# quanpn90/avsr

Hardware: AMD Instinct MI355X
Metric: AV-frames/sec/GPU (fwd+bwd) on 15s clips; WER parity on LRS2 test (higher is better)
Workload: dtype bf16

## Files before the change

### avsr_amd/_lib.py

```python
import ctypes
import os

import torch

_HERE = os.path.dirname(os.path.abspath(__file__))
LIB_PATH = os.environ.get("AVSR_LIB_PATH_AB") or os.path.join(_HERE, "libavsr_hip.so")

AVSR_F32, AVSR_BF16 = 0, 1
ACT_NONE, ACT_GELU, ACT_RELU = 0, 1, 2

_c_p = ctypes.c_void_p
_i64 = ctypes.c_int64
_f = ctypes.c_float
_i = ctypes.c_int


class GemmParams(ctypes.Structure):
    _fields_ = [
        ("M", _i), ("N", _i), ("K", _i), ("batch", _i),
        ("dtype", _i), ("a_kmajor", _i), ("b_kmajor", _i), ("c_f32", _i),
        ("A", _c_p), ("lda", _i64), ("strideA", _i64),
        ("B", _c_p), ("ldb", _i64), ("strideB", _i64),
        ("C", _c_p), ("ldc", _i64), ("strideC", _i64),
        ("alpha", _f), ("beta", _f),
        ("bias", _c_p),
        ("act", _i), ("epi_bwd", _i),
        ("preact", _c_p),
        ("res", _c_p), ("ldr", _i64), ("strideR", _i64),
        ("gate", _c_p),
        ("drop_p", _f),
        ("seed", ctypes.c_uint64),
        ("splitk", _i),
        ("ws", _c_p),
        ("db", _c_p),
        ("db_ws", _c_p),
        ("stamp", _c_p),
        ("skinny_ws", _c_p), ("ln_c1", _c_p), ("ln_eps", ctypes.c_float),
        ("kv_k", _c_p), ("kv_v", _c_p), ("kv_pos", _c_p), ("kv_rows", _i),
        ("slab_cnt", _c_p), ("kv_pos_stride", _i),
    ]


class ConvParams(ctypes.Structure):
    _fields_ = [
        ("dtype", _i),
        ("nimg", _i), ("hin", _i), ("win", _i), ("cin", _i),
        ("hout", _i), ("wout", _i), ("cout", _i),
        ("kh", _i), ("kw", _i), ("sh", _i), ("sw", _i), ("ph", _i), ("pw", _i),
        ("groups", _i),
        ("ldx", _i64), ("ldy", _i64),
        ("x", _c_p), ("w", _c_p), ("y", _c_p),
        ("dx", _c_p), ("dy", _c_p), ("dw", _c_p),
        ("stats", _c_p),
        ("alpha", _f), ("beta", _f),
        ("splitk", _i),
        ("bias", _c_p), ("act", _i), ("preact", _c_p), ("res", _c_p),
        ("ws", _c_p),
        ("bnr_h", _c_p), ("bnr_res", _c_p), ("bnr_scale", _c_p), ("bnr_shift", _c_p), ("bnr_prelu", _c_p),
        ("bnr_mean", _c_p), ("bnr_invstd", _c_p), ("bnr_scale2", _c_p), ("bnr_shift2", _c_p),
        ("bnr_mean2", _c_p), ("bnr_invstd2", _c_p), ("bnr_ws", _c_p),
    ]


class LayerNormParams(ctypes.Structure):
    _fields_ = [
        ("dtype", _i), ("rows", _i), ("N", _i), ("eps", _f),
        ("x", _c_p), ("ldx", _i64), ("y", _c_p), ("ldy", _i64),
        ("gamma", _c_p), ("beta", _c_p), ("mean", _c_p), ("rstd", _c_p),
        ("dy", _c_p), ("lddy", _i64), ("dx", _c_p), ("lddx", _i64),
        ("dres", _c_p), ("lddres", _i64), ("dgamma", _c_p), ("dbeta", _c_p), ("ws", _c_p),
        ("g", _c_p), ("ldg", _i64), ("drop_p", _f), ("seed", ctypes.c_uint64), ("db", _c_p),
    ]


class BnFinalizeParams(ctypes.Structure):
    _fields_ = [
        ("tiles", _i), ("C", _i), ("partials", _c_p), ("gamma", _c_p), ("beta", _c_p),
        ("running_mean", _c_p), ("running_var", _c_p), ("momentum", _f), ("eps", _f),
        ("training", _i), ("mean", _c_p), ("invstd", _c_p), ("scale", _c_p), ("shift", _c_p),
    ]


class BnActParams(ctypes.Structure):
    _fields_ = [
        ("dtype", _i), ("M", _i), ("C", _i),
        ("h", _c_p), ("scale", _c_p), ("shift", _c_p), ("res", _c_p), ("scale2", _c_p), ("shift2", _c_p),
        ("prelu", _c_p), ("y", _c_p), ("dy", _c_p), ("dz", _c_p),
        ("mean", _c_p), ("invstd", _c_p), ("mean2", _c_p), ("invstd2", _c_p),
        ("sums", _c_p), ("dprelu", _c_p), ("dgamma", _c_p), ("dbeta", _c_p), ("dgamma2", _c_p), ("dbeta2", _c_p),
        ("dh", _c_p), ("dh2", _c_p), ("beta_acc", _f), ("ws", _c_p),
    ]


class StemPoolParams(ctypes.Structure):
    _fields_ = [
        ("dtype", _i), ("nimg", _i), ("H", _i), ("W", _i), ("C", _i), ("Ho", _i), ("Wo", _i),
        ("h", _c_p), ("scale", _c_p), ("shift", _c_p), ("prelu", _c_p), ("y", _c_p), ("argmax", _c_p),
        ("dy", _c_p), ("dz", _c_p), ("mean", _c_p), ("invstd", _c_p),
        ("sums", _c_p), ("dprelu", _c_p), ("dgamma", _c_p), ("dbeta", _c_p), ("ws", _c_p),
        ("hmax", _c_p), ("dh", _c_p), ("m_total", _i64),
    ]


class AttnParams(ctypes.Structure):
    _fields_ = [
        ("dtype", _i), ("B", _i), ("H", _i), ("Lq", _i), ("Lk", _i), ("scale", _f),
        ("q", _c_p), ("ldq", _i64), ("k", _c_p), ("ldk", _i64), ("v", _c_p), ("ldv", _i64),
        ("o", _c_p), ("ldo", _i64), ("lse", _c_p), ("klen", _c_p), ("causal", _i),
        ("drop_p", _f), ("seed", ctypes.c_uint64),
        ("dout", _c_p), ("lddo", _i64), ("delta", _c_p), ("dq", _c_p), ("lddq", _i64),
        ("dk", _c_p), ("lddk", _i64), ("dv", _c_p), ("lddv", _i64), ("dq_out", _c_p), ("lddq_out", _i64),
        ("db", _c_p), ("db_ws", _c_p), ("drop_mask", _c_p),
    ]


class XentParams(ctypes.Structure):
    _fields_ = [
        ("dtype", _i), ("rows", _i), ("V", _i), ("x", _c_p), ("ldx", _i64), ("target", _c_p),
        ("smoothing", _f), ("lse", _c_p), ("row_loss", _c_p), ("row_correct", _c_p),
        ("dloss", _c_p), ("coef", _f), ("dx", _c_p), ("lddx", _i64),
    ]


class CtcParams(ctypes.Structure):
    _fields_ = [
        ("dtype", _i), ("B", _i), ("T", _i), ("V", _i), ("Lmax", _i), ("x", _c_p), ("ldx", _i64),
        ("lse", _c_p), ("labels", _c_p), ("label_len", _c_p), ("in_len", _c_p),
        ("alpha", _c_p), ("gamma", _c_p), ("nll", _c_p), ("dloss", _c_p), ("coef", _f),
        ("dx", _c_p), ("lddx", _i64),
    ]


class CtcAlignParams(ctypes.Structure):
    _fields_ = [
        ("dtype", _i), ("B", _i), ("T", _i), ("V", _i), ("Lmax", _i), ("blank", _i), ("x", _c_p), ("ldx", _i64),
        ("lse", _c_p), ("labels", _c_p), ("label_len", _c_p), ("in_len", _c_p),
        ("ws", _c_p), ("ali", _c_p), ("score", _c_p), ("feasible", _c_p),
    ]


class CtcBeamParams(ctypes.Structure):
    _fields_ = [
        ("U", _i), ("Tm", _i), ("V", _i), ("N", _i), ("C", _i), ("blank", _i), ("eos", _i), ("Lcap", _i),
        ("logp", _c_p), ("ldp", _i64), ("tlen", _c_p), ("cand", _c_p), ("ws", _c_p),
        ("n_out", _c_p), ("tokens", _c_p), ("len", _c_p), ("score", _c_p),
    ]


class EwParams(ctypes.Structure):
    _fields_ = [
        ("dtype", _i), ("rows", _i), ("N", _i), ("dy", _c_p), ("lddy", _i64), ("out", _c_p), ("ldout", _i64),
        ("gate", _c_p), ("ldgate", _i64), ("act", _i), ("drop_p", _f), ("seed", ctypes.c_uint64),
        ("alpha", _f), ("db", _c_p), ("ws", _c_p),
    ]


class EmbedParams(ctypes.Structure):
    _fields_ = [
        ("dtype", _i), ("rows", _i), ("L", _i), ("D", _i), ("tok", _c_p), ("table", _c_p), ("pe", _c_p),
        ("scale", _f), ("y", _c_p), ("drop_p", _f), ("seed", ctypes.c_uint64), ("dy", _c_p), ("dtable", _c_p),
        ("pe_row", _c_p), ("pe_row_stride", _i),
    ]


class AdamWParams(ctypes.Structure):
    _fields_ = [
        ("n", _i64), ("param", _c_p), ("grad", _c_p), ("exp_avg", _c_p), ("exp_avg_sq", _c_p),
        ("shadow", _c_p), ("shadow_dtype", _i), ("lr", _f), ("beta1", _f), ("beta2", _f), ("eps", _f),
        ("weight_decay", _f), ("bias_corr1", _f), ("bias_corr2", _f), ("sumsq", _c_p), ("max_norm", _f),
        ("grad_scale", _f), ("max_blocks", _i), ("grad_clear", _c_p),
    ]


def fill(struct_cls, **kw):
    p = struct_cls()
    keep = []
    for k, v in kw.items():
        if v is None:
            continue
        if isinstance(v, torch.Tensor):
            keep.append(v)
            v = v.data_ptr()
        setattr(p, k, v)
    p._keep = keep
    return p


class DecAttnParams(ctypes.Structure):
    _fields_ = [
        ("dtype", _i), ("n", _i), ("H", _i), ("klen_max", _i), ("scale", _f),
        ("q", _c_p), ("ldq", _i64), ("k", _c_p), ("ldk", _i64), ("k_bstride", _i64),
        ("v", _c_p), ("ldv", _i64), ("v_bstride", _i64), ("klen", _c_p), ("o", _c_p), ("ldo", _i64),
        ("kidx", _c_p), ("kmap", _c_p), ("ldmap", _i64), ("group", _i), ("ksplit", _i), ("ws", _c_p),
        ("cnt", _c_p),
    ]


class TopkParams(ctypes.Structure):
    _fields_ = [("rows", _i), ("V", _i), ("K", _i), ("x", _c_p), ("ldx", _i64), ("ids", _c_p)]


class CtcPrefixParams(ctypes.Structure):
    _fields_ = [
        ("n", _i), ("T", _i), ("V", _i), ("P", _i), ("blank", _i), ("eos", _i), ("out_len", _i),
        ("logp", _c_p), ("r_prev", _c_p), ("last", _c_p), ("ids", _c_p), ("r_new", _c_p), ("psi", _c_p),
        ("uidx", _c_p), ("logp_ustride", _i64), ("tlen", _c_p), ("out_len_dev", _c_p),
        ("out_len_stride", _i),
    ]


class BeamSelectParams(ctypes.Structure):
    _fields_ = [
        ("n", _i), ("V", _i), ("P", _i), ("beam", _i), ("blank", _i), ("eos", _i), ("w_dec", _f), ("w_ctc", _f),
        ("dec", _c_p), ("ld", _i64), ("ids", _c_p), ("psi", _c_p), ("s_prev", _c_p), ("score", _c_p),
        ("out_prev", _c_p), ("out_tok", _c_p), ("out_col", _c_p), ("out_score", _c_p), ("out_dec", _c_p),
        ("out_ctc", _c_p), ("out_s", _c_p), ("nseg", _i), ("seg", _c_p),
        ("bonus", _c_p), ("next", _c_p), ("out_bonus", _c_p), ("out_next", _c_p),
        ("lm", _c_p), ("lm_next", _c_p), ("w_lm", _f), ("w_len", _f), ("lm_hi", _f), ("out_lm", _c_p),
        ("out_lm_next", _c_p),
    ]


class NgramLMStruct(ctypes.Structure):
    _fields_ = [
        ("order", _i), ("nodes", _i), ("V", _i), ("start", _i),
        ("child_off", _c_p), ("backoff", _c_p), ("fail", _c_p), ("tok", _c_p), ("logp", _c_p), ("next", _c_p),
        ("uni_logp", _c_p), ("uni_next", _c_p),
    ]


class NgramParams(ctypes.Structure):
    _fields_ = [
        ("lm", NgramLMStruct), ("R", _i), ("P", _i), ("blank", _i), ("eos", _i),
        ("state", _c_p), ("ids", _c_p), ("out", _c_p), ("out_next", _c_p),
    ]

# ... 25 lines not shown
        ("sel_bonus", _c_p), ("sel_next", _c_p), ("shw", _c_p), ("end_hw", _c_p), ("node_out", _c_p),
        ("sel_lm", _c_p), ("sel_lm_next", _c_p), ("slm", _c_p), ("end_lm", _c_p), ("lm_state_out", _c_p),
        ("slen", _c_p), ("end_len", _c_p), ("lm_start", _i),
    ]


class BeamSlotResetParams(ctypes.Structure):
    _fields_ = [
        ("U", _i), ("beam", _i), ("R", _i), ("Lmax", _i), ("slot", _i), ("sos", _i), ("maxlen", _i), ("tlen", _i),
        ("upos", _c_p), ("rowpos", _c_p), ("done", _c_p),
        ("tok", _c_p), ("score", _c_p), ("sdec", _c_p), ("sctc", _c_p), ("s_prev", _c_p),
        ("best_len", _c_p), ("best_end", _c_p), ("maxlen_arr", _c_p), ("tlen_arr", _c_p), ("klen_mem", _c_p),
    ]


class FbankParams(ctypes.Structure):
    _fields_ = [
        ("B", _i), ("T", _i), ("wav", _c_p), ("ldw", _i64), ("n_samples", _c_p),
        ("bins", _i * 28), ("preemph", _f), ("ln_eps", _f), ("out", _c_p),
    ]


class TimeMaskParams(ctypes.Structure):
    _fields_ = [("B", _i), ("L", _i), ("nspan", _i), ("row_bytes", _i64), ("clip_stride_bytes", _i64),
                ("x", _c_p), ("spans", _c_p)]


class AddNoiseParams(ctypes.Structure):
    _fields_ = [("B", _i), ("L", _i), ("x", _c_p), ("ldx", _i64), ("noise", _c_p), ("ldn", _i64),
                ("lengths", _c_p), ("snr_db", _c_p), ("y", _c_p), ("ldy", _i64), ("ws", _c_p)]


class VideoNormParams(ctypes.Structure):
    _fields_ = [
        ("B", _i), ("T", _i), ("H", _i), ("W", _i), ("crop", _i), ("oy", _i), ("ox", _i),
        ("frames", _c_p), ("mean", _f), ("std", _f), ("out", _c_p),
    ]


SYMBOLS = {
    "avsr_version": ([], ctypes.c_char_p),
    "avsr_set_option": ([_i, _i64], _i),
    "avsr_get_option": ([_i], _i64),
    "avsr_gemm": ([ctypes.POINTER(GemmParams), _c_p], _i),
    "avsr_gemm_wgrad_group": ([ctypes.POINTER(GemmParams), _i, _c_p], _i),
    "avsr_gemm_skinny_splits": ([_i, _i, _i], _i),
    "avsr_conv_fwd": ([ctypes.POINTER(ConvParams), _c_p], _i),
    "avsr_conv_bwd_data": ([ctypes.POINTER(ConvParams), _c_p], _i),
    "avsr_conv_bwd_weight": ([ctypes.POINTER(ConvParams), _c_p], _i),
    "avsr_conv_stat_tiles": ([ctypes.POINTER(ConvParams)], _i),
    "avsr_conv_bnr_tiles": ([ctypes.POINTER(ConvParams)], _i),
    "avsr_conv_wgrad_ws": ([ctypes.POINTER(ConvParams)], _i64),
    "avsr_conv_path": ([ctypes.POINTER(ConvParams), _i], _i),
    "avsr_layernorm_fwd": ([ctypes.POINTER(LayerNormParams), _c_p], _i),
    "avsr_layernorm_bwd": ([ctypes.POINTER(LayerNormParams), _c_p], _i),
    "avsr_bn_finalize": ([ctypes.POINTER(BnFinalizeParams), _c_p], _i),
    "avsr_bn_act_fwd": ([ctypes.POINTER(BnActParams), _c_p], _i),
    "avsr_bn_act_bwd_reduce": ([ctypes.POINTER(BnActParams), _c_p], _i),
    "avsr_bn_bwd_apply": ([ctypes.POINTER(BnActParams), _c_p], _i),
    "avsr_stem_pool_fwd": ([ctypes.POINTER(StemPoolParams), _c_p], _i),
    "avsr_stem_pool_bwd_apply": ([ctypes.POINTER(StemPoolParams), _c_p], _i),
    "avsr_bn_bwd_finalize": ([ctypes.POINTER(BnActParams), _i, _c_p], _i),
    "avsr_avgpool_fwd": ([_i, _i, _i, _i, _c_p, _c_p, _c_p], _i),
    "avsr_avgpool_bwd": ([_i, _i, _i, _i, _c_p, _c_p, _c_p], _i),
    "avsr_attn_fwd": ([ctypes.POINTER(AttnParams), _c_p], _i),
    "avsr_debug_attn_stamps": ([_c_p], _i),
    "avsr_attn_bwd_prep": ([ctypes.POINTER(AttnParams), _c_p], _i),
    "avsr_attn_bwd": ([ctypes.POINTER(AttnParams), _c_p], _i),
    "avsr_attn_dropmask": ([ctypes.POINTER(AttnParams), _c_p], _i),
    "avsr_attn_path": ([ctypes.POINTER(AttnParams), _i], _i),
    "avsr_row_lse": ([ctypes.POINTER(XentParams), _c_p], _i),
    "avsr_lsm_fwd": ([ctypes.POINTER(XentParams), _c_p], _i),
    "avsr_lsm_bwd": ([ctypes.POINTER(XentParams), _c_p], _i),
    "avsr_ctc_fwd": ([ctypes.POINTER(CtcParams), _c_p], _i),
    "avsr_ctc_bwd": ([ctypes.POINTER(CtcParams), _c_p], _i),
    "avsr_ctc_align": ([ctypes.POINTER(CtcAlignParams), _c_p], _i),
    "avsr_ctc_beam": ([ctypes.POINTER(CtcBeamParams), _c_p], _i),
    "avsr_loss_finalize": ([_i, _c_p, _i, _c_p, _c_p, _f, _i, _c_p, _c_p], _i),
    "avsr_ew_bwd": ([ctypes.POINTER(EwParams), _c_p], _i),
    "avsr_colsum_defer": ([_i], _i),
    "avsr_colsum_flush": ([_c_p], _i),
    "avsr_colsum_inline": ([_i], _i),
    "avsr_dropout_fwd": ([ctypes.POINTER(EwParams), _c_p], _i),
    "avsr_mask_rows": ([_i, _i, _i, _i, _c_p, _i64, _c_p, _c_p], _i),
    "avsr_embed_fwd": ([ctypes.POINTER(EmbedParams), _c_p], _i),
    "avsr_embed_bwd": ([ctypes.POINTER(EmbedParams), _c_p], _i),
    "avsr_cast": ([_i, _i, _i, _i, _c_p, _i64, _c_p, _i64, _f, _f, _c_p], _i),
    "avsr_cast_flat": ([_i, _i, _i64, _c_p, _c_p, _c_p], _i),
    "avsr_stem_pack": ([_i, _i, _i, _c_p, _c_p, _c_p], _i),
    "avsr_stem_wpack": ([_i, _c_p, _c_p, _c_p], _i),
    "avsr_stem_conv_tiles": ([_i, _i], _i),
    "avsr_stem_wpack2": ([_c_p, _c_p, _c_p], _i),
    "avsr_stem_conv_fwd": ([_i, _i, _c_p, _c_p, _c_p, _c_p, _c_p], _i),
    "avsr_stem_wgrad_unpack": ([_c_p, _c_p, _c_p], _i),
    "avsr_audio_pack": ([_i, _i, _i, _i, _c_p, _c_p, _c_p], _i),
    "avsr_weightnorm_fwd": ([_i, _i, _i, _i, _c_p, _c_p, _c_p, _c_p, _c_p], _i),
    "avsr_weightnorm_bwd": ([_i, _i, _i, _c_p, _c_p, _c_p, _c_p, _c_p, _c_p, _c_p, _c_p], _i),
    "avsr_sumsq": ([_c_p, _i64, _c_p, _c_p, _c_p], _i),
    "avsr_adamw": ([ctypes.POINTER(AdamWParams), _c_p], _i),
    "avsr_log_softmax_rows": ([_i, _i, _i, _c_p, _i64, _c_p, _i64, _c_p], _i),
    "avsr_dec_attn": ([ctypes.POINTER(DecAttnParams), _c_p], _i),
    "avsr_row_topk": ([ctypes.POINTER(TopkParams), _c_p], _i),
    "avsr_log_softmax_topk": ([_i, _i, _i, _c_p, _i64, _c_p, _i64, _i, _c_p, _c_p], _i),
    "avsr_ctc_prefix": ([ctypes.POINTER(CtcPrefixParams), _c_p], _i),
    "avsr_beam_select": ([ctypes.POINTER(BeamSelectParams), _c_p], _i),
    "avsr_hotword_step": ([ctypes.POINTER(HotwordParams), _c_p], _i),
    "avsr_ngram_step": ([ctypes.POINTER(NgramParams), _c_p], _i),
    "avsr_ngram_score_seqs": ([ctypes.POINTER(NgramSeqParams), _c_p], _i),
    "avsr_beam_step_prep": ([_i, _i, _c_p, _c_p, _c_p, _c_p], _i),
    "avsr_beam_kv_put": ([_i, _i, _i, _c_p, _i64, _c_p, _c_p, _c_p, _c_p], _i),
    "avsr_beam_post": ([ctypes.POINTER(BeamPostParams), _c_p], _i),
    "avsr_beam_step_prep_rows": ([_i, _i, _c_p, _c_p, _c_p, _c_p], _i),
    "avsr_beam_kv_put_rows": ([_i, _i, _i, _c_p, _i64, _c_p, _c_p, _c_p, _c_p], _i),
    "avsr_beam_slot_reset": ([ctypes.POINTER(BeamSlotResetParams), _c_p], _i),
    "avsr_gather_rows": ([_i, _i, _i64, _c_p, _i64, _i64, _c_p, _i64, _i64, _c_p, _c_p], _i),
    "avsr_fbank_stack": ([ctypes.POINTER(FbankParams), _c_p], _i),
    "avsr_video_normalize": ([ctypes.POINTER(VideoNormParams), _c_p], _i),
    "avsr_time_mask": ([ctypes.POINTER(TimeMaskParams), _c_p], _i),
    "avsr_add_noise": ([ctypes.POINTER(AddNoiseParams), _c_p], _i),
    "avsr_rgb_to_gray": ([_c_p, _c_p, _i64, _c_p], _i),
}

_lib = None


class AvsrLibError(RuntimeError):
    pass


def load():
    global _lib
    if _lib is not None:
        return _lib
    if not os.path.exists(LIB_PATH):
        raise AvsrLibError(f"{LIB_PATH} not built: run `python -c 'import __graft_entry__ as g; g.build()'`")
    lib = ctypes.CDLL(LIB_PATH, mode=ctypes.RTLD_GLOBAL)
    for name, (argtypes, restype) in SYMBOLS.items():
        if os.environ.get("AVSR_LIB_PATH_AB") and not hasattr(lib, name):
            continue
        fn = getattr(lib, name)
        fn.argtypes = argtypes
        fn.restype = restype
    _lib = lib
    return lib


def check(rc, op):
    if rc != 0:
        raise AvsrLibError(f"{op} failed with code {rc}")


OPTIONS = {"gemm_tile": 0, "attn_sq_fwd": 1, "attn_sq_bwd": 2, "wgrad_dual": 3, "conv_192": 4, "conv_s2phase": 5,
           "conv_patch": 6, "conv_wpatch": 7, "stem_pool_2x2": 8,
           "stem_wpatch": 9, "attn_enc_fused": 10}
TILES = ["128", "256", "256x128", "128x256", "128s3", "128w8s3", "pp", "192", "192x256", "192w8s3", "64", "64s4"]
ATTN_PATHS = ["f32", "tiled", "resident", "sq", "enc"]
CONV_PATHS = ["reg", "glds", "patch", "s2", "wpatch", "stem_wpatch"]
CONV_PASSES = ["fwd", "dgrad", "wgrad"]


def set_option(name, value):
    if name == "gemm_tile" and not isinstance(value, int):
        value = 0 if value in (None, "auto") else TILES.index(value) + 1
    lib = load()
    prev = get_option(name)
    check(lib.avsr_set_option(OPTIONS[name], int(value)), f"avsr_set_option({name}, {value})")
# ... 19 lines not shown
```

### avsr_amd/csrc/common.h

```cpp
#pragma once
#include <hip/hip_runtime.h>
#include <stdint.h>
#include "avsr_hip.h"

typedef __bf16 bf16;
typedef __bf16 bf16x8 __attribute__((ext_vector_type(8)));
typedef __bf16 bf16x4 __attribute__((ext_vector_type(4)));
typedef float f32x16 __attribute__((ext_vector_type(16)));
typedef float f32x4 __attribute__((ext_vector_type(4)));
typedef int v4i32 __attribute__((ext_vector_type(4)));
typedef float f32x2 __attribute__((ext_vector_type(2)));

#define AVSR_DEV __device__ __forceinline__

AVSR_DEV float to_f(float x) { return x; }
AVSR_DEV float to_f(bf16 x) { return (float)x; }
template <typename T> AVSR_DEV T from_f(float x);
template <> AVSR_DEV float from_f<float>(float x) { return x; }
template <> AVSR_DEV bf16 from_f<bf16>(float x) { return (bf16)x; }

struct alignas(16) v16 { uint32_t w[4]; };

AVSR_DEV float fexp2(float x) { return __builtin_amdgcn_exp2f(x); }

template <int R> AVSR_DEV float rorf(float x) {
  return __int_as_float(__builtin_amdgcn_update_dpp(0, __float_as_int(x), 0x120 + R, 0xf, 0xf, false));
}
template <int R> AVSR_DEV int rori(int x) { return __builtin_amdgcn_update_dpp(0, x, 0x120 + R, 0xf, 0xf, false); }
AVSR_DEV float lanef(float x, int l) { return __int_as_float(__builtin_amdgcn_readlane(__float_as_int(x), l)); }
AVSR_DEV float row_sum16(float x) {
  x += rorf<8>(x); x += rorf<4>(x); x += rorf<2>(x); x += rorf<1>(x);
  return x;
}
AVSR_DEV float wave_sum(float x) {
  x = row_sum16(x);
  return (lanef(x, 0) + lanef(x, 16)) + (lanef(x, 32) + lanef(x, 48));
}
AVSR_DEV float xor32_max(float x) {
  const auto r = __builtin_amdgcn_permlane32_swap(__float_as_uint(x), __float_as_uint(x), false, false);
  return fmaxf(__uint_as_float(r[0]), __uint_as_float(r[1]));
}
AVSR_DEV float xor32_sum(float x) {
  const auto r = __builtin_amdgcn_permlane32_swap(__float_as_uint(x), __float_as_uint(x), false, false);
  return __uint_as_float(r[0]) + __uint_as_float(r[1]);
}
AVSR_DEV float wave_max(float x) {
  x = fmaxf(x, rorf<8>(x)); x = fmaxf(x, rorf<4>(x)); x = fmaxf(x, rorf<2>(x)); x = fmaxf(x, rorf<1>(x));
  return fmaxf(fmaxf(lanef(x, 0), lanef(x, 16)), fmaxf(lanef(x, 32), lanef(x, 48)));
}

AVSR_DEV uint32_t fmix32(uint32_t h) {
  h ^= h >> 16; h *= 0x85EBCA6Bu;
  h ^= h >> 13; h *= 0xC2B2AE35u;
  return h ^ (h >> 16);
}
AVSR_DEV uint32_t mix32_hi(uint64_t seed, uint32_t hi) {
  return (uint32_t)seed ^ fmix32(hi ^ (uint32_t)(seed >> 32) ^ 0x68E31DA4u);
}
AVSR_DEV uint32_t mix32_lo(uint32_t pre, uint32_t lo) { return fmix32((lo * 0x9E3779B1u) ^ pre); }
AVSR_DEV uint32_t mix32(uint64_t seed, uint64_t idx) {
  return mix32_lo(mix32_hi(seed, (uint32_t)(idx >> 32)), (uint32_t)idx);
}
AVSR_DEV uint32_t drop_thr16(float p) { return (uint32_t)(p * 65536.f + 0.5f); }
AVSR_DEV float drop_keep_scale(uint32_t thr) { return thr < 65536u ? 65536.f / (float)(65536u - thr) : 0.f; }
AVSR_DEV uint32_t drop_half(uint32_t h, bool odd) { return odd ? (h >> 16) : (h & 0xFFFFu); }

AVSR_DEV float drop_scale(float p, uint64_t seed, uint64_t idx) {
  const uint32_t thr = drop_thr16(p);
  return drop_half(mix32(seed, idx >> 1), idx & 1) >= thr ? drop_keep_scale(thr) : 0.0f;
}

AVSR_DEV void drop8(float p, uint64_t seed, uint64_t d0, float* v) {
  const uint32_t thr = drop_thr16(p);
  const float ks = drop_keep_scale(thr);
  const uint64_t p0 = d0 >> 1;
  const uint32_t lo = (uint32_t)p0;
  if (!(d0 & 1) && lo <= 0xFFFFFFFCu) {
    const uint32_t pre = mix32_hi(seed, (uint32_t)(p0 >> 32));
    const uint32_t g0 = lo * 0x9E3779B1u;
#pragma unroll
    for (int q = 0; q < 4; ++q) {
      const uint32_t h = fmix32((g0 + (uint32_t)q * 0x9E3779B1u) ^ pre);
      v[2 * q] *= (h & 0xFFFFu) >= thr ? ks : 0.0f;
      v[2 * q + 1] *= (h >> 16) >= thr ? ks : 0.0f;
    }
  } else {
#pragma unroll
    for (int q = 0; q < 8; ++q) v[q] *= drop_scale(p, seed, d0 + q);
  }
}

AVSR_DEV float gelu_erf(float x) { return 0.5f * x * (1.0f + erff(x * 0.70710678118654752f)); }
AVSR_DEV float gelu_erf_grad(float x) {
  float cdf = 0.5f * (1.0f + erff(x * 0.70710678118654752f));
  float pdf = 0.39894228040143268f * __expf(-0.5f * x * x);
  return cdf + x * pdf;
}
AVSR_DEV float erf_as(float z, float ez2) {
  const float t = __builtin_amdgcn_rcpf(fmaf(0.3275911f, fabsf(z), 1.0f));
  const float p = t * fmaf(t, fmaf(t, fmaf(t, fmaf(t, 1.061405429f, -1.453152027f), 1.421413741f), -0.284496736f), 0.254829592f);
  return copysignf(fmaf(-p, ez2, 1.0f), z);
}
AVSR_DEV float gelu_fast(float x) {
  const float z = x * 0.70710678118654752f;
  return 0.5f * x * (1.0f + erf_as(z, __expf(-z * z)));
}
AVSR_DEV float gelu_fast_grad(float x) {
  const float z = x * 0.70710678118654752f, e = __expf(-z * z);
  return 0.5f * (1.0f + erf_as(z, e)) + x * 0.39894228040143268f * e;
}
typedef float f32x2 __attribute__((ext_vector_type(2)));
AVSR_DEV f32x2 erf_as2(f32x2 z, f32x2 ez2) {
  const f32x2 az = {fabsf(z.x), fabsf(z.y)};
  const f32x2 d = az * 0.3275911f + 1.0f;
  const f32x2 t = {__builtin_amdgcn_rcpf(d.x), __builtin_amdgcn_rcpf(d.y)};
  f32x2 p = t * 1.061405429f + -1.453152027f;
  p = p * t + 1.421413741f;
  p = p * t + -0.284496736f;
  p = p * t + 0.254829592f;
  const f32x2 r = 1.0f - (p * t) * ez2;
  return f32x2{copysignf(r.x, z.x), copysignf(r.y, z.y)};
}
AVSR_DEV f32x2 exp_negsq2(f32x2 z) {
  const f32x2 q = z * z;
  return f32x2{__expf(-q.x), __expf(-q.y)};
}
AVSR_DEV f32x2 gelu_fast2(f32x2 x) {
  const f32x2 z = x * 0.70710678118654752f;
  const f32x2 hx = x * 0.5f;
  return hx + hx * erf_as2(z, exp_negsq2(z));
}
AVSR_DEV f32x2 gelu_fast_grad2(f32x2 x) {
  const f32x2 z = x * 0.70710678118654752f, e = exp_negsq2(z);
  return 0.5f + 0.5f * erf_as2(z, e) + (x * 0.39894228040143268f) * e;
}
template <typename T> AVSR_DEV float act_fwd_t(int act, float h) {
  if constexpr (sizeof(T) == 2) return act == AVSR_ACT_GELU ? gelu_fast(h) : (act == AVSR_ACT_RELU ? fmaxf(h, 0.f) : h);
  else return act == AVSR_ACT_GELU ? gelu_erf(h) : (act == AVSR_ACT_RELU ? fmaxf(h, 0.f) : h);
}
template <typename T> AVSR_DEV float act_bwd_t(int act, float h) {
  if constexpr (sizeof(T) == 2) return act == AVSR_ACT_GELU ? gelu_fast_grad(h) : (act == AVSR_ACT_RELU ? (h > 0.f ? 1.f : 0.f) : 1.f);
  else return act == AVSR_ACT_GELU ? gelu_erf_grad(h) : (act == AVSR_ACT_RELU ? (h > 0.f ? 1.f : 0.f) : 1.f);
}
AVSR_DEV float act_fwd(int act, float h) {
  return act == AVSR_ACT_GELU ? gelu_erf(h) : (act == AVSR_ACT_RELU ? fmaxf(h, 0.f) : h);
}
AVSR_DEV float act_bwd(int act, float h) {
  return act == AVSR_ACT_GELU ? gelu_erf_grad(h) : (act == AVSR_ACT_RELU ? (h > 0.f ? 1.f : 0.f) : 1.f);
}

AVSR_DEV void split8(const float* x, bf16x8& hi, bf16x8& lo) {
#pragma unroll
  for (int j = 0; j < 8; ++j) {
    bf16 h = (bf16)x[j];
    hi[j] = h;
    lo[j] = (bf16)(x[j] - (float)h);
  }
}

AVSR_DEV f32x4 mfma16(const bf16x8& a, const bf16x8& b, const f32x4& c) {
  return __builtin_amdgcn_mfma_f32_16x16x32_bf16(a, b, c, 0, 0, 0);
}
AVSR_DEV f32x16 mfma32(const bf16x8& a, const bf16x8& b, const f32x16& c) {
  return __builtin_amdgcn_mfma_f32_32x32x16_bf16(a, b, c, 0, 0, 0);
}

int64_t avsr_opt(int option);

#define AVSR_CHECK_LAUNCH() do { hipError_t e_ = hipGetLastError(); if (e_ != hipSuccess) return (int)e_; } while (0)

static inline int avsr_aligned16(const void* p) { return ((uintptr_t)p & 15u) == 0; }

// ... 52 lines not shown
```

### avsr_amd/csrc/elementwise.hip

```cpp
#include "common.h"

namespace {

struct EwArgs {
  int rows, N;
  const void* dy; int64_t lddy; void* out; int64_t ldout;
  const void* gate; int64_t ldgate; int act;
  float drop_p; uint64_t seed; float alpha; float* db; float* ws;
};

template <typename T>
__global__ __launch_bounds__(256) void ew_bwd_kernel(EwArgs a) {
  constexpr int VE = VecW<T>::VE;
  __shared__ float red[4 * 64 * 8];
  const int nv = a.N / VE;
  const int cvl = threadIdx.x & 63, rl = threadIdx.x >> 6;
  const int cv = blockIdx.x * 64 + cvl;
  const int chunk = (a.rows + gridDim.y - 1) / gridDim.y;
  const int r0 = blockIdx.y * chunk, r1 = min(a.rows, r0 + chunk);
  float acc[VE];
#pragma unroll
  for (int j = 0; j < VE; ++j) acc[j] = 0.f;
  if (cv < nv) {
    for (int r = r0 + rl; r < r1; r += 4) {
      float d[VE], g[VE];
      ldv((const T*)a.dy + (int64_t)r * a.lddy + cv * VE, d);
      if (a.gate) ldv((const T*)a.gate + (int64_t)r * a.ldgate + cv * VE, g);
#pragma unroll
      for (int j = 0; j < VE; ++j) d[j] *= a.alpha;
      if (a.drop_p > 0.f) {
        const uint64_t i0 = (uint64_t)r * a.N + cv * VE;
        if constexpr (VE == 8) drop8(a.drop_p, a.seed, i0, d);
        else {
#pragma unroll
          for (int j = 0; j < VE; ++j) d[j] *= drop_scale(a.drop_p, a.seed, i0 + j);
        }
      }
#pragma unroll
      for (int j = 0; j < VE; ++j) {
        float v = d[j];
        if (a.gate) v *= act_bwd_t<T>(a.act, g[j]);
        acc[j] += v;
        d[j] = v;
      }
      if (a.out) stv((T*)a.out + (int64_t)r * a.ldout + cv * VE, d);
    }
  }
  if (!a.db) return;
#pragma unroll
  for (int j = 0; j < VE; ++j) red[(rl * 64 + cvl) * VE + j] = acc[j];
  __syncthreads();
  if (rl == 0 && cv < nv) {
#pragma unroll
    for (int j = 0; j < VE; ++j) {
      const float t = red[(0 * 64 + cvl) * VE + j] + red[(1 * 64 + cvl) * VE + j] + red[(2 * 64 + cvl) * VE + j] +
                      red[(3 * 64 + cvl) * VE + j];
      a.ws[(int64_t)blockIdx.y * a.N + cv * VE + j] = t;
    }
  }
}

template <typename T>
__global__ __launch_bounds__(256) void mask_rows_kernel(int B, int T_, int N, T* x, int64_t ldx, const int* len) {
  constexpr int VE = VecW<T>::VE;
  const int nv = N / VE;
  const int64_t total = (int64_t)B * T_ * nv;
  for (int64_t i = blockIdx.x * 256 + threadIdx.x; i < total; i += (int64_t)gridDim.x * 256) {
    const int64_t row = i / nv;
    const int b = (int)(row / T_), t = (int)(row % T_);
    if (t >= len[b]) {
      float z[VE];
#pragma unroll
      for (int j = 0; j < VE; ++j) z[j] = 0.f;
      stv(x + row * ldx + (i % nv) * VE, z);
    }
  }
}

template <typename T>
__global__ __launch_bounds__(256) void embed_kernel(avsr_embed_params p, int bwd) {
  constexpr int VE = VecW<T>::VE;
  const int nv = p.D / VE;
  const int64_t total = (int64_t)p.rows * nv;
  for (int64_t i = blockIdx.x * 256 + threadIdx.x; i < total; i += (int64_t)gridDim.x * 256) {
    const int r = (int)(i / nv), d0 = (int)(i % nv) * VE;
    const int tok = p.tok[r];
    const int pos = p.pe_row ? p.pe_row[(int64_t)r * p.pe_row_stride] : r % p.L;
    if (!bwd) {
      float e[VE], o[VE];
      ldv((const T*)p.table + (int64_t)tok * p.D + d0, e);
#pragma unroll
      for (int j = 0; j < VE; ++j) {
        float v = e[j] * p.scale + p.pe[(int64_t)pos * p.D + d0 + j];
        if (p.drop_p > 0.f) v *= drop_scale(p.drop_p, p.seed, (uint64_t)r * p.D + d0 + j);
        o[j] = v;
      }
      stv((T*)p.y + (int64_t)r * p.D + d0, o);
    }
  }
}

template <typename T>
__global__ __launch_bounds__(256) void embed_bwd_kernel(avsr_embed_params p) {
  constexpr int VE = VecW<T>::VE;
  const int r = blockIdx.x;
  const int tok = p.tok[r];
  __shared__ int seen;
  if (threadIdx.x == 0) seen = 0;
  __syncthreads();
  for (int q = threadIdx.x; q < r; q += 256)
    if (p.tok[q] == tok) seen = 1;
  __syncthreads();
  if (seen) return;
  const int nv = p.D / VE;
  for (int c = threadIdx.x; c < nv; c += 256) {
    const int d0 = c * VE;
    float acc[VE];
#pragma unroll
    for (int j = 0; j < VE; ++j) acc[j] = 0.f;
    for (int q = r; q < p.rows; ++q) {
      if (p.tok[q] != tok) continue;
      float g[VE];
      ldv((const T*)p.dy + (int64_t)q * p.D + d0, g);
#pragma unroll
      for (int j = 0; j < VE; ++j) {
        float v = g[j] * p.scale;
        if (p.drop_p > 0.f) v *= drop_scale(p.drop_p, p.seed, (uint64_t)q * p.D + d0 + j);
        acc[j] += v;
      }
    }
    float* dt = p.dtable + (int64_t)tok * p.D + d0;
#pragma unroll
    for (int j = 0; j < VE; ++j) dt[j] += acc[j];
  }
}

template <typename S, typename D>
__global__ __launch_bounds__(256) void cast_kernel(int rows, int cols, const S* src, int64_t lds, D* dst,
                                                   int64_t ldd, float alpha, float beta) {
  const int64_t c0 = ((int64_t)blockIdx.x * 256 + threadIdx.x) * 4;
  if (c0 >= cols) return;
  for (int r = blockIdx.y; r < rows; r += gridDim.y) {
    const S* s = src + (int64_t)r * lds + c0;
    D* d = dst + (int64_t)r * ldd + c0;
#pragma unroll
    for (int q = 0; q < 4; ++q) {
      if (c0 + q < cols) {
        float v = alpha * to_f(s[q]);
        if (beta != 0.f) v += beta * to_f(d[q]);
        d[q] = from_f<D>(v);
      }
    }
  }
}

__global__ __launch_bounds__(256) void cast_flat_f32_bf16_kernel(int64_t n8, const float4* __restrict__ src,
                                                                 bf16x8* __restrict__ dst) {
  for (int64_t i = (int64_t)blockIdx.x * 256 + threadIdx.x; i < n8; i += (int64_t)gridDim.x * 256) {
    const float4 a = src[2 * i], b = src[2 * i + 1];
    bf16x8 o;
    o[0] = (bf16)a.x; o[1] = (bf16)a.y; o[2] = (bf16)a.z; o[3] = (bf16)a.w;
    o[4] = (bf16)b.x; o[5] = (bf16)b.y; o[6] = (bf16)b.z; o[7] = (bf16)b.w;
    dst[i] = o;
  }
}

__global__ __launch_bounds__(256) void cast_flat_bf16_f32_kernel(int64_t n8, const bf16x8* __restrict__ src,
                                                                 float4* __restrict__ dst) {
  for (int64_t i = (int64_t)blockIdx.x * 256 + threadIdx.x; i < n8; i += (int64_t)gridDim.x * 256) {
    const bf16x8 v = src[i];
    dst[2 * i] = float4{(float)v[0], (float)v[1], (float)v[2], (float)v[3]};
    dst[2 * i + 1] = float4{(float)v[4], (float)v[5], (float)v[6], (float)v[7]};
  }
}

template <typename T>
__global__ __launch_bounds__(256) void audio_pack_kernel(int B, int F, int T_, const float* a, T* out) {
  const int64_t total = (int64_t)B * T_ * F;
  for (int64_t i = blockIdx.x * 256 + threadIdx.x; i < total; i += (int64_t)gridDim.x * 256) {
    const int f = (int)(i % F);
    const int64_t bt = i / F;
    const int b = (int)(bt / T_), t = (int)(bt % T_);
    out[i] = from_f<T>(a[((int64_t)b * F + f) * T_ + t]);
  }
}

template <typename T>
int ew_launch(const avsr_ew_params* p, hipStream_t st) {
  constexpr int VE = VecW<T>::VE;
  if (p->N % VE) return AVSR_E_SHAPE;
  if (p->rows == 0) return 0;
  if (p->db && !p->ws) return AVSR_E_ARG;
  const int nv = p->N / VE;
  dim3 grid((nv + 63) / 64, 1);
  int gy = 4096 / (int)grid.x;
  gy = gy < 16 ? 16 : (gy > AVSR_EW_ROWBLOCKS ? AVSR_EW_ROWBLOCKS : gy);
  gy = gy > p->rows ? p->rows : gy;
  grid.y = gy;
  EwArgs a;
  a.rows = p->rows; a.N = p->N; a.dy = p->dy; a.lddy = p->lddy; a.out = p->out; a.ldout = p->ldout;
  a.gate = p->gate; a.ldgate = p->ldgate; a.act = p->act; a.drop_p = p->drop_p; a.seed = p->seed;
  a.alpha = p->alpha; a.db = p->db; a.ws = p->ws;
  hipLaunchKernelGGL(ew_bwd_kernel<T>, grid, dim3(256), 0, st, a);
  AVSR_CHECK_LAUNCH();
  if (p->db) return colsum_launch((const float*)p->ws, (int)grid.y, (int64_t)p->N, p->N, p->db, 0, nullptr, st);
  return 0;
}

int embed_launch(const avsr_embed_params* p, int bwd, hipStream_t st) {
  if (!p) return AVSR_E_ARG;
  return avsr_by_dtype(p->dtype, [&](auto t) -> int {
    using T = decltype(t);
    constexpr int VE = VecW<T>::VE;
    if (p->D % VE) return AVSR_E_SHAPE;
    if (p->rows <= 0) return 0;
    if (bwd) hipLaunchKernelGGL(embed_bwd_kernel<T>, dim3(p->rows), dim3(256), 0, st, *p);
    else hipLaunchKernelGGL(embed_kernel<T>, dim3(avsr_grid((int64_t)p->rows * p->D / VE)), dim3(256), 0, st, *p, bwd);
    AVSR_CHECK_LAUNCH();
    return 0;
  });
}

}

extern "C" int avsr_ew_bwd(const avsr_ew_params* p, void* stream) {
  if (!p) return AVSR_E_ARG;
  return avsr_by_dtype(p->dtype, [&](auto t) -> int { return ew_launch<decltype(t)>(p, (hipStream_t)stream); });
}

extern "C" int avsr_dropout_fwd(const avsr_ew_params* p, void* stream) {
  if (!p) return AVSR_E_ARG;
  return avsr_by_dtype(p->dtype, [&](auto t) -> int {
    if (!p->out) return AVSR_E_ARG;
    avsr_ew_params q = *p;
    q.gate = nullptr; q.db = nullptr;
    return ew_launch<decltype(t)>(&q, (hipStream_t)stream);
  });
}

extern "C" int avsr_mask_rows(int dtype, int B, int T, int N, void* x, int64_t ldx, const int* len, void* stream) {
  return avsr_by_dtype(dtype, [&](auto t) -> int {
    using E = decltype(t);
    constexpr int VE = VecW<E>::VE;
    if (N % VE || ldx % VE) return AVSR_E_ALIGN;
    const int g = avsr_grid((int64_t)B * T * N / VE);
    hipLaunchKernelGGL(mask_rows_kernel<E>, dim3(g), dim3(256), 0, (hipStream_t)stream, B, T, N, (E*)x, ldx, len);
    AVSR_CHECK_LAUNCH();
    return 0;
  });
}

extern "C" int avsr_embed_fwd(const avsr_embed_params* p, void* stream) { return embed_launch(p, 0, (hipStream_t)stream); }
extern "C" int avsr_embed_bwd(const avsr_embed_params* p, void* stream) { return embed_launch(p, 1, (hipStream_t)stream); }

extern "C" int avsr_cast(int sd, int dd, int rows, int cols, const void* src, int64_t lds, void* dst, int64_t ldd,
                         float alpha, float beta, void* stream) {
  if (rows <= 0 || cols <= 0) return 0;
  const int64_t gx = ((int64_t)cols + 1023) / 1024;
  int64_t gy = 4096 / gx;
  gy = gy < 1 ? 1 : (gy > rows ? rows : gy);
  gy = gy > 65535 ? 65535 : gy;
  const dim3 g((unsigned)gx, (unsigned)gy);
  hipStream_t st = (hipStream_t)stream;
  if (sd == AVSR_F32 && dd == AVSR_BF16) hipLaunchKernelGGL((cast_kernel<float, bf16>), dim3(g), dim3(256), 0, st, rows, cols, (const float*)src, lds, (bf16*)dst, ldd, alpha, beta);
  else if (sd == AVSR_F32 && dd == AVSR_F32) hipLaunchKernelGGL((cast_kernel<float, float>), dim3(g), dim3(256), 0, st, rows, cols, (const float*)src, lds, (float*)dst, ldd, alpha, beta);
  else if (sd == AVSR_BF16 && dd == AVSR_F32) hipLaunchKernelGGL((cast_kernel<bf16, float>), dim3(g), dim3(256), 0, st, rows, cols, (const bf16*)src, lds, (float*)dst, ldd, alpha, beta);
  else if (sd == AVSR_BF16 && dd == AVSR_BF16) hipLaunchKernelGGL((cast_kernel<bf16, bf16>), dim3(g), dim3(256), 0, st, rows, cols, (const bf16*)src, lds, (bf16*)dst, ldd, alpha, beta);
  else return AVSR_E_DTYPE;
  AVSR_CHECK_LAUNCH();
  return 0;
}

extern "C" int avsr_cast_flat(int sd, int dd, int64_t n, const void* src, void* dst, void* stream) {
  if (n <= 0) return 0;
  hipStream_t st = (hipStream_t)stream;
  if (sd == AVSR_F32 && dd == AVSR_BF16 && n % 8 == 0 && ((uintptr_t)src & 15) == 0 && ((uintptr_t)dst & 15) == 0) {
    const int64_t n8 = n / 8;
    int64_t g = (n8 + 255) / 256;
    g = g > 256 * 32 ? 256 * 32 : g;
    hipLaunchKernelGGL(cast_flat_f32_bf16_kernel, dim3((unsigned)g), dim3(256), 0, st, n8, (const float4*)src, (bf16x8*)dst);
    AVSR_CHECK_LAUNCH();
    return 0;
  }
  if (sd == AVSR_BF16 && dd == AVSR_F32 && n % 8 == 0 && ((uintptr_t)src & 15) == 0 && ((uintptr_t)dst & 15) == 0) {
    const int64_t n8 = n / 8;
    int64_t g = (n8 + 255) / 256;
    g = g > 256 * 32 ? 256 * 32 : g;
    hipLaunchKernelGGL(cast_flat_bf16_f32_kernel, dim3((unsigned)g), dim3(256), 0, st, n8, (const bf16x8*)src, (float4*)dst);
    AVSR_CHECK_LAUNCH();
    return 0;
  }
  const int64_t cols = 4096, rows = n / cols, tail = n - rows * cols;
  const size_t es = sd == AVSR_F32 ? 4 : 2, ed = dd == AVSR_F32 ? 4 : 2;
  if (rows > 0) {
    const int rc = avsr_cast(sd, dd, (int)rows, (int)cols, src, cols, dst, cols, 1.f, 0.f, stream);
    if (rc) return rc;
  }
  if (tail > 0) return avsr_cast(sd, dd, 1, (int)tail, (const char*)src + rows * cols * es, tail,
                                 (char*)dst + rows * cols * ed, tail, 1.f, 0.f, stream);
  return 0;
}

extern "C" int avsr_audio_pack(int dtype, int B, int F, int T, const float* audio, void* out, void* stream) {
  return avsr_by_dtype(dtype, [&](auto t) -> int {
    using E = decltype(t);
    const int g = avsr_grid((int64_t)B * T * F);
    hipLaunchKernelGGL(audio_pack_kernel<E>, dim3(g), dim3(256), 0, (hipStream_t)stream, B, F, T, audio, (E*)out);
    AVSR_CHECK_LAUNCH();
    return 0;
  });
}
```

### avsr_amd/csrc/gemm.hip

```cpp
#include "gemm_dense.h"
#include "gemm_pp.h"
#include <type_traits>
#include <utility>

using namespace gemmd;

namespace {

template <typename T, typename OutT, int WM, int WN, bool AK, bool BK>
__global__ __launch_bounds__(NT) void dense_kernel(DenseArgs a) {
  extern __shared__ __attribute__((aligned(16))) char smem[];
  using TL = Tile<T, WM, WN, AK, BK>;
  const int z = blockIdx.z, bz = z / a.splits, sp = z % a.splits;
  const int m0 = blockIdx.y * TL::BM, n0 = blockIdx.x * TL::BN;
  using LA = typename std::conditional<AK, LdDenseK<T, TL::BM>, LdDenseR<T, TL::BM>>::type;
  using LB = typename std::conditional<BK, LdDenseK<T, TL::BN>, LdDenseR<T, TL::BN>>::type;
  LA la; la.p = (const T*)a.A + (int64_t)bz * a.sA; la.ld = a.lda; la.rext = a.M; la.K = a.K;
  LB lb; lb.p = (const T*)a.B + (int64_t)bz * a.sB; lb.ld = a.ldb; lb.rext = a.N; lb.K = a.K;
  const int kbeg = sp * a.kchunk, kend = min(a.K, kbeg + a.kchunk);
  f32x16 acc[2][2];
  mainloop<T, WM, WN>(la, lb, m0, n0, kbeg, kend, acc, smem);
  const Epi e = tile_epi<T, OutT, EV_GENERIC>(a, bz, sp);
  epilogue<T, OutT, WM, WN>(e, m0, n0, acc, smem);
}

template <typename OutT, bool AK, bool BK, class CF, int EV = EV_GENERIC>
__global__ __launch_bounds__(CF::NTH, CF::MINB) void dense_glds_kernel(DenseArgs a, int tiles_m, int tiles_n) {
  extern __shared__ __attribute__((aligned(16))) char smem[];
  if (a.stamp != nullptr && threadIdx.x == 0) atomicMin(a.stamp, (unsigned long long)__builtin_amdgcn_s_memrealtime());
  const int id = gemmg::xcd_remap(blockIdx.x, gridDim.x);
  int tm, tn, z;
  gemmg::tile_of(id, tiles_m, tiles_n, tm, tn, z);
  const int bz = z / a.splits, sp = z % a.splits;
  const int m0 = tm * CF::BM, n0 = tn * CF::BN;
  const int kbeg = sp * a.kchunk, kend = min(a.K, kbeg + a.kchunk);
  const int lane = threadIdx.x & 63, wave = __builtin_amdgcn_readfirstlane(threadIdx.x >> 6);
  f32x4 acc[CF::TM][CF::TN];
  const int nk = (kend - kbeg + gemmg::GBK - 1) / gemmg::GBK;
  if (a.a_bytes) {
    using LA = typename std::conditional<AK, gemmg::BDenseK<CF::BM, CF::NW>, gemmg::BDenseR<CF::BM, CF::NW>>::type;
    using LB = typename std::conditional<BK, gemmg::BDenseK<CF::BN, CF::NW>, gemmg::BDenseR<CF::BN, CF::NW>>::type;
    LA la; la.init((const bf16*)a.A + (int64_t)bz * a.sA, a.a_bytes, a.lda, m0, a.M, kend, wave, lane);
    LB lb; lb.init((const bf16*)a.B + (int64_t)bz * a.sB, a.b_bytes, a.ldb, n0, a.N, kend, wave, lane);
    gemmg::mainloop_glds<CF>(la, lb, kbeg, nk, acc, smem);
  } else {
    using LA = typename std::conditional<AK, gemmg::GDenseK<CF::BM, CF::NW>, gemmg::GDenseR<CF::BM, CF::NW>>::type;
    using LB = typename std::conditional<BK, gemmg::GDenseK<CF::BN, CF::NW>, gemmg::GDenseR<CF::BN, CF::NW>>::type;
    LA la; la.init((const bf16*)a.A + (int64_t)bz * a.sA, a.lda, m0, a.M, kend, wave, lane);
    LB lb; lb.init((const bf16*)a.B + (int64_t)bz * a.sB, a.ldb, n0, a.N, kend, wave, lane);
    gemmg::mainloop_glds<CF>(la, lb, kbeg, nk, acc, smem);
  }
  const Epi e = tile_epi<bf16, OutT, EV>(a, bz, sp);
  gemmg::epilogue_g<bf16, OutT, CF, EV>(e, m0, n0, acc, smem);
  if (a.stamp != nullptr) {
    __syncthreads();
    if (threadIdx.x == 0) atomicMax(a.stamp + 1, (unsigned long long)__builtin_amdgcn_s_memrealtime());
  }
}

template <typename OutT, bool AK, bool BK>
__global__ __launch_bounds__(gemmpp::NTH, 1) void dense_pp_kernel(DenseArgs a, int tiles_m, int tiles_n) {
  extern __shared__ __attribute__((aligned(16))) char smem[];
  const int id = gemmg::xcd_remap(blockIdx.x, gridDim.x);
  int tm, tn, z;
  gemmg::tile_of(id, tiles_m, tiles_n, tm, tn, z);
  const int bz = z / a.splits, sp = z % a.splits;
  const int m0 = tm * gemmpp::BM, n0 = tn * gemmpp::BN;
  const int kbeg = sp * a.kchunk, kend = min(a.K, kbeg + a.kchunk);
  const int lane = threadIdx.x & 63, wave = __builtin_amdgcn_readfirstlane(threadIdx.x >> 6);
  using LA = typename std::conditional<AK, gemmpp::HalfK<64>, gemmpp::HalfR<64>>::type;
  using LB = typename std::conditional<BK, gemmpp::HalfK<32>, gemmpp::HalfR<32>>::type;
  LA la; la.init((const bf16*)a.A + (int64_t)bz * a.sA, a.lda, m0, a.M, kend, wave, lane);
  LB lb; lb.init((const bf16*)a.B + (int64_t)bz * a.sB, a.ldb, n0, a.N, kend, wave, lane);
  f32x4 acc[8][4];
  gemmpp::mainloop_pp(la, lb, kbeg, (kend - kbeg + gemmg::GBK - 1) / gemmg::GBK, acc, smem);
  const Epi e = tile_epi<bf16, OutT, EV_GENERIC>(a, bz, sp);
  gemmg::epilogue_g<bf16, OutT, gemmpp::CF>(e, m0, n0, acc, smem);
}

template <typename OutT, bool AK, bool BK>
int launch_pp(const DenseArgs& a, int batch, hipStream_t st) {
  const int tm = (a.M + 255) / 256, tn = (a.N + 255) / 256;
  const long nwg = (long)tm * tn * batch * a.splits;
  if (nwg > 0x7fffffffL) return AVSR_E_SHAPE;
  hipLaunchKernelGGL((dense_pp_kernel<OutT, AK, BK>), dim3((unsigned)nwg), dim3(gemmpp::NTH), gemmpp::LDS_BYTES, st, a,
                     tm, tn);
  AVSR_CHECK_LAUNCH();
  return 0;
}

template <typename OutT>
int epi_variant(const DenseArgs& a, int batch) {
  const Epi& e = a.e;
  if (e.atomic || e.stats || e.rm_wc || e.alpha != 1.f || e.beta != 0.f || (e.N % 8)) return EV_GENERIC;
  const uintptr_t ptrs = (uintptr_t)e.C | (uintptr_t)e.preact | (uintptr_t)e.res | (uintptr_t)e.gate | (uintptr_t)e.bias;
  if (ptrs & 15u) return EV_GENERIC;
  const int64_t so = (int64_t)sizeof(OutT);
  if (((e.ldc * so) | (e.ldc * 2) | (e.ldr * 2)) & 15) return EV_GENERIC;
  if (batch > 1 && (((a.sC * so) | (a.sC * 2) | (a.sR * 2)) & 15)) return EV_GENERIC;
  if (a.splits > 1 && ((a.sSplit * so) & 15)) return EV_GENERIC;
  const bool drop = e.drop_p > 0.f;
  if (!e.bwd) {
    if (e.gate || e.colsum) return EV_GENERIC;
    if (!e.bias) return (!e.preact && !e.act && !e.res && !drop) ? EV_PLAIN : EV_GENERIC;
    if (!e.preact && !e.act && !e.res && !drop) return EV_BIAS;
    if (!e.preact && !e.act && e.res) return EV_BIAS_RES;
    if (e.preact && e.act == AVSR_ACT_GELU && !e.res) return EV_BIAS_ACT_PRE;
    return EV_GENERIC;
  }
  if (e.bias || e.preact || e.res) return EV_GENERIC;
  if (e.gate && e.act == AVSR_ACT_GELU) return EV_GATE;
  if (!e.gate && !e.act && !drop && !e.colsum) return EV_PLAIN;
  return EV_GENERIC;
}

template <typename OutT, bool BK, int EV>
constexpr bool ev_built() {
  if (EV == EV_GENERIC) return true;
  if (sizeof(OutT) != 2) return false;
  return BK ? (EV == EV_BIAS || EV == EV_BIAS_RES || EV == EV_BIAS_ACT_PRE) : (EV == EV_PLAIN || EV == EV_GATE);
}

template <typename OutT, bool AK, bool BK, class CF, int EV>
int launch_glds_ev(const DenseArgs& a, int tm, int tn, long nwg, hipStream_t st) {
  if constexpr (!ev_built<OutT, BK, EV>()) {
    return launch_glds_ev<OutT, AK, BK, CF, EV_GENERIC>(a, tm, tn, nwg, st);
  } else {
    hipLaunchKernelGGL((dense_glds_kernel<OutT, AK, BK, CF, EV>), dim3((unsigned)nwg), dim3(CF::NTH), CF::LDS_BYTES,
                       st, a, tm, tn);
    AVSR_CHECK_LAUNCH();
    return 0;
  }
}

template <typename OutT, bool AK, bool BK, class CF, bool VARIANTS = false>
int launch_glds(const DenseArgs& a, int batch, hipStream_t st) {
  const int tm = (a.M + CF::BM - 1) / CF::BM, tn = (a.N + CF::BN - 1) / CF::BN;
  const long nwg = (long)tm * tn * batch * a.splits;
  if (nwg > 0x7fffffffL) return AVSR_E_SHAPE;
  if constexpr (VARIANTS) {
    switch (epi_variant<OutT>(a, batch)) {
      case EV_PLAIN: return launch_glds_ev<OutT, AK, BK, CF, EV_PLAIN>(a, tm, tn, nwg, st);
      case EV_BIAS: return launch_glds_ev<OutT, AK, BK, CF, EV_BIAS>(a, tm, tn, nwg, st);
      case EV_BIAS_RES: return launch_glds_ev<OutT, AK, BK, CF, EV_BIAS_RES>(a, tm, tn, nwg, st);
      case EV_BIAS_ACT_PRE: return launch_glds_ev<OutT, AK, BK, CF, EV_BIAS_ACT_PRE>(a, tm, tn, nwg, st);
      case EV_GATE: return launch_glds_ev<OutT, AK, BK, CF, EV_GATE>(a, tm, tn, nwg, st);
      default: break;
    }
  }
  return launch_glds_ev<OutT, AK, BK, CF, EV_GENERIC>(a, tm, tn, nwg, st);
}

using Cfg128 = gemmg::GCfg<2, 2, 2, 2, 2>;
using Cfg256 = gemmg::GCfg<2, 4, 4, 2, 2>;
using Cfg256x128 = gemmg::GCfg<4, 2, 2, 2, 3>;
using Cfg128x256 = gemmg::GCfg<2, 4, 2, 2, 3>;
using Cfg128s3 = gemmg::GCfg<2, 2, 2, 2, 3>;
using Cfg128w8s3 = gemmg::GCfg<2, 4, 2, 1, 3>;
using Cfg192 = gemmg::GCfg<2, 2, 3, 2, 2>;
using Cfg192x256 = gemmg::GCfg<2, 4, 3, 2, 2>;
using Cfg192w8s3 = gemmg::GCfg<2, 4, 3, 1, 3>;
using Cfg64 = gemmg::GCfg<2, 2, 1, 1, 2>;
using Cfg64s4 = gemmg::GCfg<2, 2, 1, 1, 4>;
struct CorePP { static constexpr int BM = gemmpp::BM; };

template <int ID_, class CF_, bool VARIANTS_ = false>
struct TileRow {
  static constexpr int ID = ID_;
  static constexpr bool R_OK = 512 % CF_::BM == 0;
  template <bool AK> using CF = std::conditional_t<AK || R_OK, CF_, Cfg128>;
  static constexpr int bm(bool ak) { return ak ? CF<true>::BM : CF<false>::BM; }
  template <typename OutT, bool AK, bool BK>
  static int launch(const DenseArgs& a, int batch, hipStream_t st) {
    if constexpr (std::is_same_v<CF<AK>, CorePP>) return launch_pp<OutT, AK, BK>(a, batch, st);
    else return launch_glds<OutT, AK, BK, CF<AK>, VARIANTS_ && (AK || R_OK)>(a, batch, st);
  }
};
template <class... R> struct TileTable { static constexpr int COUNT = sizeof...(R); };

using Tiles = TileTable<
    TileRow<AVSR_TILE_128, Cfg128>,
    TileRow<AVSR_TILE_256, Cfg256>,
    TileRow<AVSR_TILE_256x128, Cfg256x128>,
    TileRow<AVSR_TILE_128x256, Cfg128x256>,
// ... 23 lines not shown
template <typename OutT, bool AK, bool BK, class... R>
int launch_cfg(TileTable<R...>, int cfg, const DenseArgs& a, int batch, hipStream_t st) {
  int rc = AVSR_E_ARG;
  (void)((cfg == R::ID && ((rc = R::template launch<OutT, AK, BK>(a, batch, st)), true)) || ...);
  return rc;
}

#ifndef AVSR_AB_FWD2
#define AVSR_AB_FWD2 AVSR_TILE_192
#endif
#ifndef AVSR_AB_ROUND1
#define AVSR_AB_ROUND1 AVSR_TILE_192w8s3
#endif
int tile_cfg(const avsr_gemm_params* p, int splits) {
  const int forced = (int)avsr_opt(AVSR_OPT_GEMM_TILE) - 1;
  if (forced >= 0) return forced;
  const long tiles_z = (long)p->batch * splits;
  const long t128 = (long)((p->M + 127) / 128) * ((p->N + 127) / 128) * tiles_z;
  if (p->a_kmajor) {
    const long t192 = (long)((p->M + 191) / 192) * ((p->N + 127) / 128) * tiles_z;
    const long n128 = (t128 + 255) / 256, n192 = (t192 + 255) / 256;
    if (n192 >= 2 && 3 * n192 * 50 <= 2 * n128 * 51) return AVSR_AB_FWD2;
    if (t192 > 128 && t192 <= 256) return AVSR_AB_ROUND1;
  }
  const long t64 = (long)((p->M + 63) / 64) * ((p->N + 63) / 64) * tiles_z;
  if (t128 < 256 && t64 >= 2 * t128) return (t64 <= 256 && p->K >= 2048) ? AVSR_TILE_64s4 : AVSR_TILE_64;
  return AVSR_TILE_128;
}

template <typename OutT>
int glds_by_layout(const avsr_gemm_params* p, int cfg, const DenseArgs& a, hipStream_t st) {
  if (p->a_kmajor && p->b_kmajor) return launch_cfg<OutT, true, true>(Tiles{}, cfg, a, p->batch, st);
  if (p->a_kmajor) return launch_cfg<OutT, true, false>(Tiles{}, cfg, a, p->batch, st);
  if (p->b_kmajor) return launch_cfg<OutT, false, true>(Tiles{}, cfg, a, p->batch, st);
  return launch_cfg<OutT, false, false>(Tiles{}, cfg, a, p->batch, st);
}

template <typename T, typename OutT, int WM, int WN, bool AK, bool BK>
int launch(const DenseArgs& a, int batch, hipStream_t st) {
  using TL = Tile<T, WM, WN, AK, BK>;
  dim3 grid((a.N + TL::BN - 1) / TL::BN, (a.M + TL::BM - 1) / TL::BM, batch * a.splits);
  hipLaunchKernelGGL((dense_kernel<T, OutT, WM, WN, AK, BK>), grid, dim3(NT), TL::LDS_BYTES, st, a);
  AVSR_CHECK_LAUNCH();
  return 0;
}

template <typename T, typename OutT, int WM, int WN>
int by_layout(const avsr_gemm_params* p, const DenseArgs& a, hipStream_t st) {
  if (p->a_kmajor && p->b_kmajor) return launch<T, OutT, WM, WN, true, true>(a, p->batch, st);
  if (p->a_kmajor) return launch<T, OutT, WM, WN, true, false>(a, p->batch, st);
  if (p->b_kmajor) return launch<T, OutT, WM, WN, false, true>(a, p->batch, st);
  return launch<T, OutT, WM, WN, false, false>(a, p->batch, st);
}

template <typename T, typename OutT>
int by_tile(const avsr_gemm_params* p, const DenseArgs& a, hipStream_t st) {
  if (p->N <= 64) return by_layout<T, OutT, 4, 1>(p, a, st);
  if (p->M <= 64) return by_layout<T, OutT, 1, 4>(p, a, st);
  return by_layout<T, OutT, 2, 2>(p, a, st);
}

int check_params(const avsr_gemm_params* p, int splits, bool slab, bool glds) {
  if (p->M < 0 || p->N < 0 || p->K < 0 || p->batch <= 0) return AVSR_E_SHAPE;
  if (p->dtype != AVSR_F32 && p->dtype != AVSR_BF16) return AVSR_E_DTYPE;
  const int ve = p->dtype == AVSR_BF16 ? 8 : 4;
  if (!avsr_aligned16(p->A) || !avsr_aligned16(p->B)) return AVSR_E_ALIGN;
  if (p->lda % ve || p->ldb % ve || p->strideA % ve || p->strideB % ve) return AVSR_E_ALIGN;
  if ((p->a_kmajor || p->b_kmajor) && (p->K % ve)) return AVSR_E_ALIGN;
  if (splits > 1 && !(p->c_f32 || p->dtype == AVSR_F32)) return AVSR_E_ARG;
  if (slab && (p->bias || p->act || p->preact || p->res || p->gate || p->drop_p > 0.f || p->epi_bwd || (p->N % 4) ||
               (p->ldc % 4) || (p->strideC % 4) || !avsr_aligned16(p->C)))
    return AVSR_E_ARG;
  const bool skinny = !glds && !slab && skinny_ok(p, splits);
  if (p->kv_k && (p->dtype != AVSR_F32 || p->M > 64 || splits > 1 || (p->N % 3) || !p->kv_v || !p->kv_pos ||
                  p->kv_rows < p->M || p->kv_pos_stride < 0))
    return AVSR_E_ARG;
  if (p->kv_k && !skinny) return AVSR_E_ARG;
  if (p->ln_c1 && (p->dtype != AVSR_F32 || p->M > 64 || splits > 1)) return AVSR_E_ARG;
  if (p->db && (!glds || p->dtype != AVSR_BF16 || p->c_f32 || splits > 1 || p->batch != 1 || !p->db_ws || (p->N % 8) ||
                (p->ldc % 8) || (p->ldr % 8) || !avsr_aligned16(p->C) || (p->gate && !avsr_aligned16(p->gate)) ||
                (p->preact && !avsr_aligned16(p->preact)) || (p->res && (!avsr_aligned16(p->res) || (p->ldr % 8))) ||
                (p->bias && !avsr_aligned16(p->bias))))
    return AVSR_E_ARG;
  if (p->K == 0) return AVSR_E_SHAPE;
  if (p->ln_c1 && !skinny) return AVSR_E_ARG;
  return 0;
}

}

bool gemmd::glds_ok(const avsr_gemm_params* p) {
  return p->dtype == AVSR_BF16 && p->M >= 128 && p->N >= 128 && (p->a_kmajor || p->M % 8 == 0) &&
         (p->b_kmajor || p->N % 8 == 0);
}

DenseArgs gemmd::dense_args(const avsr_gemm_params* p, int splits, bool slab) {
  DenseArgs a{};
  a.M = p->M; a.N = p->N; a.K = p->K;
  a.splits = splits;
  const int kq = glds_ok(p) ? gemmg::GBK : BKE;
  a.kchunk = ((p->K + splits - 1) / splits + kq - 1) / kq * kq;
  a.A = p->A; a.lda = p->lda; a.sA = p->strideA;
  a.B = p->B; a.ldb = p->ldb; a.sB = p->strideB;
  {
    const int esz = p->dtype == AVSR_BF16 ? 2 : 4;
    const int64_t ea = (p->a_kmajor ? ((int64_t)(p->M - 1) * p->lda + p->K) : ((int64_t)(p->K - 1) * p->lda + p->M)) * esz;
    const int64_t eb = (p->b_kmajor ? ((int64_t)(p->N - 1) * p->ldb + p->K) : ((int64_t)(p->K - 1) * p->ldb + p->N)) * esz;
    const int64_t lim = (int64_t)gemmg::OOB - (1 << 20);
    const bool ok = ea > 0 && eb > 0 && ea < lim && eb < lim;
    a.a_bytes = ok ? (uint32_t)ea : 0u;
    a.b_bytes = ok ? (uint32_t)eb : 0u;
  }
  a.sC = p->strideC; a.sR = p->strideR;
  a.stamp = p->stamp;
  a.falpha = 1.f;
  a.ln_c1 = p->ln_c1; a.ln_eps = p->ln_eps;
  a.kvk = (float*)p->kv_k; a.kvv = (float*)p->kv_v; a.kvpos = p->kv_pos; a.kvrows = p->kv_rows; a.kvposs = p->kv_pos_stride;
  Epi& e = a.e;
  e.M = p->M; e.N = p->N; e.C = p->C; e.ldc = p->ldc;
  e.alpha = p->alpha; e.beta = p->beta; e.bias = p->bias;
  e.act = p->act; e.bwd = p->epi_bwd; e.atomic = splits > 1 && !slab;
  if (slab) {
    e.C = p->ws; e.ldc = p->N; e.alpha = 1.f; e.beta = 0.f;
    a.sSplit = (int64_t)p->M * p->N + AVSR_GEMM_SLAB_PAD; a.sC = (int64_t)splits * a.sSplit;
  }
  e.preact = p->preact; e.res = p->res; e.ldr = p->ldr; e.gate = p->gate;
  e.drop_p = p->drop_p; e.seed = p->seed;
  e.colsum = p->db ? p->db_ws : nullptr;
  return a;
}

extern "C" int avsr_gemm(const avsr_gemm_params* p, void* stream) {
  if (!p) return AVSR_E_ARG;
  if (p->M == 0 || p->N == 0) return 0;
  const int splits = p->splitk > 1 ? p->splitk : 1;
  const bool slab = splits > 1 && p->ws != nullptr;
  const bool glds = glds_ok(p);
  int rc = check_params(p, splits, slab, glds);
  if (rc) return rc;
  const DenseArgs a = dense_args(p, splits, slab);
  hipStream_t st = (hipStream_t)stream;
  int colsum_bm = 0;
  if (!glds && !slab && skinny_ok(p, splits)) return skinny_launch(p, a, st);
  if (glds && wgrad_dual_ok(p, splits, slab)) {
    bool reduced;
    rc = wgrad_dual_launch(p, a, st, &reduced);
    if (reduced) return rc;
  } else if (glds) {
    const int cfg = tile_cfg(p, splits);
    rc = p->c_f32 ? glds_by_layout<float>(p, cfg, a, st) : glds_by_layout<bf16>(p, cfg, a, st);
    if (p->db) colsum_bm = cfg_bm(Tiles{}, cfg, p->a_kmajor != 0);
  } else if (p->dtype == AVSR_F32) rc = by_tile<float, float>(p, a, st);
  else if (p->c_f32) rc = by_tile<bf16, float>(p, a, st);
  else rc = by_tile<bf16, bf16>(p, a, st);
  if (rc) return rc;
  if (colsum_bm) {
    const int tiles = (p->M + colsum_bm - 1) / colsum_bm;
    rc = colsum_launch((const float*)p->db_ws, tiles, (int64_t)p->N, p->N, p->db, 0, nullptr, st);
    if (rc) return rc;
  }
  if (!slab) return 0;
  const int64_t per = (int64_t)p->M * (p->N / 4);
  if (per >= (1ll << 31)) return AVSR_E_SHAPE;
  const dim3 g((unsigned)avsr_grid(per, 256, 4096), p->batch);
  hipLaunchKernelGGL(slab_reduce_kernel, g, dim3(256), 0, st, (const float*)p->ws, splits, p->M, p->N,
                     (int64_t)p->M * p->N + AVSR_GEMM_SLAB_PAD, (float*)p->C, p->ldc, p->strideC, p->alpha, p->beta);
  AVSR_CHECK_LAUNCH();
  return 0;
}
```

### avsr_amd/csrc/gemm_core.h

```cpp
#pragma once
#include "common.h"

namespace gemmcore {

constexpr int BKE = 32, NT = 256;

template <typename T> struct V { static constexpr int VE = 16 / (int)sizeof(T); static constexpr int ROW = BKE + VE; };

AVSR_DEV void zero(v16& v) { v.w[0] = v.w[1] = v.w[2] = v.w[3] = 0u; }

struct ConvGeom {
  int nimg, hin, win, hout, wout;
  int kh, kw, sh, sw, ph, pw;
  int cin, cout;
  int64_t ldx, ldy;
  FastDiv f_hw_out, f_w_out;
  FastDiv f_hw_in, f_w_in;
  FastDiv f_kw;
  int cin_shift, cout_shift;
  int ktot_w, tap_kfw, tap_kh0, tap_kw0, tap_step;
};

template <typename T, int R> struct LdDenseK {
  static constexpr bool KMAJ = true;
// ... 176 lines not shown
  }
}

template <typename T, int WM, int WN, bool AK = true, bool BK = true> struct Tile {
  static constexpr int BM = 64 * WM, BN = 64 * WN;
  static constexpr int SA = Img<T, BM, AK>::ELEMS, SB = Img<T, BN, BK>::ELEMS;
  static constexpr int ML_BYTES = 2 * (SA + SB) * (int)sizeof(T);
  static constexpr int EP_BYTES = (BM / 2) * (BN + 4) * 4;
  static constexpr int LDS_BYTES = ML_BYTES > EP_BYTES ? ML_BYTES : EP_BYTES;
};

template <typename T, int WM, int WN, class LA, class LB>
AVSR_DEV void mainloop(LA& la, LB& lb, int m0, int n0, int kbeg, int kend, f32x16 (&acc)[2][2], char* smem) {
  using TL = Tile<T, WM, WN, LA::KMAJ, LB::KMAJ>;
  T* lA = (T*)smem;
  T* lB = lA + 2 * TL::SA;
  const int tid = threadIdx.x, lane = tid & 63, wid = tid >> 6;
  const int wm = wid / WN, wn = wid % WN;
#pragma unroll
  for (int i = 0; i < 2; ++i)
#pragma unroll
    for (int j = 0; j < 2; ++j)
#pragma unroll
      for (int r = 0; r < 16; ++r) acc[i][j][r] = 0.f;
  if (kbeg >= kend) return;
  la.init(m0, tid);
  lb.init(n0, tid);
  v16 ra[LA::VPT], rb[LB::VPT];
  const int nk = (kend - kbeg + BKE - 1) / BKE;
  la.load(m0, kbeg, ra, tid);
  lb.load(n0, kbeg, rb, tid);
  lstore<T, TL::BM, LA::KMAJ>(lA, ra, tid);
  lstore<T, TL::BN, LB::KMAJ>(lB, rb, tid);
  __syncthreads();
  for (int kt = 0; kt < nk; ++kt) {
    const int cur = kt & 1;
    const bool more = kt + 1 < nk;
    if (more) {
      la.load(m0, kbeg + (kt + 1) * BKE, ra, tid);
      lb.load(n0, kbeg + (kt + 1) * BKE, rb, tid);
    }
    const T* cA = lA + cur * TL::SA;
    const T* cB = lB + cur * TL::SB;
#pragma unroll
    for (int s = 0; s < BKE / 16; ++s) {
      bf16x8 ah[2], al[2], bh[2], bl[2];
#pragma unroll
      for (int i = 0; i < 2; ++i) frag<T, TL::BM, LA::KMAJ>(cA, wm * 64 + i * 32, s, lane, ah[i], al[i]);
#pragma unroll
      for (int j = 0; j < 2; ++j) frag<T, TL::BN, LB::KMAJ>(cB, wn * 64 + j * 32, s, lane, bh[j], bl[j]);
#pragma unroll
      for (int i = 0; i < 2; ++i)
#pragma unroll
        for (int j = 0; j < 2; ++j) {
          acc[i][j] = mfma32(ah[i], bh[j], acc[i][j]);
          if constexpr (sizeof(T) == 4) {
            acc[i][j] = mfma32(ah[i], bl[j], acc[i][j]);
            acc[i][j] = mfma32(al[i], bh[j], acc[i][j]);
          }
        }
    }
    if (more) {
      lstore<T, TL::BM, LA::KMAJ>(lA + (cur ^ 1) * TL::SA, ra, tid);
      lstore<T, TL::BN, LB::KMAJ>(lB + (cur ^ 1) * TL::SB, rb, tid);
    }
    __syncthreads();
  }
}

struct Epi {
  int M, N;
  void* C; int64_t ldc;
  float alpha, beta;
  const float* bias;
  int act, bwd, atomic;
  void* preact;
  const void* res; int64_t ldr;
  const void* gate;
  float drop_p; uint64_t seed; uint64_t drop_base;
  float* stats;
  int stats_tiles;
  int rm_wc, rm_hc, rm_hin, rm_win, rm_a, rm_b;
  float* colsum;
};

AVSR_DEV int epi_row(const Epi& e, int r) {
  if (e.rm_wc == 0) return r;
  const int q = r / e.rm_wc, j = r - q * e.rm_wc;
  const int n = q / e.rm_hc, i = q - n * e.rm_hc;
  return (n * e.rm_hin + 2 * i + e.rm_a) * e.rm_win + 2 * j + e.rm_b;
}

AVSR_DEV int acc_row(int wm, int i, int r, int lane) { return wm * 64 + i * 32 + (r & 3) + 8 * (r >> 2) + 4 * (lane >> 5); }
AVSR_DEV int acc_col(int wn, int j, int lane) { return wn * 64 + j * 32 + (lane & 31); }

template <typename T, typename OutT, int NE>
AVSR_DEV void epi_elems(const Epi& e, int row, int col, const float* v_in) {
  OutT* C = (OutT*)e.C;
  const T* R = (const T*)e.res;
  T* P = (T*)e.preact;
  const T* G = (const T*)e.gate;
  const int64_t off = (int64_t)row * e.ldc + col;
  if (e.atomic) {
#pragma unroll
    for (int q = 0; q < NE; ++q)
      if (col + q < e.N) atomicAdd((float*)C + off + q, e.alpha * v_in[q]);
    return;
  }
#pragma unroll
  for (int q = 0; q < NE; ++q) {
    if (col + q >= e.N) break;
    float v = e.alpha * v_in[q];
    const uint64_t didx = e.drop_base + (uint64_t)row * (uint64_t)e.N + col + q;
    if (!e.bwd) {
      if (e.bias) v += e.bias[col + q];
      if (P) P[off + q] = from_f<T>(v);
      v = act_fwd_t<T>(e.act, v);
      if (e.drop_p > 0.f) v *= drop_scale(e.drop_p, e.seed, didx);
      if (R) v += to_f(R[(int64_t)row * e.ldr + col + q]);
    } else {
      if (e.drop_p > 0.f) v *= drop_scale(e.drop_p, e.seed, didx);
      if (G) v *= act_bwd_t<T>(e.act, to_f(G[off + q]));
    }
    if (e.beta != 0.f) v += e.beta * to_f(C[off + q]);
    C[off + q] = from_f<OutT>(v);
  }
}

template <typename T, typename OutT>
AVSR_DEV bool epi_vec_ok(const Epi& e) {
  const uintptr_t a = (uintptr_t)e.C | (uintptr_t)e.preact | (uintptr_t)e.res | (uintptr_t)e.gate | (uintptr_t)e.bias;
  return !e.atomic && (a & 15u) == 0 && ((e.ldc * (int64_t)sizeof(OutT)) & 15) == 0 &&
         ((e.ldc * (int64_t)sizeof(T)) & 15) == 0 && ((e.ldr * (int64_t)sizeof(T)) & 15) == 0;
}

template <typename T> AVSR_DEV void ld8(const T* p, float (&o)[8]) {
  if constexpr (sizeof(T) == 2) {
    const bf16x8 x = *(const bf16x8*)p;
#pragma unroll
    for (int j = 0; j < 8; ++j) o[j] = (float)x[j];
  } else {
    const f32x4 x0 = *(const f32x4*)p, x1 = *(const f32x4*)(p + 4);
#pragma unroll
    for (int j = 0; j < 4; ++j) { o[j] = x0[j]; o[j + 4] = x1[j]; }
  }
}
template <typename T> AVSR_DEV void st8(T* p, const float (&o)[8]) {
  if constexpr (sizeof(T) == 2) {
    bf16x8 x;
#pragma unroll
    for (int j = 0; j < 8; ++j) x[j] = (bf16)o[j];
    *(bf16x8*)p = x;
  } else {
    *(f32x4*)p = f32x4{o[0], o[1], o[2], o[3]};
    *(f32x4*)(p + 4) = f32x4{o[4], o[5], o[6], o[7]};
  }
}

enum { EV_GENERIC = 0, EV_PLAIN = 1, EV_BIAS = 2, EV_BIAS_RES = 3, EV_BIAS_ACT_PRE = 4, EV_GATE = 5 };

template <int EV> AVSR_DEV void epi_fold(Epi& e) {
  if constexpr (EV != EV_GENERIC) {
    e.alpha = 1.f; e.beta = 0.f; e.atomic = 0; e.stats = nullptr; e.rm_wc = 0;
    e.bwd = EV == EV_GATE;
    if constexpr (EV == EV_PLAIN || EV == EV_GATE) e.bias = nullptr;
    else __builtin_assume(e.bias != nullptr);
    if constexpr (EV == EV_BIAS_ACT_PRE) __builtin_assume(e.preact != nullptr);
    else e.preact = nullptr;
    if constexpr (EV == EV_BIAS_RES) __builtin_assume(e.res != nullptr);
    else e.res = nullptr;
    if constexpr (EV == EV_GATE) __builtin_assume(e.gate != nullptr);
    else e.gate = nullptr;
    e.act = (EV == EV_BIAS_ACT_PRE || EV == EV_GATE) ? AVSR_ACT_GELU : AVSR_ACT_NONE;
    if constexpr (EV == EV_PLAIN || EV == EV_BIAS) e.drop_p = 0.f;
    if constexpr (EV != EV_GATE) e.colsum = nullptr;
  }
}

template <typename T, typename OutT>
AVSR_DEV void epi_vec8(const Epi& e, int row, int col, float (&v)[8], const float* bv = nullptr,
                       const bf16x8* op = nullptr) {
  const int64_t off = (int64_t)row * e.ldc + col;
#pragma unroll
  for (int q = 0; q < 8; ++q) v[q] *= e.alpha;
  float t[8];
  const uint64_t d0 = e.drop_base + (uint64_t)row * (uint64_t)e.N + col;
  if (!e.bwd) {
    if (e.bias) {
      if (bv) {
#pragma unroll
        for (int q = 0; q < 8; ++q) t[q] = bv[q];
      } else {
        ld8(e.bias + col, t);
      }
#pragma unroll
      for (int q = 0; q < 8; ++q) v[q] += t[q];
    }
    if (e.preact) st8((T*)e.preact + off, v);
    if (e.act) {
      if (sizeof(T) == 2 && e.act == AVSR_ACT_GELU) {
#pragma unroll
        for (int q = 0; q < 8; q += 2) {
          const f32x2 r = gelu_fast2(f32x2{v[q], v[q + 1]});
          v[q] = r.x; v[q + 1] = r.y;
        }
      } else {
#pragma unroll
        for (int q = 0; q < 8; ++q) v[q] = act_fwd_t<T>(e.act, v[q]);
      }
    }
    if (e.drop_p > 0.f) drop8(e.drop_p, e.seed, d0, v);
    if (e.res) {
      if (op) {
#pragma unroll
        for (int q = 0; q < 8; ++q) t[q] = (float)(*op)[q];
      } else {
        ld8((const T*)e.res + (int64_t)row * e.ldr + col, t);
      }
#pragma unroll
      for (int q = 0; q < 8; ++q) v[q] += t[q];
    }
  } else {
    if (e.drop_p > 0.f) drop8(e.drop_p, e.seed, d0, v);
    if (e.gate) {
      if (op) {
#pragma unroll
        for (int q = 0; q < 8; ++q) t[q] = (float)(*op)[q];
      } else {
        ld8((const T*)e.gate + off, t);
      }
      if (sizeof(T) == 2 && e.act == AVSR_ACT_GELU) {
#pragma unroll
        for (int q = 0; q < 8; q += 2) {
          const f32x2 r = gelu_fast_grad2(f32x2{t[q], t[q + 1]});
          v[q] *= r.x; v[q + 1] *= r.y;
        }
      } else {
#pragma unroll
        for (int q = 0; q < 8; ++q) v[q] *= act_bwd_t<T>(e.act, t[q]);
      }
    }
  }
  if (e.beta != 0.f) {
    ld8((const OutT*)e.C + off, t);
#pragma unroll
    for (int q = 0; q < 8; ++q) v[q] += e.beta * t[q];
  }
  st8((OutT*)e.C + off, v);
}

template <typename T, typename OutT, int WM, int WN>
AVSR_DEV void epilogue(const Epi& e, int m0, int n0, f32x16 (&acc)[2][2], char* smem) {
  constexpr int BM = 64 * WM, BN = 64 * WN, HR = BM / 2, LDR = BN + 4;
  const int tid = threadIdx.x, lane = tid & 63, wid = tid >> 6;
  const int wm = wid / WN, wn = wid % WN;
  float* st = (float*)smem;
  if (e.stats) {
    __syncthreads();
    float* red = st;
#pragma unroll
    for (int j = 0; j < 2; ++j) {
      float s = 0.f, c = 0.f;
#pragma unroll
      for (int i = 0; i < 2; ++i)
#pragma unroll
        for (int r = 0; r < 16; ++r) {
          const bool ok = m0 + acc_row(wm, i, r, lane) < e.M;
          s += ok ? e.alpha * acc[i][j][r] : 0.f;
          c += ok ? 1.f : 0.f;
        }
      s += __shfl_xor(s, 32, 64);
      c += __shfl_xor(c, 32, 64);
      const float mean = c > 0.f ? s / c : 0.f;
      float m2 = 0.f;
#pragma unroll
      for (int i = 0; i < 2; ++i)
#pragma unroll
        for (int r = 0; r < 16; ++r) {
          const bool ok = m0 + acc_row(wm, i, r, lane) < e.M;
          const float d = e.alpha * acc[i][j][r] - mean;
          m2 += ok ? d * d : 0.f;
        }
      m2 += __shfl_xor(m2, 32, 64);
      if (lane < 32) {
        const int lc = acc_col(wn, j, lane);
        red[(wm * BN + lc) * 3 + 0] = c;
        red[(wm * BN + lc) * 3 + 1] = mean;
        red[(wm * BN + lc) * 3 + 2] = m2;
      }
    }
    __syncthreads();
    for (int lc = tid; lc < BN; lc += NT) {
      const int col = n0 + lc;
      if (col < e.N) {
        float n = 0.f, mean = 0.f, m2 = 0.f;
        for (int w = 0; w < WM; ++w) {
          const float nb = red[(w * BN + lc) * 3 + 0], mb = red[(w * BN + lc) * 3 + 1], qb = red[(w * BN + lc) * 3 + 2];
          if (nb > 0.f) {
            const float nn = n + nb, d = mb - mean;
            mean += d * nb / nn;
            m2 += qb + d * d * n * nb / nn;
            n = nn;
          }
        }
        float* o = e.stats + ((int64_t)col * e.stats_tiles + m0 / BM) * 3;
        o[0] = n; o[1] = mean; o[2] = m2;
// ... 47 lines not shown
```

### avsr_amd/csrc/gemm_glds.h

```cpp
#pragma once
#include "gemm_core.h"

namespace gemmg {
using namespace gemmcore;

constexpr int GBK = 64;

static __device__ __attribute__((aligned(16))) uint4 g_zero_line[64];

typedef __attribute__((address_space(3))) void lds_void_t;
typedef const __attribute__((address_space(1))) void gbl_void_t;

AVSR_DEV void glds16(const void* src, char* lds_wave_base) {
  __builtin_amdgcn_global_load_lds((gbl_void_t*)src, (lds_void_t*)lds_wave_base, 16, 0, 0);
}

template <int CPR> AVSR_DEV int rswz(int k) {
  return CPR >= 16 ? ((k & 3) | (((k >> 3) & 1) << 2)) << 1 : (((k >> 1) & 1) | (((k >> 3) & 1) << 1)) << 1;
}

template <int R, int NW> struct GDenseK {
  static constexpr bool KMAJ = true;
  static constexpr int SLOTS = R / 8 / NW;
  const bf16* p[SLOTS];
// ... 219 lines not shown

template <class CF, class LA, class LB>
AVSR_DEV void mainloop_glds(const LA& la, const LB& lb, int kbeg, int nk, f32x4 (&acc)[CF::TM][CF::TN], char* smem) {
  mainloop_glds<CF>(la, lb, kbeg, nk, acc, smem, __builtin_amdgcn_readfirstlane(threadIdx.x >> 6));
}

template <typename T, typename OutT, class CF, int EV = EV_GENERIC>
AVSR_DEV void epilogue_g(const Epi& e, int m0, int n0, f32x4 (&acc)[CF::TM][CF::TN], char* smem) {
  constexpr int BN = CF::BN, LDR = BN + 4, SR = CF::WM * 32;
  const int tid = threadIdx.x, lane = tid & 63, wave = tid >> 6;
  const int wm = wave / CF::WN, wn = wave % CF::WN;
  float* st = (float*)smem;
  const bool vec = EV != EV_GENERIC || epi_vec_ok<T, OutT>(e);
  if (e.stats) {
    __syncthreads();
    float* red = st;
#pragma unroll
    for (int j = 0; j < CF::TN; ++j) {
      float s = 0.f, c = 0.f;
#pragma unroll
      for (int i = 0; i < CF::TM; ++i)
#pragma unroll
        for (int r = 0; r < 4; ++r) {
          const int row = wm * 32 * CF::FM + i * 16 + 4 * (lane >> 4) + r;
          const bool ok = m0 + row < e.M;
          s += ok ? e.alpha * acc[i][j][r] : 0.f;
          c += ok ? 1.f : 0.f;
        }
      s += __shfl_xor(s, 16, 64); s += __shfl_xor(s, 32, 64);
      c += __shfl_xor(c, 16, 64); c += __shfl_xor(c, 32, 64);
      const float mean = c > 0.f ? s / c : 0.f;
      float m2 = 0.f;
#pragma unroll
      for (int i = 0; i < CF::TM; ++i)
#pragma unroll
        for (int r = 0; r < 4; ++r) {
          const int row = wm * 32 * CF::FM + i * 16 + 4 * (lane >> 4) + r;
          const float d = e.alpha * acc[i][j][r] - mean;
          m2 += m0 + row < e.M ? d * d : 0.f;
        }
      m2 += __shfl_xor(m2, 16, 64); m2 += __shfl_xor(m2, 32, 64);
      if (lane < 16) {
        const int lc = (wn * CF::TN + j) * 16 + lane;
        red[(wm * BN + lc) * 3 + 0] = c;
        red[(wm * BN + lc) * 3 + 1] = mean;
        red[(wm * BN + lc) * 3 + 2] = m2;
      }
    }
    __syncthreads();
    for (int lc = tid; lc < BN; lc += CF::NTH) {
      const int col = n0 + lc;
      if (col < e.N) {
        float n = 0.f, mean = 0.f, m2 = 0.f;
        for (int w = 0; w < CF::WM; ++w) {
          const float nb = red[(w * BN + lc) * 3 + 0], mb = red[(w * BN + lc) * 3 + 1], qb = red[(w * BN + lc) * 3 + 2];
          if (nb > 0.f) {
            const float nn = n + nb, d = mb - mean;
            mean += d * nb / nn;
            m2 += qb + d * d * n * nb / nn;
            n = nn;
          }
        }
        float* o = e.stats + ((int64_t)col * e.stats_tiles + m0 / CF::BM) * 3;
        o[0] = n; o[1] = mean; o[2] = m2;
      }
    }
  }
  static_assert(CF::NTH % (BN / 8) == 0, "a thread's column group must be fixed");
  float cs[8];
#pragma unroll
  for (int j = 0; j < 8; ++j) cs[j] = 0.f;
  constexpr int CGV = BN / 8, IT = SR * CGV / CF::NTH;
  constexpr bool PREB = EV == EV_BIAS || EV == EV_BIAS_RES || EV == EV_BIAS_ACT_PRE;
  constexpr bool PREOP = (EV == EV_BIAS_RES || EV == EV_GATE) && sizeof(T) == 2;
  static_assert(EV == EV_GENERIC || IT * CF::NTH == SR * CGV, "whole vectors per thread per strip");
  const int lc0 = (tid % CGV) * 8;
  float bv[8];
  if constexpr (PREB) {
    if (n0 + lc0 < e.N) ld8(e.bias + n0 + lc0, bv);
  }
#pragma unroll
  for (int i = 0; i < CF::FM; ++i) {
    bf16x8 pre[PREOP ? IT : 1];
    if constexpr (PREOP) {
#pragma unroll
      for (int it = 0; it < IT; ++it) {
        const int lr = (tid + it * CF::NTH) / CGV;
        const int row = m0 + ((lr >> 5) * CF::FM + i) * 32 + (lr & 31);
        if (row < e.M && n0 + lc0 < e.N) {
          const int orow = epi_row(e, row);
          pre[it] = EV == EV_GATE ? *(const bf16x8*)((const bf16*)e.gate + (int64_t)orow * e.ldc + n0 + lc0)
                                  : *(const bf16x8*)((const bf16*)e.res + (int64_t)orow * e.ldr + n0 + lc0);
        }
      }
    }
    __syncthreads();
#pragma unroll
    for (int h = 0; h < 2; ++h)
#pragma unroll
      for (int j = 0; j < CF::TN; ++j)
#pragma unroll
        for (int r = 0; r < 4; ++r) {
          const int lr = wm * 32 + h * 16 + 4 * (lane >> 4) + r;
          st[lr * LDR + (wn * CF::TN + j) * 16 + (lane & 15)] = acc[2 * i + h][j][r];
        }
    __syncthreads();
    if constexpr (EV != EV_GENERIC) {
#pragma unroll
      for (int it = 0; it < IT; ++it) {
        const int lr = (tid + it * CF::NTH) / CGV;
        const int row = m0 + ((lr >> 5) * CF::FM + i) * 32 + (lr & 31);
        const int col = n0 + lc0;
        if (row < e.M && col < e.N) {
          const f32x4 v0 = *(const f32x4*)(st + lr * LDR + lc0), v1 = *(const f32x4*)(st + lr * LDR + lc0 + 4);
          float v[8] = {v0[0], v0[1], v0[2], v0[3], v1[0], v1[1], v1[2], v1[3]};
          epi_vec8<T, OutT>(e, epi_row(e, row), col, v, PREB ? bv : nullptr, PREOP ? &pre[it] : nullptr);
          if (e.colsum) {
#pragma unroll
            for (int j = 0; j < 8; ++j) cs[j] += v[j];
          }
        }
      }
    } else
    for (int c = tid; c < SR * BN / 8; c += CF::NTH) {
      const int lr = c / (BN / 8), lc = (c % (BN / 8)) * 8;
      const int row = m0 + ((lr >> 5) * CF::FM + i) * 32 + (lr & 31);
      const int col = n0 + lc;
      if (row < e.M && col < e.N) {
        const f32x4 v0 = *(const f32x4*)(st + lr * LDR + lc), v1 = *(const f32x4*)(st + lr * LDR + lc + 4);
        float v[8] = {v0[0], v0[1], v0[2], v0[3], v1[0], v1[1], v1[2], v1[3]};
        const int orow = epi_row(e, row);
        if (vec && col + 8 <= e.N) {
          epi_vec8<T, OutT>(e, orow, col, v);
          if (e.colsum) {
#pragma unroll
            for (int j = 0; j < 8; ++j) cs[j] += v[j];
          }
        } else {
          epi_elems<T, OutT, 4>(e, orow, col, v);
          if (col + 4 < e.N) epi_elems<T, OutT, 4>(e, orow, col + 4, v + 4);
        }
      }
    }
  }
  if (e.colsum) {
    constexpr int CG = BN / 8, RP = 9;
    __syncthreads();
#pragma unroll
    for (int j = 0; j < 8; ++j) st[tid * RP + j] = cs[j];
    __syncthreads();
    for (int t = tid; t < BN; t += CF::NTH) {
      const int g = t >> 3, j = t & 7;
      float s = 0.f;
      for (int k = g; k < CF::NTH; k += CG) s += st[k * RP + j];
      if (n0 + t < e.N) e.colsum[(int64_t)(m0 / CF::BM) * e.N + n0 + t] = s;
    }
  }
}

struct BnrArgs {
  const bf16* h; const bf16* res;
  const float *scale, *shift, *prelu, *mean, *invstd, *scale2, *shift2, *mean2, *invstd2;
  float* ws;
};

template <class CF, int RES>
AVSR_DEV void epilogue_bnr(const Epi& e, const BnrArgs& b, int m0, int n0, f32x4 (&acc)[CF::TM][CF::TN], char* smem) {
  constexpr int BN = CF::BN, LDR = BN + 4, SR = CF::WM * 32, CG = BN / 8, RP = 33, IT = SR * CG / CF::NTH;
  static_assert(CF::NTH % CG == 0 && (SR * CG) % CF::NTH == 0, "a thread's column group must be fixed");
  static_assert(CF::NTH * RP * 4 <= CF::LDS_BYTES, "partials staging exceeds LDS");
  const int tid = threadIdx.x, lane = tid & 63, wave = tid >> 6;
  const int wm = wave / CF::WN, wn = wave % CF::WN;
  float* st = (float*)smem;
  const int lc = (tid % CG) * 8, col = n0 + lc;
  const bool colok = col < e.N;
  const bool beta = e.beta != 0.f, alpha1 = e.alpha == 1.f;
  float sc[8], sh[8], pw[8], mu[8], is[8], sc2[8], sh2[8], mu2[8], is2[8];
#pragma unroll
  for (int j = 0; j < 8; ++j) {
    const int c = colok ? col + j : 0;
    sc[j] = b.scale[c]; sh[j] = b.shift[c]; pw[j] = b.prelu[c]; mu[j] = b.mean[c]; is[j] = b.invstd[c];
    if constexpr (RES == 2) { sc2[j] = b.scale2[c]; sh2[j] = b.shift2[c]; mu2[j] = b.mean2[c]; is2[j] = b.invstd2[c]; }
  }
  float s0[8], s1[8], s2[8], s3[8];
#pragma unroll
  for (int j = 0; j < 8; ++j) s0[j] = s1[j] = s2[j] = s3[j] = 0.f;
  bf16* C = (bf16*)e.C;
#pragma unroll
  for (int i = 0; i < CF::FM; ++i) {
    bf16x8 ph[IT], pr[IT], pc[IT];
    int64_t off[IT];
    bool ok[IT];
#pragma unroll
    for (int it = 0; it < IT; ++it) {
      const int lr = (tid + it * CF::NTH) / CG;
      const int row = m0 + ((lr >> 5) * CF::FM + i) * 32 + (lr & 31);
      ok[it] = row < e.M && colok;
      off[it] = ok[it] ? (int64_t)epi_row(e, row) * e.ldc + col : 0;
      ph[it] = *(const bf16x8*)(b.h + off[it]);
// ... 88 lines not shown
```

### avsr_amd/csrc/layernorm.hip

```cpp
#include <algorithm>

#include "common.h"

namespace {

struct LnArgs {
  int rows, N; float eps;
  const void* x; int64_t ldx; void* y; int64_t ldy;
  const float* gamma; const float* beta; float* mean; float* rstd;
  const void* dy; int64_t lddy; void* dx; int64_t lddx; const void* dres; int64_t lddres;
  float* dgamma; float* dbeta; float* ws;
  void* g; int64_t ldg; float drop_p; uint64_t seed; bool db;
};

template <typename T, int VPL>
__global__ __launch_bounds__(256) void ln_fwd_kernel(LnArgs a) {
  constexpr int VE = VecW<T>::VE;
  const int row = blockIdx.x * 4 + (threadIdx.x >> 6), lane = threadIdx.x & 63;
  if (row >= a.rows) return;
  const T* x = (const T*)a.x + (int64_t)row * a.ldx;
  float v[VPL][VE];
  float s = 0.f;
#pragma unroll
  for (int i = 0; i < VPL; ++i) {
    const int c = (lane + i * 64) * VE;
    if (c < a.N) ldv(x + c, v[i]);
    else
#pragma unroll
      for (int j = 0; j < VE; ++j) v[i][j] = 0.f;
#pragma unroll
    for (int j = 0; j < VE; ++j) s += v[i][j];
  }
  const float mean = wave_sum(s) / a.N;
  float q = 0.f;
#pragma unroll
  for (int i = 0; i < VPL; ++i) {
    const int c = (lane + i * 64) * VE;
    if (c < a.N)
#pragma unroll
      for (int j = 0; j < VE; ++j) { const float d = v[i][j] - mean; q += d * d; }
  }
  const float rstd = rsqrtf(wave_sum(q) / a.N + a.eps);
  T* y = (T*)a.y + (int64_t)row * a.ldy;
#pragma unroll
  for (int i = 0; i < VPL; ++i) {
    const int c = (lane + i * 64) * VE;
    if (c < a.N) {
      float o[VE];
#pragma unroll
      for (int j = 0; j < VE; ++j) o[j] = (v[i][j] - mean) * rstd * a.gamma[c + j] + a.beta[c + j];
      stv(y + c, o);
    }
  }
  if (lane == 0) { a.mean[row] = mean; a.rstd[row] = rstd; }
}

template <typename T, int VPL, int W, int R>
__global__ __launch_bounds__(64 * W) void ln_bwd_kernel(LnArgs a) {
  constexpr int VE = VecW<T>::VE;
  const int lane = threadIdx.x & 63;
  const int nw = gridDim.x * W;
  float dg[VPL][VE], db[VPL][VE], gm[VPL][VE], gb[VPL][VE];
#pragma unroll
  for (int i = 0; i < VPL; ++i) {
    const int c = (lane + i * 64) * VE;
#pragma unroll
    for (int j = 0; j < VE; ++j) {
      dg[i][j] = 0.f; db[i][j] = 0.f; gb[i][j] = 0.f; gm[i][j] = c < a.N ? a.gamma[c + j] : 0.f;
    }
  }
  for (int row0 = blockIdx.x * W + (threadIdx.x >> 6); row0 < a.rows; row0 += R * nw) {
    float xv[R][VPL][VE], dv[R][VPL][VE], rv[R][VPL][VE];
    float mean[R], rstd[R];
    bool live[R];
#pragma unroll
    for (int u = 0; u < R; ++u) {
      const int row = min(row0 + u * nw, a.rows - 1);
      live[u] = row0 + u * nw < a.rows;
      const T* x = (const T*)a.x + (int64_t)row * a.ldx;
      const T* dy = (const T*)a.dy + (int64_t)row * a.lddy;
      const T* dr = a.dres ? (const T*)a.dres + (int64_t)row * a.lddres : nullptr;
      mean[u] = a.mean[row]; rstd[u] = a.rstd[row];
#pragma unroll
      for (int i = 0; i < VPL; ++i) {
        const int c = min((lane + i * 64) * VE, a.N - VE);
        ldv(x + c, xv[u][i]);
        ldv(dy + c, dv[u][i]);
        if (dr) ldv(dr + c, rv[u][i]);
        else
#pragma unroll
          for (int j = 0; j < VE; ++j) rv[u][i][j] = 0.f;
      }
    }
#pragma unroll
    for (int u = 0; u < R; ++u) {
      float s1 = 0.f, s2 = 0.f;
#pragma unroll
      for (int i = 0; i < VPL; ++i) {
        const bool cok = (lane + i * 64) * VE < a.N && live[u];
#pragma unroll
        for (int j = 0; j < VE; ++j) {
          const float xh = (xv[u][i][j] - mean[u]) * rstd[u];
          const float g = cok ? dv[u][i][j] * gm[i][j] : 0.f;
          s1 += g;
          s2 += g * xh;
          dg[i][j] += cok ? dv[u][i][j] * xh : 0.f;
          db[i][j] += cok ? dv[u][i][j] : 0.f;
          xv[u][i][j] = xh;
          dv[u][i][j] = g;
        }
      }
      s1 = wave_sum(s1) / a.N;
      s2 = wave_sum(s2) / a.N;
      if (live[u]) {
        T* dx = (T*)a.dx + (int64_t)(row0 + u * nw) * a.lddx;
#pragma unroll
        for (int i = 0; i < VPL; ++i) {
          const int c = (lane + i * 64) * VE;
          if (c < a.N) {
            float o[VE];
#pragma unroll
            for (int j = 0; j < VE; ++j) o[j] = rv[u][i][j] + rstd[u] * (dv[u][i][j] - s1 - xv[u][i][j] * s2);
            stv(dx + c, o);
            if (a.g) {
              float d[VE];
#pragma unroll
              for (int j = 0; j < VE; ++j) d[j] = to_f(from_f<T>(o[j]));
              if (a.drop_p > 0.f) {
                const uint64_t i0 = (uint64_t)(row0 + u * nw) * a.N + c;
                if constexpr (VE == 8) drop8(a.drop_p, a.seed, i0, d);
                else {
#pragma unroll
                  for (int j = 0; j < VE; ++j) d[j] *= drop_scale(a.drop_p, a.seed, i0 + j);
                }
              }
#pragma unroll
              for (int j = 0; j < VE; ++j) gb[i][j] += d[j];
              stv((T*)a.g + (int64_t)(row0 + u * nw) * a.ldg + c, d);
            }
          }
        }
      }
    }
  }
  if (!a.dgamma) return;
  extern __shared__ __attribute__((aligned(16))) float red[];
  const int w = threadIdx.x >> 6;
  const int nq = a.db ? 3 : 2;
  for (int q = 0; q < nq; ++q) {
    __syncthreads();
#pragma unroll
    for (int i = 0; i < VPL; ++i) {
      const int c = (lane + i * 64) * VE;
      if (c < a.N) {
        float* dst = red + w * a.N + c;
#pragma unroll
        for (int j = 0; j < VE; j += 4)
          *(f32x4*)(dst + j) = q == 0 ? f32x4{dg[i][j], dg[i][j + 1], dg[i][j + 2], dg[i][j + 3]}
                             : q == 1 ? f32x4{db[i][j], db[i][j + 1], db[i][j + 2], db[i][j + 3]}
                                      : f32x4{gb[i][j], gb[i][j + 1], gb[i][j + 2], gb[i][j + 3]};
      }
    }
    __syncthreads();
    for (int c = threadIdx.x; c < a.N; c += 64 * W) {
      float t = 0.f;
#pragma unroll
      for (int v = 0; v < W; ++v) t += red[v * a.N + c];
      a.ws[((int64_t)blockIdx.x * nq + q) * a.N + c] = t;
    }
  }
}

constexpr int LN_BWD_WAVES = 4, LN_BWD_ROWS = 1;

template <typename T, int VPL>
void ln_launch_vpl(bool bwd, int blocks, hipStream_t st, const LnArgs& a) {
  if (bwd)
    hipLaunchKernelGGL((ln_bwd_kernel<T, VPL, LN_BWD_WAVES, LN_BWD_ROWS>), dim3(blocks), dim3(64 * LN_BWD_WAVES),
                       (size_t)LN_BWD_WAVES * a.N * sizeof(float), st, a);
  else
    hipLaunchKernelGGL((ln_fwd_kernel<T, VPL>), dim3(blocks), dim3(256), 0, st, a);
}

template <typename T>
int ln_launch(const avsr_layernorm_params* p, bool bwd, hipStream_t st) {
  constexpr int VE = VecW<T>::VE;
  LnArgs a;
  a.rows = p->rows; a.N = p->N; a.eps = p->eps;
  a.x = p->x; a.ldx = p->ldx; a.y = p->y; a.ldy = p->ldy; a.gamma = p->gamma; a.beta = p->beta;
  a.mean = p->mean; a.rstd = p->rstd; a.dy = p->dy; a.lddy = p->lddy; a.dx = p->dx; a.lddx = p->lddx;
  a.dres = p->dres; a.lddres = p->lddres; a.dgamma = p->dgamma; a.dbeta = p->dbeta; a.ws = p->ws;
  a.g = bwd ? p->g : nullptr; a.ldg = p->ldg; a.drop_p = p->drop_p; a.seed = p->seed; a.db = bwd && p->db != nullptr;
  if (a.db && (!a.g || !p->dgamma)) return AVSR_E_ARG;
  if (bwd && p->dgamma && (!p->ws || p->N > 2048)) return AVSR_E_ARG;
  const int vpl = (p->N / VE + 63) / 64;
  const int blocks = bwd ? std::min((p->rows + LN_BWD_WAVES - 1) / LN_BWD_WAVES, AVSR_LN_BLOCKS) : (p->rows + 3) / 4;
  if (vpl <= 1) ln_launch_vpl<T, 1>(bwd, blocks, st, a);
  else if (vpl <= 2) ln_launch_vpl<T, 2>(bwd, blocks, st, a);
  else if (vpl <= 4) ln_launch_vpl<T, 4>(bwd, blocks, st, a);
  else if (vpl <= 8) ln_launch_vpl<T, 8>(bwd, blocks, st, a);
  else return AVSR_E_SHAPE;
  AVSR_CHECK_LAUNCH();
  if (!bwd || !p->dgamma) return 0;
  const int nq = a.db ? 3 : 2;
  const int rc = colsum_launch((const float*)p->ws, blocks, (int64_t)nq * p->N, 2 * p->N, p->dgamma, p->N, p->dbeta, st);
  if (rc || !a.db) return rc;
  return colsum_launch((const float*)p->ws + 2 * p->N, blocks, (int64_t)3 * p->N, p->N, p->db, 0, nullptr, st);
}

template <typename T>
int ln_check(const avsr_layernorm_params* p) {
  constexpr int VE = VecW<T>::VE;
  if (p->N % VE || p->ldx % VE || p->ldy % VE) return AVSR_E_ALIGN;
  return 0;
}

int ln_entry(const avsr_layernorm_params* p, bool bwd, void* stream) {
  if (!p) return AVSR_E_ARG;
  return avsr_by_dtype(p->dtype, [&](auto t) -> int {
    using T = decltype(t);
    const int rc = ln_check<T>(p);
    if (rc) return rc;
    if (p->rows == 0) return 0;
    return ln_launch<T>(p, bwd, (hipStream_t)stream);
  });
}

}

extern "C" int avsr_layernorm_fwd(const avsr_layernorm_params* p, void* stream) { return ln_entry(p, false, stream); }
extern "C" int avsr_layernorm_bwd(const avsr_layernorm_params* p, void* stream) { return ln_entry(p, true, stream); }
```

### avsr_amd/engine.py

```python
import math
import os
import random

import numpy as np
import torch

from . import ops
from . import _lib as L
from .arena import Arena

GELU, RELU, NONE = L.ACT_GELU, L.ACT_RELU, L.ACT_NONE
_BN_FUSE = True
_DB_FUSE = True
_COLSUM_DEFER = True
_SIDE_BIAS = True
WGRAD_GROUP = False
SIDE_ORDER = "o,f2,f1,c,q"
ATTN_MASK = True
_CTC_SIDE = True
_STEM_DIRECT = True
_LN_EW_FUSE = True
SIDE_STREAM = True
EARLY_NORM = True
OPT_OVERLAP = True
OPT_OVERLAP_BLOCKS = 128
OPT_CLEAR_IN_UPDATE = True


_STEP_STREAMS = {}


def prioritize_step_stream(device):
    if device.type != "cuda":
        return None
    idx = device.index if device.index is not None else torch.cuda.current_device()
    s = _STEP_STREAMS.get(idx)
    if s is None:
        s = _STEP_STREAMS[idx] = torch.cuda.Stream(device=idx, priority=-1)
    prev = torch.cuda.current_stream(idx)
    if prev != s:
        s.wait_stream(prev)
    torch.cuda.set_stream(s)
    return s


def wgrad_splitk(M, N, K):
    tiles = ((N + 127) // 128) * ((K + 127) // 128)
    if ops.L.get_option("wgrad_dual") == 0:
        return 1 if tiles > 256 else max(1, min(16, 512 // max(tiles, 1), M // 512))
    return 1 if tiles >= 128 else max(1, min(16, 256 // max(tiles, 1), M // 1024))


def _pad8(n):
    return (n + 7) // 8 * 8


class _Plan:
    __slots__ = ("fz", "cut", "enc", "resnet", "dec", "ctc", "dirty")


class _Seeds:

    def __init__(self, base):
        self.base = base & 0xFFFFFFFFFFFF
        self.i = 0

    def next(self):
        self.i += 1
        return self.peek(0)

    def peek(self, k):
        return (self.base * 0x9E3779B97F4A7C15 + (self.i + k) * 0xBF58476D1CE4E5B9) & 0xFFFFFFFFFFFFFFFF


def positional_encoding(L_, d, device):
    pe = torch.zeros(L_, d)
    pos = torch.arange(0, L_, dtype=torch.float32).unsqueeze(1)
    div = torch.exp(torch.arange(0, d, 2, dtype=torch.float32) * -(math.log(10000.0) / d))
    pe[:, 0::2] = torch.sin(pos * div)
    pe[:, 1::2] = torch.cos(pos * div)
    return pe.to(device)


class Engine:
    RES_BLOCKS = [(1, 0, 64, 64, 1), (1, 1, 64, 64, 1), (2, 0, 64, 128, 2), (2, 1, 128, 128, 1),
                  (3, 0, 128, 256, 2), (3, 1, 256, 256, 1), (4, 0, 256, 512, 2), (4, 1, 512, 512, 1)]

    def __init__(self, shell, cfg, device, dtype=torch.bfloat16):
        self.cfg = cfg
        self.device = torch.device(device)
        self.dtype = dtype
        self.D = cfg.hidden_size
        self.H = cfg.num_attention_heads
        self.F = cfg.intermediate_size
        self.nl = cfg.num_hidden_layers
        self.dD = cfg.ddim
        self.dH = cfg.dheads
        self.dF = cfg.dunits
        self.dl = cfg.dlayers
        self.V = cfg.odim
        self.Vp = _pad8(cfg.odim)
        self.G = cfg.num_conv_pos_embedding_groups
        self.PK = cfg.num_conv_pos_embeddings
        assert self.D // self.H == 64 and self.dD // self.dH == 64, "kernels use head dim 64"
        assert cfg.adim == self.D == self.dD, "proj_decoder (adim != ddim) not on the hot path"
        self.layerdrop = float(getattr(cfg, "layerdrop", 0.0) or 0.0)
        self.len_norm = bool(getattr(cfg, "transformer_length_normalized_loss", False))
        if getattr(cfg, "modality_fuse", "concat") not in ("concat", "add"):
            raise ValueError(f"unknown modality_fuse {cfg.modality_fuse!r}")
        self.fuse_add = getattr(cfg, "modality_fuse", "concat") == "add"
        if getattr(cfg, "modality", "av") not in ("av", "audio", "video"):
            raise ValueError(f"unknown modality {cfg.modality!r}")
        self.last_modality = None
        self.force_modality = None
        self.capture = None
        self._pinned = [(None, None)] * 4
        self._pin_next = 0
        self._nbt = None
        self.side = (torch.cuda.Stream(device=self.device)
                     if self.device.type == "cuda" and SIDE_STREAM else None)
        self._side_ev = [torch.cuda.Event() for _ in range(8)] if self.side is not None else []
        self._amask, self._amask_wait = None, False
        self._amask_ev = torch.cuda.Event() if self.side is not None else None
        self._side_i = 0
        self._side_keep = []
        self._side_defer = None
        E = "encoder.encoder.layers"
        groups = []
        for i in range(self.nl):
            a = f"{E}.{i}.attention."
            groups.append([a + "q_proj.weight", a + "k_proj.weight", a + "v_proj.weight"])
            groups.append([a + "q_proj.bias", a + "k_proj.bias", a + "v_proj.bias"])
        for i in range(self.dl):
            s = f"decoder.decoders.{i}.self_attn."
            groups.append([s + "linear_q.weight", s + "linear_k.weight", s + "linear_v.weight"])
            groups.append([s + "linear_q.bias", s + "linear_k.bias", s + "linear_v.bias"])
            c = f"decoder.decoders.{i}.src_attn."
            groups.append([c + "linear_k.weight", c + "linear_v.weight"])
            groups.append([c + "linear_k.bias", c + "linear_v.bias"])
        perms = {}
        for n, p in shell.named_parameters():
            if p.dim() == 4:
                perms[n] = (0, 2, 3, 1)
        self.pc = "encoder.encoder.pos_conv_embed.conv."
        perms[self.pc + "parametrizations.weight.original1"] = (0, 2, 1)
        pad_rows = {"decoder.output_layer.weight": self.Vp, "ctc.ctc_lo.weight": self.Vp,
                    "decoder.output_layer.bias": self.Vp, "ctc.ctc_lo.bias": self.Vp}
        frozen = ["encoder.mask_emb", "encoder.label_embs_concat"]
        stats = []
        for m in shell.modules():
            for k, b in list(m._buffers.items()):
                if b is not None:
                    m._buffers[k] = b.to(self.device)
                    if k in ("running_mean", "running_var") and b.dtype == torch.float32:
                        stats.append((m, k))
        self.bn_flat = torch.empty(sum(m._buffers[k].numel() for m, k in stats), device=self.device)
        o = 0
        for m, k in stats:
            b = m._buffers[k]
            view = self.bn_flat[o:o + b.numel()].view(b.shape)
            view.copy_(b)
            m._buffers[k] = view
            o += b.numel()
        self.arena = Arena(shell, self.device, dtype, fuse_groups=groups, pad_rows=pad_rows, perms=perms, frozen=frozen)
        self.on_grad_ready = None
        self.pre_video_grads = None
        self.before_forward = None
        self.before_backward = None
        self.after_backward = None
        d0, d1 = self.arena.segments["decay"]
        self._layer_decay_off = []
        for i in range(self.nl):
            pre = f"encoder.encoder.layers.{i}."
            offs = [m["off"] for n, m in self.arena.meta.items() if n.startswith(pre) and d0 <= m["off"] < d1]
            self._layer_decay_off.append(min(offs) if offs else d1)
        if self.layerdrop > 0:
            self.arena.ld_ranges = [self.arena.ranges_of(f"encoder.encoder.layers.{i}.") for i in range(self.nl)]
        self._fz = None
        EN = "encoder."
        self._units = ([(EN + "feature_extractor_audio.", EN + "feature_extractor_video."),
                        (EN + "layer_norm.", EN + "post_extract_proj."), (self.pc,)]
                       + [(f"{E}.{i}.",) for i in range(self.nl)] + [(EN + "encoder.layer_norm.",)])
        self.shell = shell
        self.step_count = 0
        self._pe = positional_encoding(max(512, 64), self.dD, self.device)
        self._stem_wp = None

    @staticmethod
    def new_seeds(seed=None):
        return _Seeds(random.getrandbits(48) if seed is None else seed)

    def draw_modality(self, train):
        cfg = self.cfg
        mod = getattr(cfg, "modality", "av")
        if mod == "audio":
            return "video_off"
        if mod == "video":
            return "audio_off"
        if not train:
            return None
        p_modality, p_audio = np.random.random(), np.random.random()
        if p_modality < cfg.modality_dropout:
            return "audio_off" if p_audio < cfg.audio_dropout else "video_off"
        return None

    def ensure_pe(self, L_):
# ... 330 lines not shown
        R = "encoder.feature_extractor_video.resnet."
        hw = ctx["hw_last"]
        fuse = self.dtype == torch.bfloat16 and _BN_FUSE
        blocks = ctx["blocks"]
        dout = self._e(N * hw * hw, 512)
        ops.avgpool_bwd(dfeat, N, hw * hw, 512, dout)
        red = None
        for j in range(len(blocks) - 1, -1, -1):
            blk = blocks[j]
            p, cout, cin = blk["p"], blk["cout"], blk["cin"]
            M2 = blk["h2"].shape[0]
            down = blk["gd"] is not None
            res, rst = (blk["hd"], blk["std"]) if down else (blk["x"], None)
            g2 = dict(dprelu=self.g(p + "relu2.weight"), dgamma=self.g(p + "bn2.weight"), dbeta=self.g(p + "bn2.bias"))
            if down:
                g2.update(dgamma2=self.g(p + "downsample.1.weight"), dbeta2=self.g(p + "downsample.1.bias"))
            if red is None:
                dz2, sums2 = ops.bn_act_bwd_reduce(dout, blk["h2"], blk["st2"], self.arena.master(p + "relu2.weight"),
                                                   res=res, st2=rst, **g2)
            else:
                dz2, sums2 = dout, ops.bn_bwd_finalize(red[0], red[1], cout, **g2)
            dh2 = self._e(M2, cout)
            dhd = self._e(M2, cout) if down else None
            ops.bn_bwd_apply(dz2, blk["h2"], blk["st2"], sums2, dh2, res=res, st2=rst, dh2=dhd)
            if self._live(p + "conv2.weight"):
                self._conv_wgrad(blk["g2"], blk["a1"], dh2, self.g(p + "conv2.weight"))
            da1 = self._e(M2, cout)
            g1 = dict(dprelu=self.g(p + "relu1.weight"), dgamma=self.g(p + "bn1.weight"), dbeta=self.g(p + "bn1.bias"))
            prelu1 = self.arena.master(p + "relu1.weight")
            if fuse:
                ws, tiles = ops.conv_bwd_data_bnr(blk["g2"], dh2, self.w(p + "conv2.weight"), da1, blk["h1"],
                                                  blk["st1"], prelu1)
                dz1, sums1 = da1, ops.bn_bwd_finalize(ws, tiles, cout, **g1)
            else:
                ops.conv_bwd_data(blk["g2"], dh2, self.w(p + "conv2.weight"), da1)
                dz1, sums1 = ops.bn_act_bwd_reduce(da1, blk["h1"], blk["st1"], prelu1, **g1)
            dh1 = self._e(M2, cout)
            ops.bn_bwd_apply(dz1, blk["h1"], blk["st1"], sums1, dh1)
            if self._live(p + "conv1.weight"):
                self._conv_wgrad(blk["g1"], blk["x"], dh1, self.g(p + "conv1.weight"))
            if fuse:
                if j > 0:
                    pb = blocks[j - 1]
                    pdown = pb["gd"] is not None
                    tgt = dict(h=pb["h2"], st=pb["st2"], prelu=self.arena.master(pb["p"] + "relu2.weight"),
                               res=pb["hd"] if pdown else pb["x"], st2=pb["std"] if pdown else None)
                else:
                    tgt = dict(h=ctx["hmax"], st=ctx["st0"], prelu=self.arena.master(R + "frontend3D.2.weight"))
            red = None
            if not down:
                dx = dz2
                if fuse:
                    red = ops.conv_bwd_data_bnr(blk["g1"], dh1, self.w(p + "conv1.weight"), dx, beta=1.0, **tgt)
                else:
                    ops.conv_bwd_data(blk["g1"], dh1, self.w(p + "conv1.weight"), dx, beta=1.0)
            else:
                dx = self._e(blk["x"].shape[0], cin)
                ops.conv_bwd_data(blk["g1"], dh1, self.w(p + "conv1.weight"), dx)
                if self._live(p + "downsample.0.weight"):
                    self._conv_wgrad(blk["gd"], blk["x"], dhd, self.g(p + "downsample.0.weight"))
                if fuse:
                    red = ops.conv_bwd_data_bnr(blk["gd"], dhd, self.w(p + "downsample.0.weight"), dx, beta=1.0, **tgt)
                else:
                    ops.conv_bwd_data(blk["gd"], dhd, self.w(p + "downsample.0.weight"), dx, beta=1.0)
            dout = dx
        dh0 = self._e(N * 44 * 44, 64)
        dzp, sums = ops.stem_pool_bwd_reduce(dout, ctx["hmax"], N, 44, 44, ctx["st0"],
                                             self.arena.master(R + "frontend3D.2.weight"),
                                             dprelu=self.g(R + "frontend3D.2.weight"),
                                             dgamma=self.g(R + "frontend3D.1.weight"),
                                             dbeta=self.g(R + "frontend3D.1.bias"), reduced=red)
        ops.stem_pool_bwd_apply(dzp, ctx["am"], ctx["h0"], N, 44, 44, ctx["st0"], sums, dh0)
        if self._live(R + "frontend3D.0.weight"):
            gp = self._z(64, 7, 7, 8, dtype=torch.float32)
            ops.conv_bwd_weight(ctx["gs"], ctx["xp"], dh0, gp)
            ops.stem_wgrad_unpack(gp, self.g(R + "frontend3D.0.weight"))

    def _ln(self, x, name, eps, save=None):
        y, mean, rstd = ops.layernorm_fwd(x, self.arena.master(name + ".weight"), self.arena.master(name + ".bias"), eps)
        return y, mean, rstd

    def _ln_bwd(self, dy, x, name, mean, rstd, dres=None, dx=None, ew=None):
        if ew is not None and _LN_EW_FUSE:
            g, p, seed, dbn = ew
            return ops.layernorm_bwd(dy, x, self.arena.master(name + ".weight"), mean, rstd, dx=dx, dres=dres,
                                     dgamma=self.g(name + ".weight"), dbeta=self.g(name + ".bias"), g=g, drop_p=p,
                                     seed=seed, db=self.g(dbn))
        out = ops.layernorm_bwd(dy, x, self.arena.master(name + ".weight"), mean, rstd, dx=dx, dres=dres,
                                dgamma=self.g(name + ".weight"), dbeta=self.g(name + ".bias"))
        if ew is not None:
            g, p, seed, dbn = ew
            ops.ew_bwd(out, out=g, drop_p=p, seed=seed, db=self.g(dbn))
        return out

    def encoder_fwd(self, audios, videos, bt, train, save, seeds, modality=None, plan=None):
        cfg = self.cfg
        B, T = bt["B"], bt["T"]
        M, D = B * T, self.D
        EN = "encoder."
        cut = 0 if plan is None else plan.cut
        ctx = {"B": B, "T": T, "modality": modality, "plan": plan}
        draws = [float(torch.rand([])) for _ in range(self.nl)]
        kept = [i for i in range(self.nl) if not (train and draws[i] < self.layerdrop)]
        p_att = cfg.attention_dropout if train else 0.0
        amask = self._attn_masks(B, T, p_att, {i: seeds.peek(3 + 4 * j) for j, i in enumerate(kept)})
        add = self.fuse_add
        fcat = self._e(M, D if add else 2 * D)
        fa = self._e(M, D) if add else fcat[:, :D]
        ain = self._e(M, cfg.audio_feat_dim)
        ops.audio_pack(audios.contiguous(), ain)
        if modality == "audio_off":
            fa.zero_()
        else:
            ops.linear_fwd(ain, self.w(EN + "feature_extractor_audio.proj.weight"),
                           self.arena.master(EN + "feature_extractor_audio.proj.bias"), out=fa)
        feat, vctx = self.video_fwd(videos, train, save and modality != "video_off" and (plan is None or plan.resnet))
        if modality == "video_off":
            if add:
                fcat.copy_(fa)
            else:
                fcat[:, D:].zero_()
        else:
            ops.linear_fwd(feat, self.w(EN + "feature_extractor_video.proj.weight"),
                           self.arena.master(EN + "feature_extractor_video.proj.bias"),
                           res=fa if add and modality != "audio_off" else None, out=fcat if add else fcat[:, D:])
        self.arena.wait_update()
        ln0, m0, r0 = self._ln(fcat, EN + "layer_norm", 1e-5)
        sd_in = seeds.next()
        p_in = cfg.dropout_input if train else 0.0
        if add:
            x = ops.dropout_fwd(ln0, self._e(M, D), p_in, sd_in) if p_in > 0 else ln0.clone()
        else:
            x = ops.linear_fwd(ln0, self.w(EN + "post_extract_proj.weight"),
                               self.arena.master(EN + "post_extract_proj.bias"), drop_p=p_in, seed=sd_in)
        if not bt["full"]:
            ops.mask_rows(x, B, T, bt["lens"])
        klen = None if bt["full"] else bt["lens"]
        pc = self.pc
        v = self.arena.master(pc + "parametrizations.weight.original1")
        gpc = self.arena.master(pc + "parametrizations.weight.original0").reshape(-1)
        norm = self._e(self.PK, dtype=torch.float32)
        wpc = self._e(D, self.PK, D // self.G)
        ops.weightnorm_fwd(v, gpc, norm, wpc)
        geo = ops.ConvGeom(B, T, 1, D // self.G, D // self.G, self.PK, 1, (1, 1), (self.PK // 2, 0), groups=self.G,
                           hout=T, wout=1)
        pre = self._e(M, D)
        y = self._e(M, D)
        ops.conv_fwd(geo, x, wpc, y, bias=self.arena.master(pc + "bias"), act=GELU, preact=pre, res=x)
        sd_pc = seeds.next()
        p_h = cfg.hidden_dropout if train else 0.0
        if p_h > 0:
            ops.dropout_fwd(y, y, p_h, sd_pc)
        if save:
            ctx.update(klen=klen)
            if cut <= 0:
                ctx.update(ain=ain, vctx=vctx, feat=feat)
            if cut <= 1:
                ctx.update(fcat=fcat, ln0=ln0, m0=m0, r0=r0, sd_in=sd_in, p_in=p_in)
            if cut <= 2:
                ctx.update(x_pre=x, geo=geo, wpc=wpc, norm=norm, pre=pre, sd_pc=sd_pc, p_h=p_h)
        x = y
        layers = []
        for i in range(self.nl):
            if i not in kept:
                if save:
                    layers.append(None)
                continue
            x, lc = self._enc_layer_fwd(i, x, B, T, klen, train, save and 3 + i >= cut, seeds, amask.get(i))
            if save:
                layers.append(lc)
        E = "encoder.encoder."
        out, mf, rf = self._ln(x, E + "layer_norm", 1e-5)
        if save:
            ctx.update(layers=layers, x_last=x, mf=mf, rf=rf)
        return out, ctx

    def _attn_masks(self, B, T, p_att, seeds_by_layer):
        H = self.H
        if not (ATTN_MASK and p_att > 0 and self.dtype == torch.bfloat16 and seeds_by_layer
                and B * H * T * ((T + 1) // 2) <= 0xFFFFFFFF):
            return {}
        words = ops.attn_mask_words(B, H, T, T)
        if self._amask is None or self._amask.shape[1] != words:
            self._amask = None
            self._amask = torch.empty(self.nl, words, dtype=torch.int64, device=self.device)
        buf = self._amask

        def run():
            for i, sd in seeds_by_layer.items():
                ops.attn_dropmask(buf[i], B=B, H=H, Lq=T, Lk=T, drop_p=p_att, seed=sd)
        self._on_side(run)
        self._amask_wait = self.side is not None
        if self._amask_wait:
            self._amask_ev.record(self.side)
        return {i: (sd, buf[i]) for i, sd in seeds_by_layer.items()}

    def _enc_layer_fwd(self, i, x, B, T, klen, train, save, seeds, amask=None):
        cfg = self.cfg
        D, H = self.D, self.H
        M = B * T
        p = f"encoder.encoder.layers.{i}."
        a = p + "attention."
        ln1, m1, r1 = self._ln(x, p + "layer_norm", 1e-5)
        wqkv = self.arena.span([a + "q_proj.weight", a + "k_proj.weight", a + "v_proj.weight"])
        bqkv = self.arena.span([a + "q_proj.bias", a + "k_proj.bias", a + "v_proj.bias"], buf="master")
        qkv = ops.linear_fwd(ln1, wqkv, bqkv)
        o = self._e(M, D)
        lse = self._e(B, H, T, dtype=torch.float32)
        sd_att = seeds.next()
        p_att = cfg.attention_dropout if train else 0.0
        mask = None
        if amask is not None:
            assert amask[0] == sd_att, "attention mask seed out of step with the dropout sites"
            mask = amask[1]
            if self._amask_wait:
                torch.cuda.current_stream(self.device).wait_event(self._amask_ev)
                self._amask_wait = False
        ops.attn_fwd(qkv[:, :D], qkv[:, D:2 * D], qkv[:, 2 * D:], o, lse, B=B, H=H, Lq=T, Lk=T, klen=klen,
                     scale=0.125, drop_p=p_att, seed=sd_att, mask=mask)
        sd_o = seeds.next()
        p_h = cfg.hidden_dropout if train else 0.0
        x1 = ops.linear_fwd(o, self.w(a + "out_proj.weight"), self.arena.master(a + "out_proj.bias"), res=x,
                            drop_p=p_h, seed=sd_o)
        ln2, m2, r2 = self._ln(x1, p + "final_layer_norm", 1e-5)
        ff = p + "feed_forward."
        h = self._e(M, self.F)
        sd_a = seeds.next()
        p_a = cfg.activation_dropout if train else 0.0
        act = ops.linear_fwd(ln2, self.w(ff + "intermediate_dense.weight"), self.arena.master(ff + "intermediate_dense.bias"),
                             act=GELU, preact=h, drop_p=p_a, seed=sd_a)
        sd_f = seeds.next()
        x2 = ops.linear_fwd(act, self.w(ff + "output_dense.weight"), self.arena.master(ff + "output_dense.bias"), res=x1,
                            drop_p=p_h, seed=sd_f)
        lc = None
        if save:
            lc = dict(i=i, x=x, ln1=ln1, m1=m1, r1=r1, qkv=qkv, o=o, lse=lse, sd_att=sd_att, p_att=p_att, mask=mask,
                      sd_o=sd_o, p_h=p_h,
                      x1=x1, ln2=ln2, m2=m2, r2=r2, h=h, act=act, sd_a=sd_a, p_a=p_a, sd_f=sd_f)
        return x2, lc

    def _ew_next(self, i, lc, M):
        return (self._e(M, self.D), lc["p_h"], lc["sd_f"], f"encoder.encoder.layers.{i}.feed_forward.output_dense.bias")

    def _enc_layer_bwd(self, i, lc, dx2, B, T, klen, g2=None, lc_prev=None):
        D, H = self.D, self.H
        M = B * T
        p = f"encoder.encoder.layers.{i}."
        a = p + "attention."
        ff = p + "feed_forward."
        if g2 is None:
            g2 = self._e(M, D)
            ops.ew_bwd(dx2, out=g2, drop_p=lc["p_h"], seed=lc["sd_f"], db=self.g(ff + "output_dense.bias"))
        base = len(self._side_defer) if self._side_defer is not None else None
        tags = [] if base is not None else None

        def tag(t):
            if tags is not None and len(self._side_defer) == base + len(tags) + 1:
                tags.append(t)
        if self._live(ff + "output_dense.weight"):
            self._wgrad(g2, lc["act"], self.g(ff + "output_dense.weight"))
        tag("f2")
        dh = ops.linear_dgrad(g2, self.w(ff + "output_dense.weight"), gate=lc["h"], act=GELU, drop_p=lc["p_a"],
                              seed=lc["sd_a"], db=self._fused_db(ff + "intermediate_dense.bias"))
        self._bias_grad(dh, self.g(ff + "intermediate_dense.bias"), fused=True)
        if self._live(ff + "intermediate_dense.weight"):
            self._wgrad(dh, lc["ln2"], self.g(ff + "intermediate_dense.weight"))
        tag("f1")
        dln2 = ops.linear_dgrad(dh, self.w(ff + "intermediate_dense.weight"))
        go = self._e(M, D)
        dx1 = self._ln_bwd(dln2, lc["x1"], p + "final_layer_norm", lc["m2"], lc["r2"], dres=dx2, dx=dx2,
                           ew=(go, lc["p_h"], lc["sd_o"], a + "out_proj.bias"))
        names_b = [a + "q_proj.bias", a + "k_proj.bias", a + "v_proj.bias"]
        names_w = [a + "q_proj.weight", a + "k_proj.weight", a + "v_proj.weight"]
        grouped = WGRAD_GROUP and self._live(*names_w) and self._live(a + "out_proj.weight")
        if not grouped and self._live(a + "out_proj.weight"):
            self._wgrad(go, lc["o"], self.g(a + "out_proj.weight"))
            tag("o")
        do = ops.linear_dgrad(go, self.w(a + "out_proj.weight"))
        qkv = lc["qkv"]
        dqkv = self._e(M, 3 * D)
        dq32 = self._dq32(M, D)
        delta = self._e(B, H, T, dtype=torch.float32)
        db_qkv = self.arena.span(names_b, buf="g")
        ops.attn_bwd(do, qkv[:, :D], qkv[:, D:2 * D], qkv[:, 2 * D:], lc["o"], lc["lse"], dq32, dqkv[:, D:2 * D],
                     dqkv[:, 2 * D:], delta, B=B, H=H, Lq=T, Lk=T, klen=klen, scale=0.125, drop_p=lc["p_att"],
                     seed=lc["sd_att"], dq=None if dq32 is not None else dqkv[:, :D], mask=lc["mask"])
        if dq32 is not None:
            ops.cast(dq32, dqkv[:, :D])
        if self._live(*names_b):
            self._bias_grad_side(dqkv, db_qkv)
        tag("c")
        if grouped:
            dwq, dwo = self.arena.span(names_w, buf="g"), self.g(a + "out_proj.weight")
            o = lc["o"]
            ln1 = lc["ln1"]
            self._on_side(lambda: ops.wgrad_group([(dqkv, ln1, dwq, 1.0), (go, o, dwo, 1.0)]), dqkv, ln1, go, o)
        elif self._live(*names_w):
            self._wgrad(dqkv, lc["ln1"], self.arena.span(names_w, buf="g"))
        tag("q")
        if tags is not None and SIDE_ORDER:
            items = self._side_defer[base:]
            if len(tags) == len(items):
                by = dict(zip(tags, items))
                order = [t for t in SIDE_ORDER.replace(".", ",").split(",") if t in by]
                order += [t for t in tags if t not in order]
                self._side_defer[base:] = [by[t] for t in order]
        dln1 = ops.linear_dgrad(dqkv, self.arena.span(names_w))
        ew = self._ew_next(lc_prev["i"], lc_prev, M) if lc_prev is not None else None
        dx = self._ln_bwd(dln1, lc["x"], p + "layer_norm", lc["m1"], lc["r1"], dres=dx1, dx=dx1, ew=ew)
        return dx, (ew[0] if ew is not None else None)

    def encoder_bwd(self, ctx, dout):
        cfg = self.cfg
        B, T = ctx["B"], ctx["T"]
        M, D = B * T, self.D
        EN = "encoder."
        E = "encoder.encoder."
        plan = ctx.get("plan")
        cut = 0 if plan is None else plan.cut
        layers = ctx["layers"]
        ex = [i for i in range(self.nl) if layers[i] is not None]
        self.arena.ld_touched.update(ex)
        ew = self._ew_next(ex[-1], layers[ex[-1]], M) if ex else None
        dx = self._ln_bwd(dout, ctx["x_last"], E + "layer_norm", ctx["mf"], ctx["rf"], ew=ew)
        g2 = ew[0] if ew is not None else None
        for i in reversed(range(self.nl)):
            if layers[i] is not None:
                j = ex.index(i)
                self._side_layer(True)
                dx, g2 = self._enc_layer_bwd(i, layers[i], dx, B, T, ctx["klen"], g2=g2,
                                             lc_prev=layers[ex[j - 1]] if j > 0 else None)
                self._side_layer(False)
                ops.colsum_flush()
            if self.on_grad_ready is not None:
                self.on_grad_ready(self._layer_decay_off[i])
        if cut > 2:
            return self._encoder_bwd_end()
        pc = self.pc
        if ctx["p_h"] > 0:
            ops.ew_bwd(dx, out=dx, drop_p=ctx["p_h"], seed=ctx["sd_pc"])
        gp = self._e(M, D)
        ops.ew_bwd(dx, out=gp, gate=ctx["pre"], act=GELU, db=self.g(pc + "bias"))
        if self._live(pc + "parametrizations.weight.original1", pc + "parametrizations.weight.original0"):
            dwpc = self._z(D, self.PK, D // self.G, dtype=torch.float32)
            ops.conv_bwd_weight(ctx["geo"], ctx["x_pre"], gp, dwpc)
            ops.weightnorm_bwd(self.arena.master(pc + "parametrizations.weight.original1"),
                               self.arena.master(pc + "parametrizations.weight.original0").reshape(-1), ctx["norm"], dwpc,
                               self.g(pc + "parametrizations.weight.original1"),
                               self.g(pc + "parametrizations.weight.original0").reshape(-1),
                               self._e(self.PK, dtype=torch.float32))
        if cut == 2:
            return self._encoder_bwd_end()
        ops.conv_bwd_data(ctx["geo"], gp, ctx["wpc"], dx, beta=1.0)
        if ctx["klen"] is not None:
# ... 349 lines not shown
```

### avsr_amd/ops.py

```python
import ctypes
import os

import torch

from . import _lib as L

_DT = {torch.float32: L.AVSR_F32, torch.bfloat16: L.AVSR_BF16}

PROBE = {}

SLAB_PAD = 1088


def slab_ws(batch, splitk, M, N):
    return batch * splitk * (M * N + SLAB_PAD)


def dtype_code(t):
    try:
        return _DT[t.dtype]
    except KeyError:
        raise L.AvsrLibError(f"unsupported dtype {t.dtype}")


def _ptr(t):
    return None if t is None else ctypes.c_void_p(t.data_ptr())


_SKINNY_WS = {}
SKINNY_WS = 1 << 19
SKINNY_CNT = 4096
SKINNY_SPLIT = True
SLAB_FUSED_REDUCE = True


def skinny_splits(N, K, dtype=torch.float32):
    code = L.AVSR_BF16 if dtype == torch.bfloat16 else L.AVSR_F32
    return int(L.load().avsr_gemm_skinny_splits(code, int(N), int(K)))


def _norm_dev(device):
    device = torch.device(device)
    return device if device.index is not None else torch.device(device.type, torch.cuda.current_device())


def _skinny_ws(device):
    device = _norm_dev(device)
    key = (device, L.stream_ptr().value)
    ws = _SKINNY_WS.get(key)
    if ws is None:
        if torch.cuda.is_current_stream_capturing():
            raise L.AvsrLibError("few-row GEMM workspace first requested inside a graph capture: call "
                                 "ops.reserve_stream_workspaces() on the capture stream before capturing")
        ws = _SKINNY_WS[key] = torch.zeros(SKINNY_WS + SKINNY_CNT, device=device, dtype=torch.float32)
    return ws


_SLAB_CNT = {}
SLAB_CNT = 4096


def _slab_cnt(device):
    key = (_norm_dev(device), L.stream_ptr().value)
    c = _SLAB_CNT.get(key)
    if c is None:
        if torch.cuda.is_current_stream_capturing():
            raise L.AvsrLibError("slab counters first requested inside a graph capture")
        c = _SLAB_CNT[key] = torch.zeros(SLAB_CNT, device=key[0], dtype=torch.int32)
    return c


def reserve_stream_workspaces(device, dec_attn_floats=0):
    assert not torch.cuda.is_current_stream_capturing()
    device = _norm_dev(device)
    _skinny_ws(device)
    _slab_cnt(device)
    key = (device, L.stream_ptr().value)
    ws = _DA_WS.get(key)
    if dec_attn_floats and (ws is None or ws.numel() < dec_attn_floats):
        _DA_WS[key] = torch.empty(dec_attn_floats, device=device, dtype=torch.float32)


def _pos_stride(pos, rows, per_row):
    assert pos.dtype == torch.int32 and pos.is_contiguous() and pos.numel() >= (rows if per_row else 1)
    return 1 if per_row else 0


def gemm(A, B, C, *, M, N, K, a_kmajor, b_kmajor, lda, ldb, ldc, batch=1,
         strideA=0, strideB=0, strideC=0, alpha=1.0, beta=0.0, bias=None, act=L.ACT_NONE,
         epi_bwd=False, preact=None, res=None, ldr=None, strideR=0, gate=None, drop_p=0.0, seed=0,
         splitk=1, ws=None, db=None, db_ws=None, skinny_split=None, ln_c1=None, ln_eps=0.0, kv=None):
    lib = L.load()
    assert A.is_cuda and B.is_cuda and C.is_cuda
    assert A.dtype == B.dtype, "A/B dtype mismatch"
    dt = dtype_code(A)
    c_f32 = 1 if (C.dtype == torch.float32 and dt == L.AVSR_BF16) else 0
    if not c_f32:
        assert C.dtype == A.dtype
    if bias is not None:
        assert bias.dtype == torch.float32 and bias.is_contiguous()
    for t in (res, preact, gate):
        if t is not None:
            assert t.dtype == A.dtype
    p = L.GemmParams()
    p.M, p.N, p.K, p.batch = M, N, K, batch
    p.dtype, p.a_kmajor, p.b_kmajor, p.c_f32 = dt, int(a_kmajor), int(b_kmajor), c_f32
    p.A, p.lda, p.strideA = A.data_ptr(), lda, strideA
    p.B, p.ldb, p.strideB = B.data_ptr(), ldb, strideB
    p.C, p.ldc, p.strideC = C.data_ptr(), ldc, strideC
    p.alpha, p.beta = alpha, beta
    p.bias = None if bias is None else bias.data_ptr()
    p.act, p.epi_bwd = act, int(epi_bwd)
    p.preact = None if preact is None else preact.data_ptr()
    p.res = None if res is None else res.data_ptr()
    p.ldr = ldc if ldr is None else ldr
    p.strideR = strideR
    p.gate = None if gate is None else gate.data_ptr()
    p.drop_p, p.seed = float(drop_p), int(seed) & 0xFFFFFFFFFFFFFFFF
    p.splitk = int(splitk)
    if ws is not None:
        assert ws.dtype == torch.float32 and ws.numel() >= slab_ws(batch, splitk, M, N)
        p.ws = ws.data_ptr()
    if (SKINNY_SPLIT if skinny_split is None else skinny_split) and M <= 64 and splitk <= 1:
        p.skinny_ws = _skinny_ws(A.device).data_ptr()
    elif ws is not None and splitk > 1 and SLAB_FUSED_REDUCE:
        p.slab_cnt = _slab_cnt(A.device).data_ptr()
    if ln_c1 is not None:
        assert ln_c1.dtype == torch.float32 and ln_c1.numel() >= N and dt == L.AVSR_F32
        p.ln_c1, p.ln_eps = ln_c1.data_ptr(), float(ln_eps)
    if kv is not None:
        kc, vc, pos, rows = kv[:4]
        assert kc.dtype == vc.dtype == torch.float32 and pos.dtype == torch.int32 and dt == L.AVSR_F32
        p.kv_k, p.kv_v, p.kv_pos, p.kv_rows = kc.data_ptr(), vc.data_ptr(), pos.data_ptr(), int(rows)
        p.kv_pos_stride = _pos_stride(pos, M, len(kv) > 4 and bool(kv[4]))
    if db is not None:
        assert db.dtype == torch.float32 and db.numel() >= N and db_ws is not None and db_ws.dtype == torch.float32
        assert db_ws.numel() >= ((M + 63) // 64) * N
        p.db, p.db_ws = db.data_ptr(), db_ws.data_ptr()
    probe = PROBE.get("gemm")
    if probe is not None and probe["match"](M, N, K, a_kmajor, b_kmajor, dt):
        i = len(probe["events"])
        st = probe["stamps"]
        assert 2 * i + 2 <= st.numel(), "probe stamp buffer full"
        p.stamp = st[2 * i:].data_ptr()
        s, e = torch.cuda.Event(enable_timing=True), torch.cuda.Event(enable_timing=True)
        s.record()
        L.check(lib.avsr_gemm(ctypes.byref(p), L.stream_ptr()), "avsr_gemm")
        e.record()
        probe["events"].append((s, e))
        return C
    L.check(lib.avsr_gemm(ctypes.byref(p), L.stream_ptr()), "avsr_gemm")
    return C


def wgrad_group(problems):
    lib = L.load()
    arr = (L.GemmParams * len(problems))()
    for p, (dy, x, dW, alpha) in zip(arr, problems):
        assert dy.dtype == x.dtype == torch.bfloat16 and dW.dtype == torch.float32
        M, N = dy.shape
        K = x.shape[1]
        p.M, p.N, p.K, p.batch = N, K, M, 1
        p.dtype, p.a_kmajor, p.b_kmajor, p.c_f32 = L.AVSR_BF16, 0, 0, 1
        p.A, p.lda = dy.data_ptr(), dy.stride(0)
        p.B, p.ldb = x.data_ptr(), x.stride(0)
        p.C, p.ldc = dW.data_ptr(), dW.stride(0)
        p.alpha, p.beta = float(alpha), 1.0
        p.ldr, p.splitk = dW.stride(0), 1
    L.check(lib.avsr_gemm_wgrad_group(arr, len(problems), L.stream_ptr()), "avsr_gemm_wgrad_group")



def linear_fwd(x, W, bias=None, *, act=L.ACT_NONE, preact=None, res=None, drop_p=0.0, seed=0, out=None,
               skinny_split=None, ln=None, kv=None):
    M, K = x.shape
    N = W.shape[0]
    assert W.shape[1] == K and x.stride(1) == 1 and W.stride(1) == 1
    if out is None:
        out = torch.empty(M, N, device=x.device, dtype=x.dtype)
    gemm(x, W, out, M=M, N=N, K=K, a_kmajor=True, b_kmajor=True, lda=x.stride(0), ldb=W.stride(0),
         ldc=out.stride(0), bias=bias, act=act, preact=preact, res=res,
         ldr=None if res is None else res.stride(0), drop_p=drop_p, seed=seed, skinny_split=skinny_split,
         ln_c1=None if ln is None else ln[0], ln_eps=0.0 if ln is None else ln[1], kv=kv)
    return out


def fold_layernorm(W, b, gamma, beta):
    Wg = (W * gamma.unsqueeze(0)).contiguous()
    bb = (W.double() @ beta.double() + (0 if b is None else b.double())).float()
    c1 = Wg.double().sum(1).float()
    return Wg, bb, c1


def linear_dgrad(dy, W, *, gate=None, act=L.ACT_NONE, drop_p=0.0, seed=0, out=None, beta=0.0, db=None):
    M, N = dy.shape
    K = W.shape[1]
    if out is None:
        out = torch.empty(M, K, device=dy.device, dtype=dy.dtype)
    fused = (db is not None and dy.dtype == torch.bfloat16 and M >= 128 and K >= 128 and K % 8 == 0
             and out.stride(0) % 8 == 0)
    ws = _colsum_ws(((M + 63) // 64) * K, dy.device) if fused else None
    gemm(dy, W, out, M=M, N=K, K=N, a_kmajor=True, b_kmajor=False, lda=dy.stride(0), ldb=W.stride(0),
         ldc=out.stride(0), epi_bwd=True, gate=gate, act=act, drop_p=drop_p, seed=seed, beta=beta,
         db=db if fused else None, db_ws=ws)
    if db is not None and not fused:
        ew_bwd(out, db=db)
    return out


def linear_wgrad(dy, x, dW, *, beta=0.0):
    M, N = dy.shape
    K = x.shape[1]
    assert dW.shape == (N, K) and dW.dtype == torch.float32
    gemm(dy, x, dW, M=N, N=K, K=M, a_kmajor=False, b_kmajor=False, lda=dy.stride(0), ldb=x.stride(0),
         ldc=dW.stride(0), beta=beta)
    return dW



class ConvGeom:

    def __init__(self, nimg, hin, win, cin, cout, kh, kw, stride=(1, 1), pad=(0, 0), groups=1,
                 hout=None, wout=None, ldx=None, ldy=None):
        self.nimg, self.hin, self.win, self.cin, self.cout = nimg, hin, win, cin, cout
        self.kh, self.kw = kh, kw
        self.sh, self.sw = stride
        self.ph, self.pw = pad
        self.groups = groups
        self.hout = hout if hout is not None else (hin + 2 * self.ph - kh) // self.sh + 1
        self.wout = wout if wout is not None else (win + 2 * self.pw - kw) // self.sw + 1
        self.ldx = ldx if ldx is not None else groups * cin
        self.ldy = ldy if ldy is not None else groups * cout

    def params(self, dtype):
        p = L.ConvParams()
        p.dtype = dtype
        p.nimg, p.hin, p.win, p.cin = self.nimg, self.hin, self.win, self.cin
        p.hout, p.wout, p.cout = self.hout, self.wout, self.cout
        p.kh, p.kw, p.sh, p.sw, p.ph, p.pw = self.kh, self.kw, self.sh, self.sw, self.ph, self.pw
        p.groups, p.ldx, p.ldy = self.groups, self.ldx, self.ldy
        p.alpha, p.beta = 1.0, 0.0
        return p

    @property
    def out_pixels(self):
        return self.nimg * self.hout * self.wout

    @property
    def in_pixels(self):
        return self.nimg * self.hin * self.win


def conv_stat_tiles(g, dtype):
    p = g.params(dtype)
    return L.load().avsr_conv_stat_tiles(ctypes.byref(p))


def conv_path(g, dtype, pass_, *, bias=False, act=L.ACT_NONE, preact=False, res=False, ws=False, splitk=0):
    p = g.params(_DT.get(dtype, dtype))
    p.act, p.splitk = act, splitk
    for name, on in (("bias", bias), ("preact", preact), ("res", res), ("ws", ws)):
        setattr(p, name, 16 if on else None)
    rc = L.load().avsr_conv_path(ctypes.byref(p), L.CONV_PASSES.index(pass_))
    if not 0 <= rc < len(L.CONV_PATHS):
        L.check(rc, "avsr_conv_path")
    return L.CONV_PATHS[rc]
# ... 5 lines not shown
    if stats is not None:
        tiles = L.load().avsr_conv_stat_tiles(ctypes.byref(p))
        if stats.dtype != torch.float32 or stats.numel() < g.groups * g.cout * tiles * 3 or not stats.is_contiguous():
            raise ValueError(f"conv_fwd stats: need fp32 [{g.cout}, {tiles}, 3], got {tuple(stats.shape)}")
    p.x, p.w, p.y = x.data_ptr(), w.data_ptr(), y.data_ptr()
    p.stats = None if stats is None else stats.data_ptr()
    p.bias = None if bias is None else bias.data_ptr()
    p.act = act
    p.preact = None if preact is None else preact.data_ptr()
    p.res = None if res is None else res.data_ptr()
    p._keep = [t for t in (x, w, y, stats, bias, preact, res) if t is not None]
    L.check(L.load().avsr_conv_fwd(ctypes.byref(p), L.stream_ptr()), "avsr_conv_fwd")
    return y


def conv_bwd_data(g, dy, w, dx, alpha=1.0, beta=0.0):
    p = g.params(dtype_code(dy))
    assert dy.dtype == w.dtype == dx.dtype
    p.dy, p.w, p.dx = dy.data_ptr(), w.data_ptr(), dx.data_ptr()
    p.alpha, p.beta = alpha, beta
    L.check(L.load().avsr_conv_bwd_data(ctypes.byref(p), L.stream_ptr()), "avsr_conv_bwd_data")
    return dx


def bn_fin_ws(tiles, C):
    return (tiles + ((tiles + 15) // 16 if tiles > 256 else 0)) * 4 * C


def conv_bwd_data_bnr(g, dy, w, dx, h, st, prelu, *, res=None, st2=None, alpha=1.0, beta=0.0):
    p = g.params(dtype_code(dy))
    assert dy.dtype == w.dtype == dx.dtype == h.dtype == torch.bfloat16
    lib = L.load()
    tiles = lib.avsr_conv_bnr_tiles(ctypes.byref(p))
    ws = torch.empty(bn_fin_ws(tiles, g.cin), device=dx.device)
    p.dy, p.w, p.dx = dy.data_ptr(), w.data_ptr(), dx.data_ptr()
    p.alpha, p.beta = alpha, beta
    p.bnr_h, p.bnr_res = h.data_ptr(), None if res is None else res.data_ptr()
    p.bnr_scale, p.bnr_shift, p.bnr_prelu = st.scale.data_ptr(), st.shift.data_ptr(), prelu.data_ptr()
    p.bnr_mean, p.bnr_invstd = st.mean.data_ptr(), st.invstd.data_ptr()
    if st2 is not None:
        p.bnr_scale2, p.bnr_shift2 = st2.scale.data_ptr(), st2.shift.data_ptr()
        p.bnr_mean2, p.bnr_invstd2 = st2.mean.data_ptr(), st2.invstd.data_ptr()
    p.bnr_ws = ws.data_ptr()
    L.check(lib.avsr_conv_bwd_data(ctypes.byref(p), L.stream_ptr()), "avsr_conv_bwd_data(bnr)")
    return ws, tiles


_WGRAD_SLAB = True


def conv_bwd_weight(g, x, dy, dw, splitk=0, slab=None):
    p = g.params(dtype_code(x))
    assert x.dtype == dy.dtype and dw.dtype == torch.float32
    p.x, p.dy, p.dw = x.data_ptr(), dy.data_ptr(), dw.data_ptr()
    p.splitk = splitk
    lib = L.load()
    ws = None
    if _WGRAD_SLAB if slab is None else slab:
        n = lib.avsr_conv_wgrad_ws(ctypes.byref(p))
        if n > 0:
            ws = torch.empty(n, device=dw.device, dtype=torch.float32)
            p.ws = ws.data_ptr()
    L.check(lib.avsr_conv_bwd_weight(ctypes.byref(p), L.stream_ptr()), "avsr_conv_bwd_weight")
    return dw


def _call(name, params):
    L.check(getattr(L.load(), name)(ctypes.byref(params), L.stream_ptr()), name)



def layernorm_fwd(x, gamma, beta, eps, y=None, mean=None, rstd=None):
    rows, N = x.shape
    y = torch.empty_like(x) if y is None else y
    mean = torch.empty(rows, device=x.device) if mean is None else mean
    rstd = torch.empty(rows, device=x.device) if rstd is None else rstd
    _call("avsr_layernorm_fwd", L.fill(L.LayerNormParams, dtype=dtype_code(x), rows=rows, N=N, eps=eps,
                                        x=x, ldx=x.stride(0), y=y, ldy=y.stride(0), gamma=gamma, beta=beta,
                                        mean=mean, rstd=rstd))
    return y, mean, rstd


def layernorm_bwd(dy, x, gamma, mean, rstd, dx=None, dres=None, dgamma=None, dbeta=None, g=None, drop_p=0.0, seed=0,
                  db=None):
    rows, N = x.shape
    dx = torch.empty_like(x) if dx is None else dx
    if db is not None:
        assert g is not None and dgamma is not None
    ws = None if dgamma is None else _colsum_ws(256 * (3 if db is not None else 2) * N, x.device)
    _call("avsr_layernorm_bwd", L.fill(L.LayerNormParams, dtype=dtype_code(x), rows=rows, N=N, eps=0.0,
                                        x=x, ldx=x.stride(0), ldy=N, gamma=gamma, mean=mean, rstd=rstd,
                                        dy=dy, lddy=dy.stride(0), dx=dx, lddx=dx.stride(0),
                                        dres=dres, lddres=0 if dres is None else dres.stride(0),
                                        dgamma=dgamma, dbeta=dbeta, ws=ws, g=g, ldg=0 if g is None else g.stride(0),
                                        drop_p=float(drop_p), seed=int(seed) & (2 ** 64 - 1), db=db))
    return dx



class BnState:

    def __init__(self, C, device):
        buf = torch.empty(4, C, device=device)
        self.mean, self.invstd, self.scale, self.shift = buf[0], buf[1], buf[2], buf[3]


def bn_finalize(st, gamma, beta, running_mean, running_var, *, partials=None, training=True,
                momentum=0.1, eps=1e-5):
    C = gamma.shape[0]
    tiles = 0 if partials is None else partials.shape[1]
    _call("avsr_bn_finalize", L.fill(L.BnFinalizeParams, tiles=tiles, C=C, partials=partials, gamma=gamma,
                                      beta=beta, running_mean=running_mean, running_var=running_var,
                                      momentum=momentum, eps=eps, training=int(training), mean=st.mean,
                                      invstd=st.invstd, scale=st.scale, shift=st.shift))
    return st


def bn_act_fwd(h, st, prelu, y, res=None, st2=None):
    M, C = h.shape
    _call("avsr_bn_act_fwd", L.fill(L.BnActParams, dtype=dtype_code(h), M=M, C=C, h=h, scale=st.scale,
                                     shift=st.shift, res=res, scale2=None if st2 is None else st2.scale,
                                     shift2=None if st2 is None else st2.shift, prelu=prelu, y=y))
    return y


def _bn_params(h, st, *, M=None, res=None, st2=None, **kw):
    M = h.shape[0] if M is None else M
    C = h.shape[-1]
    return L.fill(L.BnActParams, dtype=dtype_code(h), M=M, C=C, h=h, scale=st.scale, shift=st.shift, res=res,
                  scale2=None if st2 is None else st2.scale, shift2=None if st2 is None else st2.shift,
                  mean=st.mean, invstd=st.invstd, mean2=None if st2 is None else st2.mean,
                  invstd2=None if st2 is None else st2.invstd, **kw)


def bn_act_bwd_reduce(dy, h, st, prelu, *, res=None, st2=None, dz=None, sums=None, dprelu=None, dgamma=None,
                      dbeta=None, dgamma2=None, dbeta2=None):
    C = h.shape[-1]
    dz = torch.empty_like(h) if dz is None else dz
    sums = torch.empty(C, 3, device=h.device) if sums is None else sums
    ws = torch.empty(bn_fin_ws(2048, C), device=h.device)
    _call("avsr_bn_act_bwd_reduce", _bn_params(h, st, res=res, st2=st2, ws=ws, prelu=prelu, dy=dy, dz=dz, sums=sums,
                                               dprelu=dprelu, dgamma=dgamma, dbeta=dbeta, dgamma2=dgamma2,
                                               dbeta2=dbeta2))
    return dz, sums


def bn_bwd_finalize(ws, tiles, C, *, sums=None, dprelu=None, dgamma=None, dbeta=None, dgamma2=None, dbeta2=None):
    sums = torch.empty(C, 3, device=ws.device) if sums is None else sums
    p = L.fill(L.BnActParams, C=C, ws=ws, sums=sums, dprelu=dprelu, dgamma=dgamma, dbeta=dbeta, dgamma2=dgamma2,
               dbeta2=dbeta2)
    L.check(L.load().avsr_bn_bwd_finalize(ctypes.byref(p), tiles, L.stream_ptr()), "avsr_bn_bwd_finalize")
    return sums


def bn_bwd_apply(dz, h, st, sums, dh, *, res=None, st2=None, dh2=None, beta_acc=0.0):
    _call("avsr_bn_bwd_apply", _bn_params(h, st, res=res, st2=st2, dz=dz, sums=sums, dh=dh, dh2=dh2,
                                          beta_acc=beta_acc))
    return dh


def bn_act_bwd(dy, h, st, prelu, dh, *, res=None, st2=None, dh2=None, dz=None, sums=None,
               dprelu=None, dgamma=None, dbeta=None, dgamma2=None, dbeta2=None, beta_acc=0.0):
    dz, sums = bn_act_bwd_reduce(dy, h, st, prelu, res=res, st2=st2, dz=dz, sums=sums, dprelu=dprelu,
                                 dgamma=dgamma, dbeta=dbeta, dgamma2=dgamma2, dbeta2=dbeta2)
    bn_bwd_apply(dz, h, st, sums, dh, res=res, st2=st2, dh2=dh2, beta_acc=beta_acc)
    return dz


def stem_pool_fwd(h, nimg, H, W, st, prelu, y, argmax, hmax=None):
    C = h.shape[-1]
    _call("avsr_stem_pool_fwd", L.fill(L.StemPoolParams, dtype=dtype_code(h), nimg=nimg, H=H, W=W, C=C,
                                        Ho=(H + 1) // 2, Wo=(W + 1) // 2, h=h, scale=st.scale, shift=st.shift,
                                        prelu=prelu, y=y, argmax=argmax, hmax=hmax))
    return y


def stem_pool_bwd(dy, argmax, hmax, h, nimg, H, W, st, prelu, dh, *, dzp=None, sums=None, dprelu=None,
                  dgamma=None, dbeta=None, reduced=None):
# ... 149 lines not shown
        ws = torch.empty(max(4, ctc_align_ws(B, T, Lmax)), device=dev, dtype=torch.uint8)
    _call("avsr_ctc_align", L.fill(L.CtcAlignParams, dtype=dtype_code(x), B=B, T=T, V=V, Lmax=Lmax, blank=blank,
                                    x=x, ldx=x.stride(0), lse=lse, labels=labels, label_len=label_len,
                                    in_len=in_len, ws=ws, ali=ali, score=score, feasible=feasible))
    return ali, score, feasible


def token_logp(x, V, target, out=None, lse=None):
    rows = x.shape[0]
    if out is None:
        out = torch.empty(rows, device=x.device, dtype=torch.float32)
    if lse is None:
        lse = torch.empty(rows, device=x.device, dtype=torch.float32)
    lsm_fwd(x, V, target, 0.0, lse, out, None)
    return out.neg_()


CTC_BEAM_MAX = 16
CTC_BEAM_LCAP = 511


def ctc_beam_ws(U, Tm, N):
    return U * (Tm * N + 1) * 8


def ctc_beam(logp, tlen, cand, N, *, blank, eos, Lcap=None, ws=None):
    U, Tm, V = logp.shape
    C = cand.shape[-1]
    if logp.dtype != torch.float32 or cand.dtype != torch.int32 or tlen.dtype != torch.int32:
        raise TypeError("ctc_beam: logp fp32, cand and tlen int32")
    if logp.stride(2) != 1 or logp.stride(0) != Tm * logp.stride(1) or not cand.is_contiguous() \
            or tuple(cand.shape[:2]) != (U, Tm) or tlen.numel() != U:
        raise ValueError("ctc_beam: logp rows u*Tm + t, cand (U, Tm, C) contiguous, tlen (U,)")
    if Lcap is None:
        Lcap = min(Tm, CTC_BEAM_LCAP)
    dev = logp.device
    inside = 1 <= N <= CTC_BEAM_MAX and 0 <= Lcap <= CTC_BEAM_LCAP
    n_out = torch.empty(U, device=dev, dtype=torch.int32)
    tokens = torch.empty(U, N, Lcap, device=dev, dtype=torch.int32) if inside else None
    length = torch.empty(U, N, device=dev, dtype=torch.int32) if inside else n_out
    score = torch.empty(U, N, device=dev, dtype=torch.float32) if inside else n_out
    if ws is None:
        ws = torch.empty(max(1, ctc_beam_ws(U, Tm, N) // 8) if inside else 1, device=dev, dtype=torch.int64)
    _call("avsr_ctc_beam", L.fill(L.CtcBeamParams, U=U, Tm=Tm, V=V, N=N, C=C, blank=blank, eos=eos, Lcap=Lcap,
                                   logp=logp, ldp=logp.stride(1), tlen=tlen, cand=cand, ws=ws, n_out=n_out,
                                   tokens=tokens, len=length, score=score))
    return n_out, tokens, length, score


def loss_finalize(B, nll, row_loss, row_correct, mtlalpha, out, att_per_token=False):
    L.check(L.load().avsr_loss_finalize(B, nll.data_ptr(), row_loss.shape[0], row_loss.data_ptr(),
                                        _p(row_correct), mtlalpha, int(bool(att_per_token)), out.data_ptr(),
                                        L.stream_ptr()),
            "avsr_loss_finalize")
    return out



_COLSUM = {"on": False, "keep": []}


def _colsum_ws(n, device):
    ws = torch.empty(n, device=device)
    if _COLSUM["on"]:
        _COLSUM["keep"].append(ws)
    return ws


def colsum_defer(on):
    prev = _COLSUM["on"]
    L.load().avsr_colsum_defer(int(bool(on)))
    _COLSUM["on"] = bool(on)
    if not on:
        _COLSUM["keep"].clear()
    return prev


def colsum_flush():
    if _COLSUM["on"] or _COLSUM["keep"]:
        L.check(L.load().avsr_colsum_flush(L.stream_ptr()), "avsr_colsum_flush")
        _COLSUM["keep"].clear()


def ew_bwd(dy, *, out=None, gate=None, act=L.ACT_NONE, drop_p=0.0, seed=0, alpha=1.0, db=None, inline=False):
    rows, N = dy.shape
    lib = L.load()
    if inline and db is not None:
        ws = torch.empty(256 * N, device=dy.device)
        prev = lib.avsr_colsum_inline(1)
    else:
        ws = None if db is None else _colsum_ws(256 * N, dy.device)
    try:
        _call("avsr_ew_bwd", L.fill(L.EwParams, dtype=dtype_code(dy), rows=rows, N=N, dy=dy, lddy=dy.stride(0),
                                     ws=ws, out=out, ldout=0 if out is None else out.stride(0), gate=gate,
                                     ldgate=0 if gate is None else gate.stride(0), act=act, drop_p=float(drop_p),
                                     seed=int(seed) & (2 ** 64 - 1), alpha=alpha, db=db))
    finally:
        if inline and db is not None:
            lib.avsr_colsum_inline(prev)
    return out


def dropout_fwd(x, out, p, seed):
    rows, N = x.shape
    _call("avsr_dropout_fwd", L.fill(L.EwParams, dtype=dtype_code(x), rows=rows, N=N, dy=x, lddy=x.stride(0),
                                      out=out, ldout=out.stride(0), drop_p=float(p),
                                      seed=int(seed) & (2 ** 64 - 1), alpha=1.0))
    return out


def mask_rows(x, B, T, lengths):
    L.check(L.load().avsr_mask_rows(dtype_code(x), B, T, x.shape[1], x.data_ptr(), x.stride(0),
                                    lengths.data_ptr(), L.stream_ptr()), "avsr_mask_rows")
    return x


def embed_fwd(tok, table, pe, scale, y, L_, drop_p=0.0, seed=0, pe_row=None, per_row=False):
    _call("avsr_embed_fwd", L.fill(L.EmbedParams, dtype=dtype_code(table), rows=tok.shape[0], L=L_,
                                    D=table.shape[1], tok=tok, table=table, pe=pe, scale=scale, y=y,
                                    drop_p=float(drop_p), seed=int(seed) & (2 ** 64 - 1), pe_row=pe_row,
                                    pe_row_stride=0 if pe_row is None else _pos_stride(pe_row, tok.shape[0], per_row)))
    return y


def embed_bwd(tok, dy, scale, dtable, L_, drop_p=0.0, seed=0):
    _call("avsr_embed_bwd", L.fill(L.EmbedParams, dtype=dtype_code(dy), rows=tok.shape[0], L=L_,
                                    D=dy.shape[1], tok=tok, scale=scale, dy=dy, dtable=dtable,
                                    drop_p=float(drop_p), seed=int(seed) & (2 ** 64 - 1)))


def cast(src, dst, alpha=1.0, beta=0.0):
    rows, cols = src.shape
    assert dst.shape == src.shape
    L.check(L.load().avsr_cast(dtype_code(src), dtype_code(dst), rows, cols, src.data_ptr(), src.stride(0),
                               dst.data_ptr(), dst.stride(0), alpha, beta, L.stream_ptr()), "avsr_cast")
    return dst


def cast_flat(src, dst):
    assert src.is_contiguous() and dst.is_contiguous() and src.numel() == dst.numel()
    L.check(L.load().avsr_cast_flat(dtype_code(src), dtype_code(dst), src.numel(), src.data_ptr(), dst.data_ptr(),
                                    L.stream_ptr()), "avsr_cast_flat")
    return dst


def stem_pack(videos, out):
    B, _, T = videos.shape[:3]
    assert videos.dtype == torch.float32 and videos.is_contiguous()
    L.check(L.load().avsr_stem_pack(dtype_code(out), B, T, videos.data_ptr(), out.data_ptr(), L.stream_ptr()),
            "avsr_stem_pack")
    return out


def stem_wpack(w, wp):
    L.check(L.load().avsr_stem_wpack(dtype_code(wp), w.data_ptr(), wp.data_ptr(), L.stream_ptr()), "avsr_stem_wpack")
    return wp


STEM_K = 288
STEM_DIRECT_MAX_BYTES = 0x7fffffff


def stem_wpack2(w, wk):
    assert w.dtype == torch.float32 and w.numel() == 64 * 245 and w.is_contiguous()
    assert wk.dtype == torch.bfloat16 and wk.numel() == 64 * STEM_K
    L.check(L.load().avsr_stem_wpack2(w.data_ptr(), wk.data_ptr(), L.stream_ptr()), "avsr_stem_wpack2")
    return wk


def stem_conv_tiles(B, T):
    return L.load().avsr_stem_conv_tiles(int(B), int(T))


def stem_conv_fwd(videos, wk, h, stats=None):
    B, _, T = videos.shape[:3]
    assert videos.dtype == torch.float32 and videos.is_contiguous() and tuple(videos.shape[3:]) == (88, 88)
    assert h.dtype == torch.bfloat16 and h.numel() == B * T * 44 * 44 * 64 and h.is_contiguous()
    if stats is not None:
        assert stats.dtype == torch.float32 and stats.numel() >= 64 * stem_conv_tiles(B, T) * 3
    L.check(L.load().avsr_stem_conv_fwd(B, T, videos.data_ptr(), wk.data_ptr(), h.data_ptr(),
                                        None if stats is None else stats.data_ptr(), L.stream_ptr()),
            "avsr_stem_conv_fwd")
    return h


def stem_wgrad_unpack(gp, gw):
    L.check(L.load().avsr_stem_wgrad_unpack(gp.data_ptr(), gw.data_ptr(), L.stream_ptr()), "avsr_stem_wgrad_unpack")


def audio_pack(audios, out):
    B, F, T = audios.shape
# ... 198 lines not shown
```

### include/avsr_hip.h

```cpp
#ifndef AVSR_HIP_H
#define AVSR_HIP_H

#include <stdint.h>

#ifdef __cplusplus
extern "C" {
#endif

enum { AVSR_F32 = 0, AVSR_BF16 = 1 };
enum { AVSR_ACT_NONE = 0, AVSR_ACT_GELU = 1, AVSR_ACT_RELU = 2 };
enum { AVSR_E_SHAPE = 1001, AVSR_E_ALIGN = 1002, AVSR_E_DTYPE = 1003, AVSR_E_ARG = 1004 };

const char* avsr_version(void);

enum {
  AVSR_OPT_GEMM_TILE = 0,
  AVSR_OPT_ATTN_SQ_FWD = 1,
  AVSR_OPT_ATTN_SQ_BWD = 2,
  AVSR_OPT_WGRAD_DUAL = 3,
  AVSR_OPT_CONV_192 = 4,
  AVSR_OPT_CONV_S2PHASE = 5,
  AVSR_OPT_CONV_PATCH = 6,
  AVSR_OPT_CONV_WPATCH = 7,
  AVSR_OPT_STEM_POOL_2X2 = 8,
  AVSR_OPT_STEM_WPATCH = 9,
  AVSR_OPT_ATTN_ENC_FUSED = 10,
  AVSR_OPT_COUNT = 11
};
enum {
  AVSR_TILE_128 = 0, AVSR_TILE_256 = 1, AVSR_TILE_256x128 = 2, AVSR_TILE_128x256 = 3, AVSR_TILE_128s3 = 4,
  AVSR_TILE_128w8s3 = 5, AVSR_TILE_PP = 6, AVSR_TILE_192 = 7, AVSR_TILE_192x256 = 8, AVSR_TILE_192w8s3 = 9,
  AVSR_TILE_64 = 10, AVSR_TILE_64s4 = 11, AVSR_TILE_COUNT = 12
};
int avsr_set_option(int option, int64_t value);
int64_t avsr_get_option(int option);

typedef struct {
  int M, N, K, batch;
  int dtype;
  int a_kmajor, b_kmajor;
  int c_f32;
  const void* A; int64_t lda, strideA;
  const void* B; int64_t ldb, strideB;
  void* C;       int64_t ldc, strideC;
  float alpha, beta;
  const float* bias;
  int act;
  int epi_bwd;
  void* preact;
  const void* res;  int64_t ldr, strideR;
  const void* gate;
  float drop_p;
  uint64_t seed;
  int splitk;
  float* ws;
  float* db;
  float* db_ws;
  unsigned long long* stamp;
  float* skinny_ws;
  const float* ln_c1;
  float ln_eps;
  void* kv_k;
  void* kv_v;
  const int* kv_pos;
  int kv_rows;
  unsigned* slab_cnt;
  int kv_pos_stride;
} avsr_gemm_params;
#define AVSR_GEMM_COLSUM_WS(M, N) ((int64_t)(((M) + 63) / 64) * (N))
#define AVSR_GEMM_SLAB_PAD 1088
#define AVSR_SKINNY_WS (1 << 19)
#define AVSR_SKINNY_CNT 4096
#define AVSR_SLAB_CNT 4096
#define AVSR_SKINNY_WS_BYTES ((int64_t)AVSR_SKINNY_WS * 4 + AVSR_SKINNY_CNT * 4)
#define AVSR_GEMM_SLAB_WS(batch, splitk, M, N) ((int64_t)(batch) * (splitk) * ((int64_t)(M) * (N) + AVSR_GEMM_SLAB_PAD))

int avsr_gemm(const avsr_gemm_params* p, void* stream);
int avsr_gemm_wgrad_group(const avsr_gemm_params* p, int n, void* stream);
int avsr_gemm_skinny_splits(int dtype, int N, int K);

typedef struct {
  int dtype;
  int nimg, hin, win, cin;
  int hout, wout, cout;
  int kh, kw, sh, sw, ph, pw;
  int groups;
  int64_t ldx, ldy;
  const void* x; const void* w; void* y;
  void* dx; const void* dy; float* dw;
  float* stats;
  float alpha, beta;
  int splitk;
  const float* bias; int act; void* preact; const void* res;
  float* ws;
  const void* bnr_h; const void* bnr_res;
  const float* bnr_scale; const float* bnr_shift; const float* bnr_prelu;
  const float* bnr_mean; const float* bnr_invstd;
  const float* bnr_scale2; const float* bnr_shift2; const float* bnr_mean2; const float* bnr_invstd2;
  float* bnr_ws;
} avsr_conv_params;

int avsr_conv_fwd(const avsr_conv_params* p, void* stream);
int avsr_conv_bwd_data(const avsr_conv_params* p, void* stream);
int avsr_conv_bwd_weight(const avsr_conv_params* p, void* stream);
int avsr_conv_stat_tiles(const avsr_conv_params* p);
int avsr_conv_bnr_tiles(const avsr_conv_params* p);
int64_t avsr_conv_wgrad_ws(const avsr_conv_params* p);
enum { AVSR_CONV_FWD = 0, AVSR_CONV_DGRAD = 1, AVSR_CONV_WGRAD = 2 };
enum {
  AVSR_CONV_PATH_REG = 0, AVSR_CONV_PATH_GLDS = 1, AVSR_CONV_PATH_PATCH = 2, AVSR_CONV_PATH_S2 = 3,
  AVSR_CONV_PATH_WPATCH = 4, AVSR_CONV_PATH_STEM_WPATCH = 5
};
int avsr_conv_path(const avsr_conv_params* p, int pass);

typedef struct {
  int dtype, rows, N;
  float eps;
  const void* x; int64_t ldx;
  void* y; int64_t ldy;
  const float* gamma; const float* beta;
  float* mean; float* rstd;
  const void* dy; int64_t lddy;
  void* dx; int64_t lddx;
  const void* dres; int64_t lddres;
  float* dgamma; float* dbeta;
  float* ws;
  void* g; int64_t ldg; float drop_p; uint64_t seed; float* db;
} avsr_layernorm_params;
#define AVSR_LN_BLOCKS 256
#define AVSR_LN_WS(N) (AVSR_LN_BLOCKS * 2 * (N))
#define AVSR_LN_WS3(N) (AVSR_LN_BLOCKS * 3 * (N))
int avsr_layernorm_fwd(const avsr_layernorm_params* p, void* stream);
int avsr_layernorm_bwd(const avsr_layernorm_params* p, void* stream);

typedef struct {
  int tiles, C;
  const float* partials;
  const float* gamma; const float* beta;
  float* running_mean; float* running_var;
  float momentum, eps;
  int training;
  float* mean; float* invstd; float* scale; float* shift;
} avsr_bn_finalize_params;
int avsr_bn_finalize(const avsr_bn_finalize_params* p, void* stream);

typedef struct {
  int dtype, M, C;
  const void* h;
  const float* scale; const float* shift;
  const void* res;
  const float* scale2; const float* shift2;
  const float* prelu;
  void* y;
  const void* dy; void* dz;
  const float* mean; const float* invstd;
  const float* mean2; const float* invstd2;
  float* sums;
  float* dprelu;
  float* dgamma; float* dbeta; float* dgamma2; float* dbeta2;
  void* dh; void* dh2; float beta_acc;
  float* ws;
} avsr_bn_act_params;
#define AVSR_BN_FIN_WS(tiles, C) (((int64_t)(tiles) + ((tiles) > 256 ? ((tiles) + 15) / 16 : 0)) * 4 * (C))
#define AVSR_BN_WS(C) AVSR_BN_FIN_WS(2048, C)
int avsr_bn_act_fwd(const avsr_bn_act_params* p, void* stream);
int avsr_bn_act_bwd_reduce(const avsr_bn_act_params* p, void* stream);
int avsr_bn_bwd_finalize(const avsr_bn_act_params* p, int tiles, void* stream);
int avsr_bn_bwd_apply(const avsr_bn_act_params* p, void* stream);

typedef struct {
  int dtype, nimg, H, W, C, Ho, Wo;
  const void* h; const float* scale; const float* shift; const float* prelu;
  void* y; uint8_t* argmax;
  const void* dy; void* dz;
  const float* mean; const float* invstd;
  float* sums; float* dprelu; float* dgamma; float* dbeta;
  float* ws;
  void* hmax;
  void* dh;
  int64_t m_total;
} avsr_stem_pool_params;
int avsr_stem_pool_fwd(const avsr_stem_pool_params* p, void* stream);
int avsr_stem_pool_bwd_apply(const avsr_stem_pool_params* p, void* stream);

int avsr_avgpool_fwd(int dtype, int nimg, int P, int C, const void* x, void* y, void* stream);
int avsr_avgpool_bwd(int dtype, int nimg, int P, int C, const void* dy, void* dx, void* stream);

typedef struct {
  int dtype, B, H, Lq, Lk;
  float scale;
  const void* q; int64_t ldq;
  const void* k; int64_t ldk;
  const void* v; int64_t ldv;
  void* o; int64_t ldo;
  float* lse;
  const int* klen;
  int causal;
  float drop_p; uint64_t seed;
  const void* dout; int64_t lddo;
  float* delta;
  float* dq; int64_t lddq;
  void* dk; int64_t lddk;
  void* dv; int64_t lddv;
  void* dq_out; int64_t lddq_out;
  float* db; float* db_ws;
  uint64_t* drop_mask;
} avsr_attn_params;
#define AVSR_ATTN_DB_WS(B, H) ((int64_t)(B) * 3 * (H) * 64)
#define AVSR_ATTN_MASK_WORDS(B, H, Lq, Lk) \
  ((int64_t)(B) * (H) * (((Lq) + 31) / 32) * (2 * (((Lk) + 63) / 64)) * 16)
int avsr_debug_attn_stamps(unsigned long long* buf);
int avsr_attn_fwd(const avsr_attn_params* p, void* stream);
int avsr_attn_bwd_prep(const avsr_attn_params* p, void* stream);
int avsr_attn_bwd(const avsr_attn_params* p, void* stream);
enum { AVSR_ATTN_FWD = 0, AVSR_ATTN_BWD = 1 };
enum {
  AVSR_ATTN_PATH_F32 = 0, AVSR_ATTN_PATH_TILED = 1, AVSR_ATTN_PATH_RESIDENT = 2, AVSR_ATTN_PATH_SQ = 3,
  AVSR_ATTN_PATH_ENC = 4
};
int avsr_attn_path(const avsr_attn_params* p, int pass);
int avsr_attn_dropmask(const avsr_attn_params* p, void* stream);

typedef struct {
  int dtype, rows, V;
  const void* x; int64_t ldx;
  const int* target;
  float smoothing;
  float* lse; float* row_loss; int* row_correct;
  const float* dloss; float coef;
  void* dx; int64_t lddx;
} avsr_xent_params;
int avsr_row_lse(const avsr_xent_params* p, void* stream);
int avsr_lsm_fwd(const avsr_xent_params* p, void* stream);
int avsr_lsm_bwd(const avsr_xent_params* p, void* stream);

typedef struct {
  int dtype, B, T, V, Lmax;
  const void* x; int64_t ldx;
  const float* lse;
  const int* labels;
  const int* label_len; const int* in_len;
  float* alpha; float* gamma;
  float* nll;
  const float* dloss; float coef;
  void* dx; int64_t lddx;
} avsr_ctc_params;
int avsr_ctc_fwd(const avsr_ctc_params* p, void* stream);
int avsr_ctc_bwd(const avsr_ctc_params* p, void* stream);

int avsr_loss_finalize(int B, const float* nll, int rows, const float* row_loss, const int* row_correct,
                       float mtlalpha, int att_per_token, float* out, void* stream);

typedef struct {
  int dtype, B, T, V, Lmax, blank;
  const void* x; int64_t ldx;
  const float* lse;
  const int* labels;
  const int* label_len; const int* in_len;
  unsigned char* ws;
  int* ali;
  float* score;
  int* feasible;
} avsr_ctc_align_params;
#define AVSR_CTC_ALIGN_WS(B, T, Lmax) (((int64_t)(B) * (T) * (2 * (int64_t)(Lmax) + 1) + 3) & ~(int64_t)3)
int avsr_ctc_align(const avsr_ctc_align_params* p, void* stream);

typedef struct {
  int U, Tm, V, N, C, blank, eos, Lcap;
  const float* logp; int64_t ldp;
  const int* tlen;
  const int* cand;
  void* ws;
  int* n_out;
  int* tokens;
  int* len;
  float* score;
} avsr_ctc_beam_params;
#define AVSR_CTC_BEAM_WS(U, Tm, N) ((int64_t)(U) * ((int64_t)(Tm) * (N) + 1) * 8)
int avsr_ctc_beam(const avsr_ctc_beam_params* p, void* stream);

typedef struct {
  int dtype, rows, N;
  const void* dy; int64_t lddy;
  void* out; int64_t ldout;
  const void* gate; int64_t ldgate; int act;
  float drop_p; uint64_t seed;
  float alpha;
  float* db;
  float* ws;
} avsr_ew_params;
#define AVSR_EW_ROWBLOCKS 256
#define AVSR_EW_WS(N) (AVSR_EW_ROWBLOCKS * (N))
int avsr_ew_bwd(const avsr_ew_params* p, void* stream);
int avsr_colsum_defer(int on);
int avsr_colsum_flush(void* stream);
int avsr_colsum_inline(int on);
int avsr_dropout_fwd(const avsr_ew_params* p, void* stream);
int avsr_mask_rows(int dtype, int B, int T, int N, void* x, int64_t ldx, const int* len, void* stream);

typedef struct {
  int dtype, rows, L, D;
  const int* tok; const void* table; const float* pe; float scale;
  void* y; float drop_p; uint64_t seed;
  const void* dy; float* dtable;
  const int* pe_row;
  int pe_row_stride;
} avsr_embed_params;
int avsr_embed_fwd(const avsr_embed_params* p, void* stream);
int avsr_embed_bwd(const avsr_embed_params* p, void* stream);

int avsr_cast(int src_dtype, int dst_dtype, int rows, int cols, const void* src, int64_t lds,
              void* dst, int64_t ldd, float alpha, float beta, void* stream);
int avsr_cast_flat(int src_dtype, int dst_dtype, int64_t n, const void* src, void* dst, void* stream);
int avsr_stem_pack(int dtype, int B, int T, const float* video, void* out, void* stream);
int avsr_stem_wpack(int dtype, const float* w, void* wp, void* stream);
int avsr_stem_conv_tiles(int B, int T);
int avsr_stem_wpack2(const float* w, void* wk, void* stream);
int avsr_stem_conv_fwd(int B, int T, const float* video, const void* wk, void* h, float* stats, void* stream);
int avsr_stem_wgrad_unpack(const float* gp, float* gw, void* stream);
int avsr_audio_pack(int dtype, int B, int F, int T, const float* audio, void* out, void* stream);

int avsr_weightnorm_fwd(int dtype, int O, int K, int C, const float* v, const float* g, float* norm,
                        void* w, void* stream);
int avsr_weightnorm_bwd(int O, int K, int C, const float* v, const float* g, const float* norm,
                        const float* dw, float* dv, float* dg, float* scratch, void* stream);

#define AVSR_SUMSQ_WS 1024
int avsr_sumsq(const float* x, int64_t n, float* out, float* ws, void* stream);
typedef struct {
  int64_t n;
  float* param; const float* grad; float* exp_avg; float* exp_avg_sq;
  void* shadow; int shadow_dtype;
  float lr, beta1, beta2, eps, weight_decay;
  float bias_corr1, bias_corr2;
  const float* sumsq; float max_norm;
  float grad_scale;
  int max_blocks;
  float* grad_clear;
} avsr_adamw_params;
int avsr_adamw(const avsr_adamw_params* p, void* stream);

int avsr_log_softmax_rows(int dtype, int rows, int V, const void* x, int64_t ldx, float* out, int64_t ldo,
                          void* stream);

typedef struct {
  int dtype, n, H, klen_max;
  float scale;
  const void* q; int64_t ldq;
  const void* k; int64_t ldk, k_bstride;
  const void* v; int64_t ldv, v_bstride;
  const int* klen;
  void* o; int64_t ldo;
  const int* kidx;
  const int* kmap; int64_t ldmap;
  int group;
  int ksplit;
  float* ws;
  unsigned* cnt;
} avsr_dec_attn_params;
int avsr_dec_attn(const avsr_dec_attn_params* p, void* stream);

typedef struct {
  int rows, V, K;
  const float* x; int64_t ldx;
  int* ids;
} avsr_topk_params;
int avsr_row_topk(const avsr_topk_params* p, void* stream);
int avsr_log_softmax_topk(int dtype, int rows, int V, const void* x, int64_t ldx, float* out, int64_t ldo,
                          int K, int* ids, void* stream);

typedef struct {
  int n, T, V, P;
  int blank, eos, out_len;
  const float* logp;
  const float* r_prev;
  const int* last;
  const int* ids;
  float* r_new;
  float* psi;
  const int* uidx; int64_t logp_ustride; const int* tlen;
// ... 160 lines not shown
```

Baseline: 147,400.

## Precompute hidden-dropout bitmasks on side stream and consume them in epilogues

Adds a batched kernel that writes packed 1-bit hidden-dropout keep masks for many dropout sites from their seeds. It is presumably launched on the side stream and synchronised through an event. The GEMM residual epilogue, layernorm backward and elementwise backward read mask bits instead of recomputing the hash per element. This takes hashing off the critical path in forward and backward, at the cost of extra mask memory, extra reads, and a cross-stream dependency.

```diff
diff --git a/avsr_amd/_lib.py b/avsr_amd/_lib.py
--- a/avsr_amd/_lib.py
+++ b/avsr_amd/_lib.py
@@ -38,6 +38,7 @@
         ("skinny_ws", _c_p), ("ln_c1", _c_p), ("ln_eps", ctypes.c_float),
         ("kv_k", _c_p), ("kv_v", _c_p), ("kv_pos", _c_p), ("kv_rows", _i),
         ("slab_cnt", _c_p), ("kv_pos_stride", _i),
+        ("drop_mask", _c_p),
     ]
 
 
@@ -70,6 +71,7 @@
         ("dy", _c_p), ("lddy", _i64), ("dx", _c_p), ("lddx", _i64),
         ("dres", _c_p), ("lddres", _i64), ("dgamma", _c_p), ("dbeta", _c_p), ("ws", _c_p),
         ("g", _c_p), ("ldg", _i64), ("drop_p", _f), ("seed", ctypes.c_uint64), ("db", _c_p),
+        ("drop_mask", _c_p),
     ]
 
 
@@ -151,7 +153,7 @@
     _fields_ = [
         ("dtype", _i), ("rows", _i), ("N", _i), ("dy", _c_p), ("lddy", _i64), ("out", _c_p), ("ldout", _i64),
         ("gate", _c_p), ("ldgate", _i64), ("act", _i), ("drop_p", _f), ("seed", ctypes.c_uint64),
-        ("alpha", _f), ("db", _c_p), ("ws", _c_p),
+        ("alpha", _f), ("db", _c_p), ("ws", _c_p), ("drop_mask", _c_p),
     ]
 
 
@@ -343,6 +345,7 @@
     "avsr_colsum_flush": ([_c_p], _i),
     "avsr_colsum_inline": ([_i], _i),
     "avsr_dropout_fwd": ([ctypes.POINTER(EwParams), _c_p], _i),
+    "avsr_drop_mask": ([_i, ctypes.POINTER(ctypes.c_uint64), ctypes.POINTER(_c_p), _i, _i, _f, _c_p], _i),
     "avsr_mask_rows": ([_i, _i, _i, _i, _c_p, _i64, _c_p, _c_p], _i),
     "avsr_embed_fwd": ([ctypes.POINTER(EmbedParams), _c_p], _i),
     "avsr_embed_bwd": ([ctypes.POINTER(EmbedParams), _c_p], _i),
diff --git a/avsr_amd/csrc/common.h b/avsr_amd/csrc/common.h
--- a/avsr_amd/csrc/common.h
+++ b/avsr_amd/csrc/common.h
@@ -65,29 +65,45 @@
 AVSR_DEV float drop_keep_scale(uint32_t thr) { return thr < 65536u ? 65536.f / (float)(65536u - thr) : 0.f; }
 AVSR_DEV uint32_t drop_half(uint32_t h, bool odd) { return odd ? (h >> 16) : (h & 0xFFFFu); }
 
+AVSR_DEV bool drop_keep(uint32_t thr, uint64_t seed, uint64_t idx) {
+  return drop_half(mix32(seed, idx >> 1), idx & 1) >= thr;
+}
 AVSR_DEV float drop_scale(float p, uint64_t seed, uint64_t idx) {
   const uint32_t thr = drop_thr16(p);
-  return drop_half(mix32(seed, idx >> 1), idx & 1) >= thr ? drop_keep_scale(thr) : 0.0f;
-}
-
-AVSR_DEV void drop8(float p, uint64_t seed, uint64_t d0, float* v) {
+  return drop_keep(thr, seed, idx) ? drop_keep_scale(thr) : 0.0f;
+}
+
+AVSR_DEV uint32_t drop_keep8(float p, uint64_t seed, uint64_t d0) {
   const uint32_t thr = drop_thr16(p);
-  const float ks = drop_keep_scale(thr);
   const uint64_t p0 = d0 >> 1;
   const uint32_t lo = (uint32_t)p0;
+  uint32_t bits = 0;
   if (!(d0 & 1) && lo <= 0xFFFFFFFCu) {
     const uint32_t pre = mix32_hi(seed, (uint32_t)(p0 >> 32));
     const uint32_t g0 = lo * 0x9E3779B1u;
 #pragma unroll
     for (int q = 0; q < 4; ++q) {
       const uint32_t h = fmix32((g0 + (uint32_t)q * 0x9E3779B1u) ^ pre);
-      v[2 * q] *= (h & 0xFFFFu) >= thr ? ks : 0.0f;
-      v[2 * q + 1] *= (h >> 16) >= thr ? ks : 0.0f;
+      bits |= ((h & 0xFFFFu) >= thr ? 1u : 0u) << (2 * q);
+      bits |= ((h >> 16) >= thr ? 1u : 0u) << (2 * q + 1);
     }
   } else {
 #pragma unroll
-    for (int q = 0; q < 8; ++q) v[q] *= drop_scale(p, seed, d0 + q);
-  }
+    for (int q = 0; q < 8; ++q) bits |= (drop_keep(thr, seed, d0 + q) ? 1u : 0u) << q;
+  }
+  return bits;
+}
+template <int NE> AVSR_DEV void drop_apply_bits(uint32_t bits, float ks, float* v) {
+#pragma unroll
+  for (int q = 0; q < NE; ++q) v[q] *= (bits >> q) & 1u ? ks : 0.0f;
+}
+AVSR_DEV void drop8(float p, uint64_t seed, uint64_t d0, float* v) {
+  drop_apply_bits<8>(drop_keep8(p, seed, d0), drop_keep_scale(drop_thr16(p)), v);
+}
+template <int NE> AVSR_DEV uint32_t drop_mask_bits(const uint8_t* mask, uint64_t i0) {
+  static_assert(NE == 4 || NE == 8, "a byte or a nibble");
+  const uint32_t b = mask[i0 >> 3];
+  return NE == 8 ? b : (b >> (uint32_t)(i0 & 4)) & 0xFu;
 }
 
 AVSR_DEV float gelu_erf(float x) { return 0.5f * x * (1.0f + erff(x * 0.70710678118654752f)); }
diff --git a/avsr_amd/csrc/elementwise.hip b/avsr_amd/csrc/elementwise.hip
--- a/avsr_amd/csrc/elementwise.hip
+++ b/avsr_amd/csrc/elementwise.hip
@@ -7,6 +7,7 @@
   const void* dy; int64_t lddy; void* out; int64_t ldout;
   const void* gate; int64_t ldgate; int act;
   float drop_p; uint64_t seed; float alpha; float* db; float* ws;
+  const uint8_t* mask;
 };
 
 template <typename T>
@@ -30,7 +31,8 @@
       for (int j = 0; j < VE; ++j) d[j] *= a.alpha;
       if (a.drop_p > 0.f) {
         const uint64_t i0 = (uint64_t)r * a.N + cv * VE;
-        if constexpr (VE == 8) drop8(a.drop_p, a.seed, i0, d);
+        if (a.mask) drop_apply_bits<VE>(drop_mask_bits<VE>(a.mask, i0), drop_keep_scale(drop_thr16(a.drop_p)), d);
+        else if constexpr (VE == 8) drop8(a.drop_p, a.seed, i0, d);
         else {
 #pragma unroll
           for (int j = 0; j < VE; ++j) d[j] *= drop_scale(a.drop_p, a.seed, i0 + j);
@@ -185,9 +187,39 @@
   }
 }
 
+constexpr int DROP_MASK_SITES = 64;
+struct DropMaskArgs {
+  uint64_t seed[DROP_MASK_SITES];
+  uint8_t* out[DROP_MASK_SITES];
+  int64_t bytes;
+  float p;
+};
+
+__global__ __launch_bounds__(256) void drop_mask_kernel(DropMaskArgs a) {
+  const uint64_t seed = a.seed[blockIdx.y];
+  uint8_t* out = a.out[blockIdx.y];
+  const int64_t chunks = (a.bytes + 15) / 16;
+  for (int64_t c = (int64_t)blockIdx.x * 256 + threadIdx.x; c < chunks; c += (int64_t)gridDim.x * 256) {
+    const int64_t b0 = c * 16;
+    if (b0 + 16 <= a.bytes) {
+      uint32_t w[4];
+#pragma unroll
+      for (int j = 0; j < 4; ++j) {
+        w[j] = 0;
+#pragma unroll
+        for (int k = 0; k < 4; ++k) w[j] |= drop_keep8(a.p, seed, (uint64_t)(b0 + 4 * j + k) * 8) << (8 * k);
+      }
+      *(v16*)(out + b0) = v16{{w[0], w[1], w[2], w[3]}};
+    } else {
+      for (int64_t b = b0; b < a.bytes; ++b) out[b] = (uint8_t)drop_keep8(a.p, seed, (uint64_t)b * 8);
+    }
+  }
+}
+
 template <typename T>
 int ew_launch(const avsr_ew_params* p, hipStream_t st) {
   constexpr int VE = VecW<T>::VE;
+  if (p->drop_mask && (p->N % 8)) return AVSR_E_ARG;
   if (p->N % VE) return AVSR_E_SHAPE;
   if (p->rows == 0) return 0;
   if (p->db && !p->ws) return AVSR_E_ARG;
@@ -201,6 +233,7 @@
   a.rows = p->rows; a.N = p->N; a.dy = p->dy; a.lddy = p->lddy; a.out = p->out; a.ldout = p->ldout;
   a.gate = p->gate; a.ldgate = p->ldgate; a.act = p->act; a.drop_p = p->drop_p; a.seed = p->seed;
   a.alpha = p->alpha; a.db = p->db; a.ws = p->ws;
+  a.mask = p->drop_p > 0.f ? (const uint8_t*)p->drop_mask : nullptr;
   hipLaunchKernelGGL(ew_bwd_kernel<T>, grid, dim3(256), 0, st, a);
   AVSR_CHECK_LAUNCH();
   if (p->db) return colsum_launch((const float*)p->ws, (int)grid.y, (int64_t)p->N, p->N, p->db, 0, nullptr, st);
@@ -236,6 +269,26 @@
     q.gate = nullptr; q.db = nullptr;
     return ew_launch<decltype(t)>(&q, (hipStream_t)stream);
   });
+}
+
+extern "C" int avsr_drop_mask(int k, const uint64_t* seeds, void* const* masks, int rows, int N, float drop_p,
+                              void* stream) {
+  if (k < 0 || rows < 0 || N < 0 || (k > 0 && (!seeds || !masks))) return AVSR_E_ARG;
+  if (N % 8) return AVSR_E_ARG;
+  for (int i = 0; i < k; ++i)
+    if (!masks[i] || !avsr_aligned16(masks[i])) return AVSR_E_ALIGN;
+  const int64_t bytes = (int64_t)rows * N / 8;
+  if (k == 0 || bytes == 0) return 0;
+  for (int i0 = 0; i0 < k; i0 += DROP_MASK_SITES) {
+    const int n = k - i0 < DROP_MASK_SITES ? k - i0 : DROP_MASK_SITES;
+    DropMaskArgs a{};
+    for (int i = 0; i < n; ++i) { a.seed[i] = seeds[i0 + i]; a.out[i] = (uint8_t*)masks[i0 + i]; }
+    a.bytes = bytes; a.p = drop_p;
+    hipLaunchKernelGGL(drop_mask_kernel, dim3(avsr_grid((bytes + 15) / 16, 256, 256), n), dim3(256), 0,
+                       (hipStream_t)stream, a);
+    AVSR_CHECK_LAUNCH();
+  }
+  return 0;
 }
 
 extern "C" int avsr_mask_rows(int dtype, int B, int T, int N, void* x, int64_t ldx, const int* len, void* stream) {
diff --git a/avsr_amd/csrc/gemm.hip b/avsr_amd/csrc/gemm.hip
--- a/avsr_amd/csrc/gemm.hip
+++ b/avsr_amd/csrc/gemm.hip
@@ -100,6 +100,7 @@
   if (batch > 1 && (((a.sC * so) | (a.sC * 2) | (a.sR * 2)) & 15)) return EV_GENERIC;
   if (a.splits > 1 && ((a.sSplit * so) & 15)) return EV_GENERIC;
   const bool drop = e.drop_p > 0.f;
+  if (e.drop_mask && (e.bwd || e.preact || e.act || !e.res)) return EV_GENERIC;
   if (!e.bwd) {
     if (e.gate || e.colsum) return EV_GENERIC;
     if (!e.bias) return (!e.preact && !e.act && !e.res && !drop) ? EV_PLAIN : EV_GENERIC;
@@ -289,6 +290,7 @@
                 (p->preact && !avsr_aligned16(p->preact)) || (p->res && (!avsr_aligned16(p->res) || (p->ldr % 8))) ||
                 (p->bias && !avsr_aligned16(p->bias))))
     return AVSR_E_ARG;
+  if (p->drop_mask && p->drop_p > 0.f && ((p->N % 8) || p->batch != 1 || splits > 1)) return AVSR_E_ARG;
   if (p->K == 0) return AVSR_E_SHAPE;
   if (p->ln_c1 && !skinny) return AVSR_E_ARG;
   return 0;
@@ -333,6 +335,7 @@
   }
   e.preact = p->preact; e.res = p->res; e.ldr = p->ldr; e.gate = p->gate;
   e.drop_p = p->drop_p; e.seed = p->seed;
+  e.drop_mask = p->drop_p > 0.f ? (const uint8_t*)p->drop_mask : nullptr;
   e.colsum = p->db ? p->db_ws : nullptr;
   return a;
 }
diff --git a/avsr_amd/csrc/gemm_core.h b/avsr_amd/csrc/gemm_core.h
--- a/avsr_amd/csrc/gemm_core.h
+++ b/avsr_amd/csrc/gemm_core.h
@@ -282,7 +282,13 @@
   int stats_tiles;
   int rm_wc, rm_hc, rm_hin, rm_win, rm_a, rm_b;
   float* colsum;
-};
+  const uint8_t* drop_mask;
+};
+
+AVSR_DEV float epi_drop_scale(const Epi& e, uint64_t didx) {
+  if (e.drop_mask) return (e.drop_mask[didx >> 3] >> (uint32_t)(didx & 7)) & 1u ? drop_keep_scale(drop_thr16(e.drop_p)) : 0.0f;
+  return drop_scale(e.drop_p, e.seed, didx);
+}
 
 AVSR_DEV int epi_row(const Epi& e, int r) {
   if (e.rm_wc == 0) return r;
@@ -316,10 +322,10 @@
       if (e.bias) v += e.bias[col + q];
       if (P) P[off + q] = from_f<T>(v);
       v = act_fwd_t<T>(e.act, v);
-      if (e.drop_p > 0.f) v *= drop_scale(e.drop_p, e.seed, didx);
+      if (e.drop_p > 0.f) v *= epi_drop_scale(e, didx);
       if (R) v += to_f(R[(int64_t)row * e.ldr + col + q]);
     } else {
-      if (e.drop_p > 0.f) v *= drop_scale(e.drop_p, e.seed, didx);
+      if (e.drop_p > 0.f) v *= epi_drop_scale(e, didx);
       if (G) v *= act_bwd_t<T>(e.act, to_f(G[off + q]));
     }
     if (e.beta != 0.f) v += e.beta * to_f(C[off + q]);
@@ -373,18 +379,23 @@
     else e.gate = nullptr;
     e.act = (EV == EV_BIAS_ACT_PRE || EV == EV_GATE) ? AVSR_ACT_GELU : AVSR_ACT_NONE;
     if constexpr (EV == EV_PLAIN || EV == EV_BIAS) e.drop_p = 0.f;
+    if constexpr (EV != EV_BIAS_RES) e.drop_mask = nullptr;
     if constexpr (EV != EV_GATE) e.colsum = nullptr;
   }
 }
 
 template <typename T, typename OutT>
 AVSR_DEV void epi_vec8(const Epi& e, int row, int col, float (&v)[8], const float* bv = nullptr,
-                       const bf16x8* op = nullptr) {
+                       const bf16x8* op = nullptr, uint32_t mbits = 0) {
   const int64_t off = (int64_t)row * e.ldc + col;
 #pragma unroll
   for (int q = 0; q < 8; ++q) v[q] *= e.alpha;
   float t[8];
   const uint64_t d0 = e.drop_base + (uint64_t)row * (uint64_t)e.N + col;
+  auto drop = [&](float (&x)[8]) {
+    if (e.drop_mask) drop_apply_bits<8>(op ? mbits : drop_mask_bits<8>(e.drop_mask, d0), drop_keep_scale(drop_thr16(e.drop_p)), x);
+    else drop8(e.drop_p, e.seed, d0, x);
+  };
   if (!e.bwd) {
     if (e.bias) {
       if (bv) {
@@ -409,7 +420,7 @@
         for (int q = 0; q < 8; ++q) v[q] = act_fwd_t<T>(e.act, v[q]);
       }
     }
-    if (e.drop_p > 0.f) drop8(e.drop_p, e.seed, d0, v);
+    if (e.drop_p > 0.f) drop(v);
     if (e.res) {
       if (op) {
 #pragma unroll
@@ -421,7 +432,7 @@
       for (int q = 0; q < 8; ++q) v[q] += t[q];
     }
   } else {
-    if (e.drop_p > 0.f) drop8(e.drop_p, e.seed, d0, v);
+    if (e.drop_p > 0.f) drop(v);
     if (e.gate) {
       if (op) {
 #pragma unroll
diff --git a/avsr_amd/csrc/gemm_glds.h b/avsr_amd/csrc/gemm_glds.h
--- a/avsr_amd/csrc/gemm_glds.h
+++ b/avsr_amd/csrc/gemm_glds.h
@@ -325,6 +325,7 @@
 #pragma unroll
   for (int i = 0; i < CF::FM; ++i) {
     bf16x8 pre[PREOP ? IT : 1];
+    uint32_t prem[PREOP ? IT : 1];
     if constexpr (PREOP) {
 #pragma unroll
       for (int it = 0; it < IT; ++it) {
@@ -334,6 +335,8 @@
           const int orow = epi_row(e, row);
           pre[it] = EV == EV_GATE ? *(const bf16x8*)((const bf16*)e.gate + (int64_t)orow * e.ldc + n0 + lc0)
                                   : *(const bf16x8*)((const bf16*)e.res + (int64_t)orow * e.ldr + n0 + lc0);
+          if constexpr (EV == EV_BIAS_RES)
+            prem[it] = e.drop_mask ? drop_mask_bits<8>(e.drop_mask, (uint64_t)orow * (uint64_t)e.N + n0 + lc0) : 0u;
         }
       }
     }
@@ -357,7 +360,8 @@
         if (row < e.M && col < e.N) {
           const f32x4 v0 = *(const f32x4*)(st + lr * LDR + lc0), v1 = *(const f32x4*)(st + lr * LDR + lc0 + 4);
           float v[8] = {v0[0], v0[1], v0[2], v0[3], v1[0], v1[1], v1[2], v1[3]};
-          epi_vec8<T, OutT>(e, epi_row(e, row), col, v, PREB ? bv : nullptr, PREOP ? &pre[it] : nullptr);
+          epi_vec8<T, OutT>(e, epi_row(e, row), col, v, PREB ? bv : nullptr, PREOP ? &pre[it] : nullptr,
+                            PREOP ? prem[it] : 0u);
           if (e.colsum) {
 #pragma unroll
             for (int j = 0; j < 8; ++j) cs[j] += v[j];
diff --git a/avsr_amd/csrc/layernorm.hip b/avsr_amd/csrc/layernorm.hip
--- a/avsr_amd/csrc/layernorm.hip
+++ b/avsr_amd/csrc/layernorm.hip
@@ -11,6 +11,7 @@
   const void* dy; int64_t lddy; void* dx; int64_t lddx; const void* dres; int64_t lddres;
   float* dgamma; float* dbeta; float* ws;
   void* g; int64_t ldg; float drop_p; uint64_t seed; bool db;
+  const uint8_t* mask;
 };
 
 template <typename T, int VPL>
@@ -72,6 +73,7 @@
   for (int row0 = blockIdx.x * W + (threadIdx.x >> 6); row0 < a.rows; row0 += R * nw) {
     float xv[R][VPL][VE], dv[R][VPL][VE], rv[R][VPL][VE];
     float mean[R], rstd[R];
+    uint32_t mb[R][VPL];
     bool live[R];
 #pragma unroll
     for (int u = 0; u < R; ++u) {
@@ -86,6 +88,7 @@
         const int c = min((lane + i * 64) * VE, a.N - VE);
         ldv(x + c, xv[u][i]);
         ldv(dy + c, dv[u][i]);
+        mb[u][i] = a.mask ? drop_mask_bits<VE>(a.mask, (uint64_t)row * a.N + c) : 0u;
         if (dr) ldv(dr + c, rv[u][i]);
         else
 #pragma unroll
@@ -128,7 +131,8 @@
               for (int j = 0; j < VE; ++j) d[j] = to_f(from_f<T>(o[j]));
               if (a.drop_p > 0.f) {
                 const uint64_t i0 = (uint64_t)(row0 + u * nw) * a.N + c;
-                if constexpr (VE == 8) drop8(a.drop_p, a.seed, i0, d);
+                if (a.mask) drop_apply_bits<VE>(mb[u][i], drop_keep_scale(drop_thr16(a.drop_p)), d);
+                else if constexpr (VE == 8) drop8(a.drop_p, a.seed, i0, d);
                 else {
 #pragma unroll
                   for (int j = 0; j < VE; ++j) d[j] *= drop_scale(a.drop_p, a.seed, i0 + j);
@@ -191,6 +195,7 @@
   a.mean = p->mean; a.rstd = p->rstd; a.dy = p->dy; a.lddy = p->lddy; a.dx = p->dx; a.lddx = p->lddx;
   a.dres = p->dres; a.lddres = p->lddres; a.dgamma = p->dgamma; a.dbeta = p->dbeta; a.ws = p->ws;
   a.g = bwd ? p->g : nullptr; a.ldg = p->ldg; a.drop_p = p->drop_p; a.seed = p->seed; a.db = bwd && p->db != nullptr;
+  a.mask = a.g && p->drop_p > 0.f ? (const uint8_t*)p->drop_mask : nullptr;
   if (a.db && (!a.g || !p->dgamma)) return AVSR_E_ARG;
   if (bwd && p->dgamma && (!p->ws || p->N > 2048)) return AVSR_E_ARG;
   const int vpl = (p->N / VE + 63) / 64;
@@ -219,6 +224,7 @@
   if (!p) return AVSR_E_ARG;
   return avsr_by_dtype(p->dtype, [&](auto t) -> int {
     using T = decltype(t);
+    if (bwd && p->drop_mask && (p->N % 8)) return AVSR_E_ARG;
     const int rc = ln_check<T>(p);
     if (rc) return rc;
     if (p->rows == 0) return 0;
diff --git a/avsr_amd/engine.py b/avsr_amd/engine.py
--- a/avsr_amd/engine.py
+++ b/avsr_amd/engine.py
@@ -17,6 +17,7 @@
 WGRAD_GROUP = False
 SIDE_ORDER = "o,f2,f1,c,q"
 ATTN_MASK = True
+HIDDEN_MASK = True
 _CTC_SIDE = True
 _STEM_DIRECT = True
 _LN_EW_FUSE = True
@@ -122,6 +123,8 @@
         self._side_ev = [torch.cuda.Event() for _ in range(8)] if self.side is not None else []
         self._amask, self._amask_wait = None, False
         self._amask_ev = torch.cuda.Event() if self.side is not None else None
+        self._hmask_wait = False
+        self._hmask_ev = torch.cuda.Event() if self.side is not None else None
         self._side_i = 0
         self._side_keep = []
         self._side_defer = None
@@ -618,15 +621,15 @@
 
     def _ln_bwd(self, dy, x, name, mean, rstd, dres=None, dx=None, ew=None):
         if ew is not None and _LN_EW_FUSE:
-            g, p, seed, dbn = ew
+            g, p, seed, dbn, hm = ew
             return ops.layernorm_bwd(dy, x, self.arena.master(name + ".weight"), mean, rstd, dx=dx, dres=dres,
                                      dgamma=self.g(name + ".weight"), dbeta=self.g(name + ".bias"), g=g, drop_p=p,
-                                     seed=seed, db=self.g(dbn))
+                                     seed=seed, db=self.g(dbn), drop_mask=hm)
         out = ops.layernorm_bwd(dy, x, self.arena.master(name + ".weight"), mean, rstd, dx=dx, dres=dres,
                                 dgamma=self.g(name + ".weight"), dbeta=self.g(name + ".bias"))
         if ew is not None:
-            g, p, seed, dbn = ew
-            ops.ew_bwd(out, out=g, drop_p=p, seed=seed, db=self.g(dbn))
+            g, p, seed, dbn, hm = ew
+            ops.ew_bwd(out, out=g, drop_p=p, seed=seed, db=self.g(dbn), drop_mask=hm)
         return out
 
     def encoder_fwd(self, audios, videos, bt, train, save, seeds, modality=None, plan=None):
@@ -640,6 +643,8 @@
         kept = [i for i in range(self.nl) if not (train and draws[i] < self.layerdrop)]
         p_att = cfg.attention_dropout if train else 0.0
         amask = self._attn_masks(B, T, p_att, {i: seeds.peek(3 + 4 * j) for j, i in enumerate(kept)})
+        hmask = self._hidden_masks(M, cfg.hidden_dropout if train else 0.0,
+                                   {i: (seeds.peek(4 + 4 * j), seeds.peek(6 + 4 * j)) for j, i in enumerate(kept)})
         add = self.fuse_add
         fcat = self._e(M, D if add else 2 * D)
         fa = self._e(M, D) if add else fcat[:, :D]
@@ -702,7 +707,8 @@
                 if save:
                     layers.append(None)
                 continue
-            x, lc = self._enc_layer_fwd(i, x, B, T, klen, train, save and 3 + i >= cut, seeds, amask.get(i))
+            x, lc = self._enc_layer_fwd(i, x, B, T, klen, train, save and 3 + i >= cut, seeds, amask.get(i),
+                                        hmask.get(i))
             if save:
                 layers.append(lc)
         E = "encoder.encoder."
@@ -731,7 +737,19 @@
             self._amask_ev.record(self.side)
         return {i: (sd, buf[i]) for i, sd in seeds_by_layer.items()}
 
-    def _enc_layer_fwd(self, i, x, B, T, klen, train, save, seeds, amask=None):
+    def _hidden_masks(self, M, p_h, seeds_by_layer):
+        if not (HIDDEN_MASK and p_h > 0 and self.D % 8 == 0 and seeds_by_layer):
+            return {}
+        nbytes = (ops.drop_mask_bytes(M, self.D) + 15) // 16 * 16
+        buf = torch.empty(2 * len(seeds_by_layer), nbytes, dtype=torch.uint8, device=self.device)
+        sds = [sd for pair in seeds_by_layer.values() for sd in pair]
+        self._on_side(lambda: ops.drop_mask(list(buf), sds, M, self.D, p_h), buf)
+        self._hmask_wait = self.side is not None
+        if self._hmask_wait:
+            self._hmask_ev.record(self.side)
+        return {i: (sd_o, buf[2 * j], sd_f, buf[2 * j + 1]) for j, (i, (sd_o, sd_f)) in enumerate(seeds_by_layer.items())}
+
+    def _enc_layer_fwd(self, i, x, B, T, klen, train, save, seeds, amask=None, hmask=None):
         cfg = self.cfg
         D, H = self.D, self.H
         M = B * T
@@ -756,8 +774,15 @@
                      scale=0.125, drop_p=p_att, seed=sd_att, mask=mask)
         sd_o = seeds.next()
         p_h = cfg.hidden_dropout if train else 0.0
+        hm_o = hm_f = None
+        if hmask is not None:
+            assert hmask[0] == sd_o, "hidden dropout mask seed out of step with the dropout sites"
+            hm_o, hm_f = hmask[1], hmask[3]
+            if self._hmask_wait:
+                torch.cuda.current_stream(self.device).wait_event(self._hmask_ev)
+                self._hmask_wait = False
         x1 = ops.linear_fwd(o, self.w(a + "out_proj.weight"), self.arena.master(a + "out_proj.bias"), res=x,
-                            drop_p=p_h, seed=sd_o)
+                            drop_p=p_h, seed=sd_o, drop_mask=hm_o)
         ln2, m2, r2 = self._ln(x1, p + "final_layer_norm", 1e-5)
         ff = p + "feed_forward."
         h = self._e(M, self.F)
@@ -766,17 +791,19 @@
         act = ops.linear_fwd(ln2, self.w(ff + "intermediate_dense.weight"), self.arena.master(ff + "intermediate_dense.bias"),
                              act=GELU, preact=h, drop_p=p_a, seed=sd_a)
         sd_f = seeds.next()
+        assert hmask is None or hmask[2] == sd_f, "hidden dropout mask seed out of step with the dropout sites"
         x2 = ops.linear_fwd(act, self.w(ff + "output_dense.weight"), self.arena.master(ff + "output_dense.bias"), res=x1,
-                            drop_p=p_h, seed=sd_f)
+                            drop_p=p_h, seed=sd_f, drop_mask=hm_f)
         lc = None
         if save:
             lc = dict(i=i, x=x, ln1=ln1, m1=m1, r1=r1, qkv=qkv, o=o, lse=lse, sd_att=sd_att, p_att=p_att, mask=mask,
-                      sd_o=sd_o, p_h=p_h,
+                      sd_o=sd_o, p_h=p_h, hm_o=hm_o, hm_f=hm_f,
                       x1=x1, ln2=ln2, m2=m2, r2=r2, h=h, act=act, sd_a=sd_a, p_a=p_a, sd_f=sd_f)
         return x2, lc
 
     def _ew_next(self, i, lc, M):
-        return (self._e(M, self.D), lc["p_h"], lc["sd_f"], f"encoder.encoder.layers.{i}.feed_forward.output_dense.bias")
+        return (self._e(M, self.D), lc["p_h"], lc["sd_f"], f"encoder.encoder.layers.{i}.feed_forward.output_dense.bias",
+                lc["hm_f"])
 
     def _enc_layer_bwd(self, i, lc, dx2, B, T, klen, g2=None, lc_prev=None):
         D, H = self.D, self.H
@@ -786,7 +813,8 @@
         ff = p + "feed_forward."
         if g2 is None:
             g2 = self._e(M, D)
-            ops.ew_bwd(dx2, out=g2, drop_p=lc["p_h"], seed=lc["sd_f"], db=self.g(ff + "output_dense.bias"))
+            ops.ew_bwd(dx2, out=g2, drop_p=lc["p_h"], seed=lc["sd_f"], db=self.g(ff + "output_dense.bias"),
+                       drop_mask=lc["hm_f"])
         base = len(self._side_defer) if self._side_defer is not None else None
         tags = [] if base is not None else None
 
@@ -805,7 +833,7 @@
         dln2 = ops.linear_dgrad(dh, self.w(ff + "intermediate_dense.weight"))
         go = self._e(M, D)
         dx1 = self._ln_bwd(dln2, lc["x1"], p + "final_layer_norm", lc["m2"], lc["r2"], dres=dx2, dx=dx2,
-                           ew=(go, lc["p_h"], lc["sd_o"], a + "out_proj.bias"))
+                           ew=(go, lc["p_h"], lc["sd_o"], a + "out_proj.bias", lc["hm_o"]))
         names_b = [a + "q_proj.bias", a + "k_proj.bias", a + "v_proj.bias"]
         names_w = [a + "q_proj.weight", a + "k_proj.weight", a + "v_proj.weight"]
         grouped = WGRAD_GROUP and self._live(*names_w) and self._live(a + "out_proj.weight")
diff --git a/avsr_amd/ops.py b/avsr_amd/ops.py
--- a/avsr_amd/ops.py
+++ b/avsr_amd/ops.py
@@ -89,7 +89,8 @@
 def gemm(A, B, C, *, M, N, K, a_kmajor, b_kmajor, lda, ldb, ldc, batch=1,
          strideA=0, strideB=0, strideC=0, alpha=1.0, beta=0.0, bias=None, act=L.ACT_NONE,
          epi_bwd=False, preact=None, res=None, ldr=None, strideR=0, gate=None, drop_p=0.0, seed=0,
-         splitk=1, ws=None, db=None, db_ws=None, skinny_split=None, ln_c1=None, ln_eps=0.0, kv=None):
+         splitk=1, ws=None, db=None, db_ws=None, skinny_split=None, ln_c1=None, ln_eps=0.0, kv=None,
+         drop_mask=None):
     lib = L.load()
     assert A.is_cuda and B.is_cuda and C.is_cuda
     assert A.dtype == B.dtype, "A/B dtype mismatch"
@@ -118,6 +119,9 @@
     p.gate = None if gate is None else gate.data_ptr()
     p.drop_p, p.seed = float(drop_p), int(seed) & 0xFFFFFFFFFFFFFFFF
     p.splitk = int(splitk)
+    if drop_mask is not None:
+        _check_drop_mask(drop_mask, M, N)
+        p.drop_mask = drop_mask.data_ptr()
     if ws is not None:
         assert ws.dtype == torch.float32 and ws.numel() >= slab_ws(batch, splitk, M, N)
         p.ws = ws.data_ptr()
@@ -172,7 +176,7 @@
 
 
 def linear_fwd(x, W, bias=None, *, act=L.ACT_NONE, preact=None, res=None, drop_p=0.0, seed=0, out=None,
-               skinny_split=None, ln=None, kv=None):
+               skinny_split=None, ln=None, kv=None, drop_mask=None):
     M, K = x.shape
     N = W.shape[0]
     assert W.shape[1] == K and x.stride(1) == 1 and W.stride(1) == 1
@@ -181,7 +185,7 @@
     gemm(x, W, out, M=M, N=N, K=K, a_kmajor=True, b_kmajor=True, lda=x.stride(0), ldb=W.stride(0),
          ldc=out.stride(0), bias=bias, act=act, preact=preact, res=res,
          ldr=None if res is None else res.stride(0), drop_p=drop_p, seed=seed, skinny_split=skinny_split,
-         ln_c1=None if ln is None else ln[0], ln_eps=0.0 if ln is None else ln[1], kv=kv)
+         ln_c1=None if ln is None else ln[0], ln_eps=0.0 if ln is None else ln[1], kv=kv, drop_mask=drop_mask)
     return out
 
 
@@ -353,8 +357,10 @@
 
 
 def layernorm_bwd(dy, x, gamma, mean, rstd, dx=None, dres=None, dgamma=None, dbeta=None, g=None, drop_p=0.0, seed=0,
-                  db=None):
+                  db=None, drop_mask=None):
     rows, N = x.shape
+    if drop_mask is not None:
+        _check_drop_mask(drop_mask, rows, N)
     dx = torch.empty_like(x) if dx is None else dx
     if db is not None:
         assert g is not None and dgamma is not None
@@ -364,7 +370,8 @@
                                         dy=dy, lddy=dy.stride(0), dx=dx, lddx=dx.stride(0),
                                         dres=dres, lddres=0 if dres is None else dres.stride(0),
                                         dgamma=dgamma, dbeta=dbeta, ws=ws, g=g, ldg=0 if g is None else g.stride(0),
-                                        drop_p=float(drop_p), seed=int(seed) & (2 ** 64 - 1), db=db))
+                                        drop_p=float(drop_p), seed=int(seed) & (2 ** 64 - 1), db=db,
+                                        drop_mask=drop_mask))
     return dx
 
 
@@ -680,8 +687,11 @@
         _COLSUM["keep"].clear()
 
 
-def ew_bwd(dy, *, out=None, gate=None, act=L.ACT_NONE, drop_p=0.0, seed=0, alpha=1.0, db=None, inline=False):
+def ew_bwd(dy, *, out=None, gate=None, act=L.ACT_NONE, drop_p=0.0, seed=0, alpha=1.0, db=None, inline=False,
+           drop_mask=None):
     rows, N = dy.shape
+    if drop_mask is not None:
+        _check_drop_mask(drop_mask, rows, N)
     lib = L.load()
     if inline and db is not None:
         ws = torch.empty(256 * N, device=dy.device)
@@ -692,7 +702,7 @@
         _call("avsr_ew_bwd", L.fill(L.EwParams, dtype=dtype_code(dy), rows=rows, N=N, dy=dy, lddy=dy.stride(0),
                                      ws=ws, out=out, ldout=0 if out is None else out.stride(0), gate=gate,
                                      ldgate=0 if gate is None else gate.stride(0), act=act, drop_p=float(drop_p),
-                                     seed=int(seed) & (2 ** 64 - 1), alpha=alpha, db=db))
+                                     seed=int(seed) & (2 ** 64 - 1), alpha=alpha, db=db, drop_mask=drop_mask))
     finally:
         if inline and db is not None:
             lib.avsr_colsum_inline(prev)
@@ -705,6 +715,26 @@
                                       out=out, ldout=out.stride(0), drop_p=float(p),
                                       seed=int(seed) & (2 ** 64 - 1), alpha=1.0))
     return out
+
+
+def drop_mask_bytes(rows, N):
+    return rows * N // 8
+
+
+def _check_drop_mask(mask, rows, N):
+    assert mask.dtype == torch.uint8 and mask.is_cuda and mask.is_contiguous()
+    assert mask.numel() >= (rows * N + 7) // 8, "stored dropout mask smaller than the tensor it covers"
+
+
+def drop_mask(masks, seeds, rows, N, drop_p):
+    k = len(masks)
+    assert len(seeds) == k
+    for m in masks:
+        _check_drop_mask(m, rows, N)
+    sd = (ctypes.c_uint64 * k)(*[int(s) & (2 ** 64 - 1) for s in seeds])
+    ptr = (ctypes.c_void_p * k)(*[m.data_ptr() for m in masks])
+    L.check(L.load().avsr_drop_mask(k, sd, ptr, rows, N, float(drop_p), L.stream_ptr()), "avsr_drop_mask")
+    return masks
 
 
 def mask_rows(x, B, T, lengths):
diff --git a/include/avsr_hip.h b/include/avsr_hip.h
--- a/include/avsr_hip.h
+++ b/include/avsr_hip.h
@@ -66,6 +66,7 @@
   int kv_rows;
   unsigned* slab_cnt;
   int kv_pos_stride;
+  const void* drop_mask;
 } avsr_gemm_params;
 #define AVSR_GEMM_COLSUM_WS(M, N) ((int64_t)(((M) + 63) / 64) * (N))
 #define AVSR_GEMM_SLAB_PAD 1088
@@ -126,6 +127,7 @@
   float* dgamma; float* dbeta;
   float* ws;
   void* g; int64_t ldg; float drop_p; uint64_t seed; float* db;
+  const void* drop_mask;
 } avsr_layernorm_params;
 #define AVSR_LN_BLOCKS 256
 #define AVSR_LN_WS(N) (AVSR_LN_BLOCKS * 2 * (N))
@@ -288,6 +290,7 @@
   float alpha;
   float* db;
   float* ws;
+  const void* drop_mask;
 } avsr_ew_params;
 #define AVSR_EW_ROWBLOCKS 256
 #define AVSR_EW_WS(N) (AVSR_EW_ROWBLOCKS * (N))
@@ -296,6 +299,8 @@
 int avsr_colsum_flush(void* stream);
 int avsr_colsum_inline(int on);
 int avsr_dropout_fwd(const avsr_ew_params* p, void* stream);
+#define AVSR_DROP_MASK_BYTES(rows, N) ((int64_t)(rows) * (N) / 8)
+int avsr_drop_mask(int k, const uint64_t* seeds, void* const* masks, int rows, int N, float drop_p, void* stream);
 int avsr_mask_rows(int dtype, int B, int T, int N, void* x, int64_t ldx, const int* len, void* stream);
 
 typedef struct {
```

Result: no change. 146,800 (-0.4%).
